# unixpickle/learn-nerf

Hardware: AMD Instinct MI355X
Metric: ray-samples/s (NeRF train step: fwd + bwd + Adam, 4096 rays x 192 samples per GPU) (higher is better)
Workload: dtype bf16; 1 GPU; vanilla NeRF coarse64+fine128 train step (BASELINE.json configs[1]); rays_per_gpu=4096, coarse_samples=64, fine_samples=128, global_batch_rays=4096, parallelism=dp1, precision=bf16 MFMA, fp32 accumulate/master weights

## Files before the change

include/lnrf.h:

```cpp
#ifndef LNRF_H
#define LNRF_H

#include <stddef.h>
#include <stdint.h>

#ifdef __cplusplus
extern "C" {
#endif

typedef void* lnrf_stream_t;

#define LNRF_VERSION 200

#define LNRF_OK 0
#define LNRF_ERR_ARG (-1)
#define LNRF_ERR_SHAPE (-2)
#define LNRF_ERR_UNSUPPORTED (-3)

#define LNRF_ACT_NONE 0
#define LNRF_ACT_RELU 1
#define LNRF_ACT_SOFTPLUS 2
#define LNRF_ACT_TANH 3
#define LNRF_ACT_EXP 4
#define LNRF_ACT_SIGMOID 5

int lnrf_version(void);
const char* lnrf_last_error(void);


int lnrf_ray_aabb_stratified(const float* rays, int64_t ray_stride, int64_t n_rays,
                             const float* bbox_min, const float* bbox_max, float min_t_range,
                             float epsilon, int32_t count, const float* u, uint64_t seed,
                             uint32_t stream_id, int64_t ray_offset, float* t_min, float* t_max,
                             uint8_t* mask, float* ts, lnrf_stream_t stream);

int lnrf_camera_rays(const float* origin, const float* x_axis, const float* y_axis, const float* z_axis,
                     float x_fov, float y_fov, int32_t width, int32_t height, float* rays,
                     lnrf_stream_t stream);

int lnrf_gather_rows(const float* src, int64_t n_src, int32_t row_floats, const int32_t* idx, int64_t n,
                     float* out, lnrf_stream_t stream);

int lnrf_stratified(const float* t_min, const float* t_max, int64_t n_rays, int32_t count,
                    const float* u, uint64_t seed, uint32_t stream_id, int64_t ray_offset,
                    float* ts, lnrf_stream_t stream);

int lnrf_ray_points(const float* rays, int64_t ray_stride, const float* ts, int64_t n_rays,
                    int32_t t, float* points, float* dirs, lnrf_stream_t stream);

int lnrf_fine_sample(const float* ts_c, const float* t_min, const float* t_max,
                     const float* density_c, int64_t n_rays, int32_t tc, int32_t tf, float eps,
                     int32_t combine, const float* u, uint64_t seed, uint32_t stream_id,
                     int64_t ray_offset, float* ts_out, lnrf_stream_t stream);

int lnrf_bin_edges(const float* ts, const float* t_min, const float* t_max, int64_t n_rays,
                   int32_t t, float* starts, float* ends, lnrf_stream_t stream);

int lnrf_termination_probs(const float* ts, const float* t_min, const float* t_max,
                           const float* density, int64_t n_rays, int32_t t, float* probs,
                           lnrf_stream_t stream);

int lnrf_composite_fwd(const float* rays, int64_t ray_stride, const float* ts, const float* t_min,
                       const float* t_max, const uint8_t* mask, const float* density,
                       const float* rgb, const float* aux, int32_t n_aux, const float* background,
                       int64_t n_rays, int32_t t, float* outputs, float* alphas, float* coords,
                       float* aux_sum, const float* targets, int64_t target_stride, float* sq_err,
                       lnrf_stream_t stream);

int64_t lnrf_composite_bwd_scratch_bytes(int64_t n_rays);
int lnrf_composite_bwd_det(const float* ts, const float* t_min, const float* t_max, const uint8_t* mask,
                           const float* density, const float* rgb, const float* aux, int32_t n_aux,
                           const float* background, int64_t n_rays, int32_t t, const float* g_out, const float* outputs,
                           const float* targets, int64_t target_stride, float out_scale, const float* g_aux_w,
                           float* g_density, float* g_rgb, float* g_aux, float* g_background, void* scratch,
                           int64_t scratch_bytes, lnrf_stream_t stream);

int lnrf_distortion(const float* ts, const float* t_min, const float* t_max, const uint8_t* mask,
                    const float* density, int64_t n_rays, int32_t t, float grad_scale, float* loss,
                    float* g_density, lnrf_stream_t stream);


int lnrf_sinusoidal_emb(const float* x, int64_t ldx, int64_t m, int32_t dims, int32_t freqs,
                        float* out, int64_t ldo, int64_t col_off, lnrf_stream_t stream);

#define LNRF_DENSE_FP32 0
#define LNRF_DENSE_BF16 1
int lnrf_set_dense_precision(int32_t precision);
int32_t lnrf_get_dense_precision(void);

int lnrf_dense_fwd(const float* x, int64_t ldx, const float* w, const float* b, int32_t act,
                   float* y, int64_t ldy, int64_t m, int32_t k, int32_t n, lnrf_stream_t stream);

int lnrf_act_bwd(float* g, int64_t ldg, const float* y, int64_t ldy, int32_t act, int64_t m,
                 int32_t n, lnrf_stream_t stream);

int lnrf_dense_bwd_input(const float* gy, int64_t ldgy, const float* w, float* gx, int64_t ldgx,
                         int32_t accumulate, int64_t m, int32_t k, int32_t n, lnrf_stream_t stream);

int lnrf_dense_bwd_input_gated(const float* gy, int64_t ldgy, const float* w, const float* y_below, int64_t ldy,
                               int32_t act_below, int32_t n_gated, float* gx, int64_t ldgx, int32_t accumulate,
                               int64_t m, int32_t k, int32_t n, lnrf_stream_t stream);
int lnrf_dense_fwd_gated(const float* x, int64_t ldx, const float* w, const float* b, int32_t act,
                         const float* y_gate, int64_t ldg, int32_t act_gate, float* y, int64_t ldy, int64_t m,
                         int32_t k, int32_t n, lnrf_stream_t stream);

int64_t lnrf_dense_bwd_weight_scratch_bytes(int64_t m, int32_t k, int32_t n);
int lnrf_dense_bwd_weight_det(const float* x, int64_t ldx, const float* gy, int64_t ldgy, float* gw, float* gb,
                              int64_t m, int32_t k, int32_t n, void* scratch, int64_t scratch_bytes,
                              lnrf_stream_t stream);

int lnrf_gemm_f32(const float* a, int64_t sa_i, int64_t sa_r, const float* b, int64_t sb_r, int64_t sb_j,
                  float* c, int64_t ldc, const float* bias, int32_t act, int32_t mode, int64_t i_rows,
                  int32_t j_cols, int64_t r_depth, int32_t splits, lnrf_stream_t stream);

int64_t lnrf_gemm_f32_det_scratch_bytes(int64_t i_rows, int32_t j_cols, int64_t r_depth);
int lnrf_gemm_f32_det(const float* a, int64_t sa_i, int64_t sa_r, const float* b, int64_t sb_r, int64_t sb_j, float* c,
                      int64_t i_rows, int32_t j_cols, int64_t r_depth, void* scratch, int64_t scratch_bytes,
                      lnrf_stream_t stream);


typedef struct {
  int32_t n_levels, feature_dim, smooth, pad_;
  float bbox_min[3], bbox_max[3];
  int32_t grid_size[32];
  int32_t table_size[32];
  int64_t table_offset[32];
  int32_t hashed[32];
} lnrf_hashgrid_desc;

int lnrf_hashgrid_fwd(const lnrf_hashgrid_desc* desc, const float* tables, const float* x, int64_t m,
                      float* enc_t, lnrf_stream_t stream);

int64_t lnrf_hashgrid_bwd_scratch_bytes(const lnrf_hashgrid_desc* desc, int64_t m);
int lnrf_hashgrid_bwd_bucketed(const lnrf_hashgrid_desc* desc, const float* x, const float* u, int64_t m,
                               const float* g_enc_t, const float* level_absmax, float* g_tables, void* scratch,
                               int64_t scratch_bytes, lnrf_stream_t stream);

int lnrf_hashgrid_jvp(const lnrf_hashgrid_desc* desc, const float* tables, const float* x, const float* u,
                      int64_t m, float* enc_t, lnrf_stream_t stream);
int lnrf_hashgrid_input_grad(const lnrf_hashgrid_desc* desc, const float* tables, const float* x, int64_t m,
                             const float* g_enc_t, float* g_x, lnrf_stream_t stream);
int lnrf_hashgrid_bwd_dir(const lnrf_hashgrid_desc* desc, const float* x, const float* u, int64_t m,
                          const float* g_enc_t, float* g_tables, lnrf_stream_t stream);


int lnrf_sinusoidal_emb_bwd(const float* x, int64_t ldx, int64_t m, int32_t dims, int32_t freqs,
                            const float* g_emb, int64_t ldg, int64_t col_off, float* g_x,
                            lnrf_stream_t stream);
int lnrf_sinusoidal_emb_jvp(const float* x, int64_t ldx, int64_t m, int32_t dims, int32_t freqs,
                            const float* u, float* v_emb, int64_t ldv, int64_t col_off,
                            lnrf_stream_t stream);

int lnrf_integrated_directional_encoding(int32_t sh_degree, const float* coords, const float* roughness,
                                         int64_t m, float* out, lnrf_stream_t stream);

int lnrf_refnerf_head_fwd(const float* spatial, int64_t lds, const float* nraw, const float* d, int64_t m,
                          int32_t sh_degree, float* density, float* diffuse, float* spectral, float* tail,
                          int64_t ld_tail, float* aux, lnrf_stream_t stream);
int lnrf_refnerf_head_bwd(const float* spatial, int64_t lds, const float* nraw, const float* d, int64_t m,
                          int32_t sh_degree, const float* g_density, const float* g_diffuse,
                          const float* g_spectral, const float* g_tail, int64_t ld_tail, const float* g_aux,
                          float* g_spatial, int64_t ldgs, float* g_nraw, lnrf_stream_t stream);

int lnrf_refnerf_color_fwd(const float* dir_out, const float* spectral, const float* diffuse, int64_t m,
                           float* rgb, lnrf_stream_t stream);
int lnrf_refnerf_color_bwd(const float* dir_out, const float* spectral, const float* diffuse, int64_t m,
                           const float* g_rgb, float* g_dir_out, float* g_spectral, float* g_diffuse,
                           lnrf_stream_t stream);


typedef struct {
  int32_t input_layers, mid_layers, hidden_dim, color_layer_dim, x_freqs, d_freqs;
} lnrf_nerf_shape;

int64_t lnrf_nerf_param_count(const lnrf_nerf_shape* shape);
int64_t lnrf_nerf_packed_bytes(const lnrf_nerf_shape* shape);
int64_t lnrf_nerf_save_bytes(const lnrf_nerf_shape* shape, int64_t m);
int64_t lnrf_nerf_bwd_scratch_bytes(const lnrf_nerf_shape* shape, int64_t m);

int lnrf_nerf_pack_weights(const lnrf_nerf_shape* shape, const float* params, void* packed,
                           lnrf_stream_t stream);

int lnrf_nerf_mlp_fwd(const lnrf_nerf_shape* shape, const void* packed, const float* x,
                      const float* d, const float* rays, int64_t ray_stride, const float* ts,
                      int32_t t, int64_t m, float* density, float* rgb, void* save,
                      lnrf_stream_t stream);

int lnrf_nerf_mlp_fwd_ls(const lnrf_nerf_shape* shape, const void* packed, const float* x,
                         const float* d, const float* rays, int64_t ray_stride, const float* ts,
                         int32_t t, int64_t m, float* density, float* rgb, void* save,
                         lnrf_stream_t stream);

int64_t lnrf_nerf_packed_split_bytes(const lnrf_nerf_shape* shape);
int lnrf_nerf_pack_weights_split(const lnrf_nerf_shape* shape, const float* params, void* packed_split,
                                 lnrf_stream_t stream);
int lnrf_nerf_mlp_fwd_split(const lnrf_nerf_shape* shape, const void* packed_split, const float* x,
                            const float* d, const float* rays, int64_t ray_stride, const float* ts,
                            int32_t t, int64_t m, float* density, float* rgb, lnrf_stream_t stream);

int lnrf_nerf_mlp_bwd_chain(const lnrf_nerf_shape* shape, const void* packed, const void* save,
                            const float* density, const float* rgb, const float* g_density,
                            const float* g_rgb, int64_t m, void* scratch, lnrf_stream_t stream);

int lnrf_nerf_mlp_bwd_weights(const lnrf_nerf_shape* shape, const void* save, void* scratch,
                              int64_t m, float* grads, lnrf_stream_t stream);

int64_t lnrf_nerf_bwd_ls_scratch_bytes(const lnrf_nerf_shape* shape, int64_t m);
int64_t lnrf_nerf_bwd_ls_status_offset(const lnrf_nerf_shape* shape, int64_t m);
int lnrf_nerf_mlp_bwd_ls(const lnrf_nerf_shape* shape, const void* packed, const void* save,
                         const float* density, const float* rgb, const float* g_density,
                         const float* g_rgb, int64_t m, void* scratch, float* grads, int32_t phases,
                         lnrf_stream_t stream);
int lnrf_nerf_mlp_bwd_ls2(const lnrf_nerf_shape* shape, const void* packed_a, const void* save_a,
                          const float* density_a, const float* rgb_a, const float* g_density_a,
                          const float* g_rgb_a, int64_t m_a, void* scratch_a, float* grads_a,
                          const void* packed_b, const void* save_b, const float* density_b,
                          const float* rgb_b, const float* g_density_b, const float* g_rgb_b, int64_t m_b,
                          void* scratch_b, float* grads_b, int32_t phases, lnrf_stream_t stream);

int64_t lnrf_refnerf_trunk_packed_bytes(void);
int lnrf_refnerf_trunk_pack(const float* params, void* packed, lnrf_stream_t stream);
int lnrf_refnerf_trunk_fwd(const void* packed, const float* x, int64_t m, void* save, float* spatial_out,
                           int64_t ld, lnrf_stream_t stream);
int lnrf_refnerf_normal_pass(const void* packed, const void* save, const float* x, int64_t m, void* cdump,
                             float* nraw, lnrf_stream_t stream);
int64_t lnrf_refnerf_trunk_bwd_scratch_bytes(int64_t m);
int lnrf_refnerf_trunk_bwd(const void* packed, const void* save, const float* g_spatial, int64_t ld, int64_t m,
                           void* scratch, float* grads, lnrf_stream_t stream);
// ... 154 lines not shown
```

learn-nerf_amd/csrc/layout_host.cpp:

```cpp
#include <stdint.h>
#include <string.h>

#include "dense_plan.h"
#include "fast_math.h"
#include "hashgrid_plan.h"
#include "nerf_wgrad.h"
#include "ngp_layout.h"

using namespace lnrf;

static WgradList wgrad_list_of(int which, int64_t n_tiles) {
  return which == 0 ? wgrad_list_split(n_tiles) : which == 1 ? wgrad_list_ls_finish(n_tiles)
       : which == 2 ? wgrad_list_ref_trunk(n_tiles) : which == 3 ? wgrad_list_ref_normal(n_tiles)
                                                                 : wgrad_list_ref_dir(n_tiles);
}
template <int NXF, int NYF, int WI, int WO>
static int64_t wgrad_count_owners(const WgradProblem& pb, int32_t* count, int64_t n) {
  int64_t outside = 0;
  int64_t i;
  auto hit = [&](bool owned) {
    if (!owned) return;
    if (i >= 0 && i < n) ++count[i];
    else ++outside;
  };
  for (int w = 0; w < kWaves; ++w)
    for (int j = 0; j < kWgradWaveTiles<NXF, NYF, WI, WO>; ++j) {
      const WgradTile tile = wgrad_tile<NXF, NYF, WI, WO>(w, j);
      if (!tile.real) continue;
      for (int lane = 0; lane < 64; ++lane) {
        const int colr = lane & 31, hh = lane >> 5;
        const WgradOwner<NerfWgradEpi, WgradProblem> own(pb, tile.ot, colr);
        if (tile.bias && pb.do_bias) hit(own.bias(hh, i));
        for (int qq = 0; qq < 16; ++qq) hit(own.weight(pb, tile.it, hh, qq, i));
      }
    }
  return outside;
}

template <int P>
static int64_t ngp_count_owners(const NgpWgradProblem& pb, int64_t dense_off, int32_t* count, int64_t n) {
  constexpr int NO = kNgpWgrad[P].nyf / 2, NT = ngp_wgrad_tiles(P);
  int64_t outside = 0;
  auto hit = [&](int part, int64_t i) {
    if (i >= 0 && i < n) ++count[part * n + i];
    else ++outside;
  };
  for (int w4 = 0; w4 < 4; ++w4)
    for (int lane = 0; lane < 64; ++lane) {
      const int colr = lane & 31, hh = lane >> 5;
      const int tile_id = w4 % NT, part = w4 / NT;
      const int it = tile_id / NO, ot = tile_id % NO;
      int out_idx = -1, out_dim = 1;
      int64_t w_off = 0, b_off = 0;
      NgpWgradEpi::cols(pb, ot, colr, out_idx, out_dim, w_off, b_off);
      w_off -= dense_off;
      b_off -= dense_off;
      if (it == 0 && hh == 0 && out_idx >= 0) hit(part, b_off + out_idx);
      for (int qq = 0; qq < 16; ++qq) {
        const int r = ngp_acc_row(qq, hh);
        const int f = 2 * it + (r >> 4);
        const int in_idx = NgpWgradEpi::row(pb, f, r & 15);
        if (out_idx >= 0 && in_idx >= 0) hit(part, w_off + (int64_t)in_idx * out_dim + out_idx);
      }
    }
  return outside;
}
static bool ngp_enc_dim_ok(int enc_dim) { return enc_dim >= 1 && enc_dim <= 32; }
static HashGridDesc hashgrid_desc_of(const void* desc) {
  HashGridDesc d;
  memcpy(&d, desc, sizeof(d));
  return d;
}

extern "C" {
int lnrf_host_fwd_frags(void) { return kFwdFrags; }
int lnrf_host_bwd_frags(void) { return kBwdFrags; }
int lnrf_host_bias_floats(void) { return kBiasFloats; }
int lnrf_host_fwd_used(void) { return kFwdUsed; }
int lnrf_host_fwd_seq(int c) { return fwd_seq(c); }
int lnrf_host_fwd3_frags(void) { return kFwd3Frags; }
int lnrf_host_fwd3_used(void) { return kFwd3Used; }
int lnrf_host_fwd3_seq(int c) { return fwd3_seq(c); }
int lnrf_host_fwd3_base(int s) { return fwd3_base(s); }
int lnrf_host_bwd_seq(int c) { return bwd_seq(c); }
int lnrf_host_fwd_layer_info(int s, int what) {
  return what == 0 ? fwd_nk(s) : what == 1 ? fwd_no(s) : what == 2 ? fwd_base(s) : what == 3 ? fwd_bias_base(s)
                                                                                             : fwd_cons_base(s);
}
int lnrf_host_bwd_layer_info(int t, int what) {
  return what == 0 ? bwd_nk(t) : what == 1 ? bwd_no(t) : what == 2 ? bwd_base(t) : bwd_dense(t);
}
int lnrf_host_fwd_weight_index(int g, int lane, int j) { return fwd_stream_index(g, lane, j, false); }
int lnrf_host_bwd_weight_index(int g, int lane, int j) { return bwd_stream_index(g, lane, j, false); }
int lnrf_host_fwd_bias_index(int i) { return bias_block_index(i, false); }
int lnrf_host_nrm_frags(void) { return kNrmFrags; }
int lnrf_host_nrm_weight_index(int g, int lane, int j) { return nrm_stream_index(g, lane, j); }
int64_t lnrf_host_stream_indices(int stream, int ref, int32_t* out) {
  const int frags[8] = {kFwdFrags, kBwdFrags, kFwd3Frags, 0, kNrmFrags, kDirFwdFrags, kDirBwdFrags, 0};
  if (stream < 0 || stream > 7) return -1;
  if (stream == 3 || stream == 7) {
    const int n = stream == 3 ? kBiasFloats : kDirBiasFloats;
    for (int i = 0; out && i < n; ++i) out[i] = stream == 3 ? bias_block_index(i, ref != 0) : dir_bias_index(i);
    return n;
  }
  const int64_t n = (int64_t)frags[stream] * 512;
  for (int64_t e = 0; out && e < n; ++e) {
    const int g = (int)(e >> 9), lane = (int)((e >> 3) & 63), j = (int)(e & 7);
    out[e] = stream == 0 ? fwd_stream_index(g, lane, j, ref != 0) : stream == 1 ? bwd_stream_index(g, lane, j, ref != 0)
           : stream == 2 ? fwd3_stream_index(g, lane, j, ref != 0) : stream == 4 ? nrm_stream_index(g, lane, j)
           : stream == 5 ? dir_fwd_weight_index(g, lane, j) : dir_bwd_weight_index(g, lane, j);
  }
  return n;
}
int64_t lnrf_host_pack_offset(int what) {
  const int64_t v[17] = {kPackFwdOff, kPackBwdOff, kPackBiasOff, kPackBytes, kPack3BiasOff, kPack3Bytes,
                         kRefPackNrmOff, kRefPackDirFwdOff, kRefPackDirBwdOff, kRefPackDirBiasOff, kRefPackBytes,
                         kRef3FwdOff, kRef3BiasOff, kRef3NrmOff, kRef3DirOff, kRef3DirBiasOff, kRef3Bytes};
  return what >= 0 && what < 17 ? v[what] : -1;
}
int lnrf_host_xemb_feat(int ks, int h, int j) { return xemb_feat(ks, h, j); }
int lnrf_host_save_slot(int what, int arg) {
  return what == 0 ? kSaveXin : what == 1 ? kSaveH + 16 * arg : what == 2 ? kSaveZ : what == 3 ? kSaveDin
       : what == 4 ? kSaveH10 : what == 5 ? kSaveMask : kSaveSlots;
}
int lnrf_host_grad_slot(int what, int arg) {
  return what == 0 ? kGradDy11 : what == 1 ? kGradDy10m : what == 2 ? grad_dy_slot(arg) : kGradSlots;
}
int lnrf_host_dir_slot(int what) {
  const int v[7] = {kDirSaveXin, kDirSaveH, kDirSaveMask, kDirSaveSlots, kDirGradDy10, kDirGradDy9, kDirGradSlots};
  return what >= 0 && what < 7 ? v[what] : -1;
}
int lnrf_host_demb_feat(int ks, int h, int j) { return demb_feat(ks, h, j); }
int lnrf_host_hidden_feat(int ks, int h, int j) { return hidden_feat(ks, h, j); }
int lnrf_host_dump_info(int what) { return what == 0 ? kFragBytes : what == 1 ? kTileCols : kWaves; }
int lnrf_host_mask_bit(int ks, int j) { return 16 * (ks >> 1) + 8 * (ks & 1) + j; }
int lnrf_host_dump_lane_off(int slot, int c, int hh) { return dump_lane_off(slot, c, hh); }
void lnrf_host_sincos_pe(float r, float* s, float* c) { lnrf::sincos_pe(r, s, c); }

int lnrf_host_wgrad_const(int what) {
  const int v[8] = {kWgradMaxBlocks, kSlabMaxTiles, kSlabMaxTO, kParamCount, kDirW9, kDirB9, kDirW10, kDirB10};
  return v[what];
}
int lnrf_host_wgrad_list(int which, int64_t n_tiles, int32_t* out) {
  const WgradList list = wgrad_list_of(which, n_tiles);
  for (int i = 0; i < list.args.n_problems; ++i) {
    const WgradProblem& pb = list.args.p[i];
    int32_t* o = out + 6 * i;
    o[0] = pb.first_block; o[1] = pb.n_blocks; o[4] = pb.do_bias; o[5] = 0;
    switch (pb.shape) {
#define X(name, id, NXF, NYF, WI, WO, SPI) case name: o[2] = WgShape<name>::TI * WgShape<name>::TO; o[3] = WgShape<name>::TO; break;
      LNRF_WGRAD_SHAPES(X, X)
#undef X
      default: return -1;
    }
    switch (pb.shape) {
#define X(name) case name:
      LNRF_WGRAD_LS_SHAPES(X, X) o[5] = 1; break;
#undef X
      default: break;
    }
  }
  return list.args.n_problems;
}
int64_t lnrf_host_ngp_stream_indices(int stream, int enc_dim, int32_t* out) {
  if (stream < 0 || stream > 2 || !ngp_enc_dim_ok(enc_dim)) return -1;
  const NgpOffsets off = ngp_offsets(enc_dim, 0);
  const int ne = ngp_ne(enc_dim);
  const int64_t n = stream == 2 ? kNgpBiasFloats : (int64_t)kNgpStreamFrags * 512;
  for (int64_t e = 0; out && e < n; ++e) {
    const int g = (int)(e >> 9), lane = (int)((e >> 3) & 63), j = (int)(e & 7);
    out[e] = (int32_t)(stream == 0 ? ngp_fwd_stream_index(g, lane, j, off, enc_dim, ne)
                     : stream == 1 ? ngp_bwd_stream_index(g, lane, j, off, enc_dim, ne) : ngp_bias_index((int)e, off));
  }
  return n;
}
int64_t lnrf_host_ngp_pack_offset(int what) {
  const int64_t v[7] = {kNgpPackBiasOff, kNgpPackBytes, kNgpSplitBiasOff, kNgpSplitBytes, kNgpStreamFrags,
                        kNgpSplitMaxFrags / 2, kNgpMaxParts};
  return what >= 0 && what < 7 ? v[what] : -1;
}
int64_t lnrf_host_ngp_wgrad_owners(int enc_dim, int32_t* count, int64_t n) {
  if (!ngp_enc_dim_ok(enc_dim)) return -1;
  const int64_t dense_off = 1001;
  const NgpWgradArgs a = ngp_wgrad_args(ngp_offsets(enc_dim, dense_off), enc_dim);
  return ngp_count_owners<0>(a.p[0], dense_off, count, n) + ngp_count_owners<1>(a.p[1], dense_off, count, n) +
         ngp_count_owners<2>(a.p[2], dense_off, count, n) + ngp_count_owners<3>(a.p[3], dense_off, count, n) +
         ngp_count_owners<4>(a.p[4], dense_off, count, n);
}
int lnrf_host_ngp_parts_plan(int enc_dim, int32_t* out) {
  if (!ngp_enc_dim_ok(enc_dim)) return -1;
  const NgpPartsPlan pl = ngp_parts_plan(ngp_offsets(enc_dim, 1001), 1001);
  for (int i = 0; i < kNgpLayers; ++i) {
    int32_t* o = out + 4 * i;
    o[0] = kNgpWgrad[i].layer; o[1] = pl.lo[i]; o[2] = pl.hi[i]; o[3] = pl.parts[i];
  }
  return ngp_dense_params(enc_dim);
}
void lnrf_host_gemm_plan(int64_t sa_i, int64_t sa_r, int64_t sb_r, int64_t sb_j, int64_t I, int32_t J, int64_t R,
                         uint32_t a_low, uint32_t b_low, int32_t bf16, int32_t mode, int32_t splits, int64_t* out) {
  const GemmPlan p = gemm_plan(sa_i, sa_r, sb_r, sb_j, I, J, R, a_low, b_low, bf16 != 0, mode, splits);
  const int64_t v[15] = {p.launch, p.big, p.bf16, p.a_fast_r, p.b_fast_r, p.b_aligned, p.kc, p.nsplit, p.lda, p.ldb,
                         p.r_per_split, p.gx, p.gy, p.gz, p.splits};
  for (int i = 0; i < 15; ++i) out[i] = v[i];
}
void lnrf_host_gemm_tile(int64_t I, int32_t J, uint32_t block0, int64_t count, int64_t* out) {
  for (int64_t e = 0; e < count; ++e) {
    const GemmTile t = gemm_big_tile(block0 + (uint32_t)e, (I + BI - 1) / BI, (J + BJ - 1) / BJ);
    out[2 * e] = t.it;
    out[2 * e + 1] = t.jt;
  }
}
int64_t lnrf_host_dense_bwd_weight_scratch_bytes(int64_t m, int32_t k, int32_t n) { return dense_wgrad_scratch_bytes(m, k, n); }
int64_t lnrf_host_gemm_det_scratch_bytes(int64_t I, int32_t J, int64_t R) { return gemm_det_scratch_bytes(I, J, R); }
void lnrf_host_hashgrid_corners(const void* desc, int32_t level, const float* x, uint32_t* idx, float* w, float* dw) {
  const HashGridDesc d = hashgrid_desc_of(desc);
  const int G = d.grid_size[level];
  const Corner k = locate(x, d, G);
  for (int c = 0; c < 8; ++c) {
    const int xo = c >> 2, yo = (c >> 1) & 1, zo = c & 1;
    idx[c] = entry_index(k.base[0] + xo, k.base[1] + yo, k.base[2] + zo, G, d.table_size[level], d.hashed[level]);
    w[c] = corner_weight(k, xo, yo, zo);
    corner_weight_grad(k, xo, yo, zo, dw + 3 * c);
  }
}
int64_t lnrf_host_hashgrid_xcd_plan(const void* desc, const int32_t* levels, int32_t n, int64_t m, int32_t* plan,
                                    int64_t* work) {
  const HashGridDesc d = hashgrid_desc_of(desc);
  LevelList ll;
  ll.n = n;
  for (int i = 0; i < n; ++i) ll.level[i] = levels[i];
  unsigned grid = 0;
  const XcdPlan p = make_xcd_plan(d, ll, m, &grid);
  for (int x = 0; plan && x <= kXcds; ++x) plan[x] = p.first_seg[x];
  for (int s = 0; plan && s < p.n_segs; ++s) {
    plan[9 + 3 * s] = p.seg_level[s]; plan[10 + 3 * s] = p.seg_chunk0[s]; plan[11 + 3 * s] = p.seg_chunks[s];
  }
  for (unsigned b = 0; work && b < grid; ++b) {
    const XcdWork w = xcd_work(p, b);
    work[2 * b] = w.seg < 0 ? -1 : xcd_level(p, w);
    work[2 * b + 1] = w.seg < 0 ? 0 : xcd_first_sample(p, w);
  }
  return grid;
}
int32_t lnrf_host_hashgrid_bucket_plan(const void* desc, int64_t m, int64_t* levels, int64_t* scratch) {
  const BucketPlan p = make_plan(hashgrid_desc_of(desc), m);
  for (int i = 0; i < p.n; ++i) {
    const int64_t v[7] = {p.level[i], p.slices[i], p.split[i], p.wg_off[i], p.tuple_off[i], p.cursor_off[i], p.cap[i]};
    for (int j = 0; j < 7; ++j) levels[7 * i + j] = v[j];
  }
  const BucketScratch s = bucket_scratch(p);
  scratch[0] = s.cursor_bytes; scratch[1] = s.level_max_off; scratch[2] = s.tuple_off; scratch[3] = s.total;
  scratch[4] = p.wg_off[p.n];
  return p.n;
}
void lnrf_host_hashgrid_reduce_work(const void* desc, int64_t m, int32_t block0, int64_t count, int64_t tuples,
                                    int64_t* out) {
  const BucketPlan p = make_plan(hashgrid_desc_of(desc), m);
  for (int64_t e = 0; e < count; ++e) {
    const ReduceWork w = reduce_work(p, block0 + (int)e);
    const TupleRange r = reduce_range(p, w, tuples);
    const int64_t v[6] = {w.li, w.level, w.bucket, w.part, r.lo, r.hi};
    for (int j = 0; j < 6; ++j) out[6 * e + j] = v[j];
  }
}
int64_t lnrf_host_wgrad_owners(int which, int64_t n_tiles, int32_t* count, int64_t n) {
  const WgradList list = wgrad_list_of(which, n_tiles);
// ... 13 lines not shown
```

learn-nerf_amd/csrc/nerf_bwd_ls.hip:

```cpp
#include "nerf_chain.h"

namespace lnrf {

constexpr int kLsWaves = 4;
constexpr int kLsThreads = kLsWaves * 64;
constexpr int kLsStages = 8;
constexpr int kLsLag = 2;
constexpr int kLsDist = kLsLag + 1;
constexpr int kLsBufs = kLsDist + 1;
constexpr int kLsTileBytes = 32 * kFragBytes;
constexpr int kLsPollOff = kLsBufs * kLsTileBytes;
constexpr int kLsLds = kLsPollOff + 5 * 256;
constexpr unsigned kLsMaxSpins = 1u << 18;
constexpr int kLsSlabWaveFloats = 16 * kSlabTileFloats + 2 * 64;
constexpr int64_t kLsSlabBlockBytes = (int64_t)kLsWaves * kLsSlabWaveFloats * (int64_t)sizeof(float);
constexpr int kLsCounterStride = 32;

struct LsJob {
  const char* packed;
  const char* save;
  char* gdump;
  unsigned* counters;
  float* slabs;
  unsigned* status;
// ... 391 lines not shown
    }
  } else if (bid - n_small < kLsStages * 64) {
    ls_fold_block<kSlabReduceWaves>(bid - n_small, a.ls_slabs[k], a.pipelines[k], a.grads[k], lds);
  }
}

struct BwdHeadSeq {
  static constexpr int count = bwd_cons_base(2);
  static constexpr int at(int c) { return bwd_seq(c); }
};
constexpr int kBwdHeadStages = bwd_base(2) / kStageFrags;

__global__ __launch_bounds__(kThreads) void nerf_bwd_head_kernel(
    const char* __restrict__ packed, const char* __restrict__ save, const float* __restrict__ density,
    const float* __restrict__ rgb, const float* __restrict__ g_density, const float* __restrict__ g_rgb,
    int64_t M, int64_t n_tiles, char* __restrict__ gdump, unsigned* __restrict__ zero_words, int n_zero_words) {
  const int tid = threadIdx.x;
  const int lane = tid & 63;
  const int wave = __builtin_amdgcn_readfirstlane(tid >> 6);
  const int64_t tile = (int64_t)blockIdx.x * kWaves + wave;
  for (int i = blockIdx.x * kThreads + tid; i < n_zero_words; i += gridDim.x * kThreads) zero_words[i] = 0u;
  Ring<kBwdHeadStages, BwdHeadSeq> ring;
  ring.stream = packed + kPackBwdOff;
  ring.wave = wave;
  ring.lane = lane;
  const DumpAddr gd{gdump, n_tiles, tile, lane & 31, lane >> 5, kGradTileSlots};
  bwd_chain_tile<true>(ring, gd, save, n_tiles, density, rgb, g_density, g_rgb, M, tile, lane);
}

}

using namespace lnrf;

#ifdef LNRF_TIMELINE
extern "C" int lnrf_debug_set_ls_timeline(void* buf) {
  hipError_t e = hipMemcpyToSymbol(HIP_SYMBOL(lnrf::g_ls_timeline_buf), &buf, sizeof(buf));
  return e == hipSuccess ? LNRF_OK : hip_fail(e, "hipMemcpyToSymbol(g_ls_timeline_buf)");
}
#endif

constexpr int kLsMaxPipelines = 64;
static int ls_pipelines_for_device(int need, int* out) {
  int cus = 0;
  if (int rc = cu_count(&cus)) return rc;
  *out = cus / kLsStages < kLsMaxPipelines ? cus / kLsStages : kLsMaxPipelines;
  if (*out < need) {
    set_error("layer-stationary backward: the device has too few CUs for a pipeline of 8 per model");
    return LNRF_ERR_UNSUPPORTED;
  }
  return LNRF_OK;
}

constexpr int64_t kLsCounterWords = (int64_t)kLsMaxPipelines * kLsStages * kLsCounterStride;
constexpr int64_t kLsCounterBytes = (kLsCounterWords + 64) * (int64_t)sizeof(unsigned);
struct LsScratch {
  int64_t small_slabs, counters, status, ls_slabs, bytes;
};
static LsScratch ls_scratch(int64_t m) {
  LsScratch s;
  s.small_slabs = (int64_t)kGradSlots * padded_tiles(m) * kFragBytes;
  s.counters = s.small_slabs + kWgradSlabBytes;
  s.status = s.counters + kLsCounterWords * (int64_t)sizeof(unsigned);
  s.ls_slabs = s.counters + kLsCounterBytes;
  s.bytes = s.ls_slabs + (int64_t)kLsMaxPipelines * kLsStages * kLsSlabBlockBytes;
  return s;
}
static LsJob ls_job(const void* packed, const void* save, void* scratch, int64_t m, int pipelines) {
  const LsScratch at = ls_scratch(m);
  char* sc = (char*)scratch;
  return LsJob{(const char*)packed, (const char*)save, sc, reinterpret_cast<unsigned*>(sc + at.counters),
               reinterpret_cast<float*>(sc + at.ls_slabs), reinterpret_cast<unsigned*>(sc + at.status), padded_tiles(m),
               pipelines};
}

extern "C" int64_t lnrf_nerf_bwd_ls_scratch_bytes(const lnrf_nerf_shape* s, int64_t m) {
  return nerf_shape_fused(s) ? ls_scratch(m).bytes : -1;
}
extern "C" int64_t lnrf_nerf_bwd_ls_status_offset(const lnrf_nerf_shape* s, int64_t m) {
  return nerf_shape_fused(s) ? ls_scratch(m).status : -1;
}
int64_t lnrf::ls_scratch_bytes(int64_t m) { return ls_scratch(m).bytes; }
float* lnrf::ls_small_slabs(void* scratch, int64_t m) {
  return reinterpret_cast<float*>((char*)scratch + ls_scratch(m).small_slabs);
}

int lnrf::launch_ls_pipeline(const void* packed, const void* save, void* scratch, int64_t m, float* grads, hipStream_t st) {
  int total = 0;
  int rc = ls_pipelines_for_device(1, &total);
  if (!rc) rc = set_max_dynamic_lds(nerf_bwd_ls_kernel, kLsLds);
  if (rc) return rc;
  LsArgs a;
  a.n_jobs = 1;
  a.total_pipelines = total;
  a.job[0] = a.job[1] = ls_job(packed, save, scratch, m, total);
  hipError_t e = hipMemsetAsync(a.job[0].counters, 0, kLsCounterBytes, st);
  if (e != hipSuccess) return hip_fail(e, "hipMemsetAsync(counters)");
  hipLaunchKernelGGL(nerf_bwd_ls_kernel, dim3((unsigned)(total * kLsStages)), dim3(kLsThreads), kLsLds, st, a);
  LNRF_LAUNCH_CHECK();
  hipLaunchKernelGGL(nerf_ls_reduce_kernel, dim3(kLsStages * 64), dim3(256), 0, st, (const float*)a.job[0].slabs, total, grads);
  LNRF_LAUNCH_CHECK();
  return LNRF_OK;
}

namespace {
struct LsModel {
  const void* packed;
  const void* save;
  const float *density, *rgb, *g_density, *g_rgb;
  int64_t m;
  void* scratch;
  float* grads;
};
}

static int ls_backward(const LsModel* mdl, int n_models, int phases, hipStream_t st) {
  constexpr int kHeadLds = kRingBytes + round_up(kBiasFloats * 4, 1024);
  int total = 0;
  int rc = ls_pipelines_for_device(n_models, &total);
  if (!rc) rc = set_max_dynamic_lds(nerf_bwd_head_kernel, kHeadLds);
  if (!rc) rc = set_max_dynamic_lds(nerf_bwd_ls_kernel, kLsLds);
  if (rc) return rc;
  int pipes[2] = {total, 0};
  if (n_models == 2) {
    const double share = (double)mdl[0].m / (double)(mdl[0].m + mdl[1].m);
    pipes[0] = (int)(total * share + 0.5);
    if (pipes[0] < 1) pipes[0] = 1;
    if (pipes[0] > total - 1) pipes[0] = total - 1;
    pipes[1] = total - pipes[0];
  }
  LsArgs a;
  a.n_jobs = n_models;
  a.total_pipelines = total;
  for (int k = 0; k < n_models; ++k) {
    const LsModel& md = mdl[k];
    const LsJob& j = a.job[k] = ls_job(md.packed, md.save, md.scratch, md.m, pipes[k]);
    if (phases & 1) {
      hipLaunchKernelGGL(nerf_bwd_head_kernel, dim3((unsigned)(j.n_tiles / kWaves)), dim3(kThreads), kHeadLds, st, j.packed,
                         j.save, md.density, md.rgb, md.g_density, md.g_rgb, md.m, j.n_tiles, j.gdump, j.counters,
                         (phases & 2) ? (int)(kLsCounterBytes / sizeof(unsigned)) : 0);
      LNRF_LAUNCH_CHECK();
    }
    if ((phases & 3) == 2) {
      hipError_t e = hipMemsetAsync(j.counters, 0, kLsCounterBytes, st);
      if (e != hipSuccess) return hip_fail(e, "hipMemsetAsync(counters)");
    }
  }
  if (n_models == 1) a.job[1] = a.job[0];
  if (phases & 2) {
    hipLaunchKernelGGL(nerf_bwd_ls_kernel, dim3((unsigned)(total * kLsStages)), dim3(kLsThreads), kLsLds, st, a);
    LNRF_LAUNCH_CHECK();
  }
  if (!(phases & 4)) return LNRF_OK;
  LsFoldArgs fold;
  for (int k = 0; k < n_models; ++k) {
    const LsModel& md = mdl[k];
    const LsJob& j = a.job[k];
    const WgradList w = wgrad_list_ls_finish(j.n_tiles);
    float* small_slabs = ls_small_slabs(md.scratch, md.m);
    rc = launch_nerf_wgrad(w, md.save, md.scratch, j.n_tiles, md.grads, st, WgLayout{kSaveTileSlots, kGradTileSlots, 1},
                           small_slabs, false, false);
    if (rc) return rc;
    fold.w[k] = w.args;
    fold.small_slabs[k] = small_slabs;
    fold.ls_slabs[k] = j.slabs;
    fold.grads[k] = md.grads;
    fold.pipelines[k] = pipes[k];
  }
  if (n_models == 1) {
    fold.w[1] = fold.w[0]; fold.small_slabs[1] = fold.small_slabs[0]; fold.ls_slabs[1] = fold.ls_slabs[0];
    fold.grads[1] = fold.grads[0]; fold.pipelines[1] = fold.pipelines[0];
  }
  const int gx = fold.w[0].n_problems * kWaves * kSlabMaxTiles + kLsStages * 64;
  hipLaunchKernelGGL(nerf_ls_fold_kernel, dim3((unsigned)gx, (unsigned)n_models), dim3(64 * kSlabReduceWaves), 0, st, fold);
  LNRF_LAUNCH_CHECK();
  return LNRF_OK;
}

extern "C" int lnrf_nerf_mlp_bwd_ls(const lnrf_nerf_shape* shape, const void* packed, const void* save,
                                    const float* density, const float* rgb, const float* g_density,
                                    const float* g_rgb, int64_t m, void* scratch, float* grads, int32_t phases,
                                    lnrf_stream_t stream) {
  LNRF_REQUIRE_NERF_SHAPE(shape);
  LNRF_CHECK_ARG(packed && save && density && rgb && g_density && g_rgb && scratch && grads, "null pointer");
  LNRF_CHECK_ARG(m >= 0, "bad m");
  if (m == 0) return LNRF_OK;
  LNRF_CHECK_ARG(phases >= 1 && phases <= 7, "phases: bit 0 head, bit 1 pipeline, bit 2 small problems + fold");
  const LsModel md{packed, save, density, rgb, g_density, g_rgb, m, scratch, grads};
  return ls_backward(&md, 1, phases, as_stream(stream));
}

extern "C" int lnrf_nerf_mlp_bwd_ls2(const lnrf_nerf_shape* shape, const void* packed_a, const void* save_a,
                                     const float* density_a, const float* rgb_a, const float* g_density_a,
                                     const float* g_rgb_a, int64_t m_a, void* scratch_a, float* grads_a,
                                     const void* packed_b, const void* save_b, const float* density_b,
                                     const float* rgb_b, const float* g_density_b, const float* g_rgb_b, int64_t m_b,
                                     void* scratch_b, float* grads_b, int32_t phases, lnrf_stream_t stream) {
  LNRF_REQUIRE_NERF_SHAPE(shape);
  LNRF_CHECK_ARG(packed_a && save_a && density_a && rgb_a && g_density_a && g_rgb_a && scratch_a && grads_a, "null pointer");
  LNRF_CHECK_ARG(packed_b && save_b && density_b && rgb_b && g_density_b && g_rgb_b && scratch_b && grads_b, "null pointer");
  LNRF_CHECK_ARG(m_a > 0 && m_b > 0, "both models need evaluations (use lnrf_nerf_mlp_bwd_ls for one)");
  const LsModel md[2] = {{packed_a, save_a, density_a, rgb_a, g_density_a, g_rgb_a, m_a, scratch_a, grads_a},
                         {packed_b, save_b, density_b, rgb_b, g_density_b, g_rgb_b, m_b, scratch_b, grads_b}};
  LNRF_CHECK_ARG(phases >= 1 && phases <= 7, "phases: bit 0 head, bit 1 pipeline, bit 2 small problems + fold");
  return ls_backward(md, 2, phases, as_stream(stream));
}
```

learn-nerf_amd/csrc/nerf_chain.h:

```cpp
#pragma once
#include "fused_chain.h"

namespace lnrf {

template <class Put>
__device__ __forceinline__ void x_encode(const float (&px)[3], int h, Put put) {
  static_for<4>([&](auto ks_) {
    constexpr int ks = decltype(ks_)::value;
#pragma unroll
    for (int pp = 0; pp < 4; ++pp) {
      const int p = 4 * ks + pp;
      float s = 0.0f, co = 0.0f;
      if (p < kXPairs) {
        const int pg = kXPairs * h + p;
        const int cd = pg / kXFreqs, f = pg - kXFreqs * cd;
        const float v = cd == 0 ? px[0] : (cd == 1 ? px[1] : px[2]);
        sincos_pe(v * (float)(1 << f), &s, &co);
      }
      put(ks_, 2 * pp, s);
      put(ks_, 2 * pp + 1, co);
    }
  });
}

template <int S, bool BIAS, class RING, class Epi>
__device__ __forceinline__ void trunk_layer(RING& ring, int h, const bf16x8 (&xe)[4], const bf16x8 (&in)[16], Epi epi) {
  chain_layer<fwd_cons_base(S), fwd_nk(S), fwd_no(S)>(
      ring,
      [&](auto o_) {
        if constexpr (BIAS) return bias_acc(fwd_bias_base(S) + 32 * decltype(o_)::value, h);
        else return zero_acc();
      },
      [&](auto k_) -> bf16x8 {
        constexpr int ks = decltype(k_)::value;
        if constexpr (S == 0) return xe[ks];
        else if constexpr (ks < 16) return in[ks];
        else return xe[ks - 16];
      },
      epi);
}
template <int S, class RING, class Epi>
__device__ __forceinline__ void trunk_layer_split(RING& ring, int h, const bf16x8 (&xe_hi)[4], const bf16x8 (&xe_lo)[4],
                                                  const bf16x8 (&inh)[16], const bf16x8 (&inl)[16], Epi epi) {
  chain_layer_split<fwd_cons_base(S), fwd_nk(S), fwd_no(S)>(
      ring, [&](auto o_) { return bias_acc(fwd_bias_base(S) + 32 * decltype(o_)::value, h); },
      [&](auto k_) -> bf16x8 {
        constexpr int ks = decltype(k_)::value;
        if constexpr (S == 0) return xe_hi[ks];
        else if constexpr (ks < 16) return inh[ks];
        else return xe_hi[ks - 16];
      },
      [&](auto k_) -> bf16x8 {
        constexpr int ks = decltype(k_)::value;
        if constexpr (S == 0) return xe_lo[ks];
        else if constexpr (ks < 16) return inl[ks];
        else return xe_lo[ks - 16];
      },
      epi);
}
template <int O>
__device__ __forceinline__ void masked_out_tile(const f32x16& acc, const uint4& mk, bf16x8 (&out)[16], const DumpAddr& gd,
                                                int slot0) {
  const unsigned mb = mask_word(mk, O);
  out[2 * O] = masked_frag<0>(acc, mb, 16 * (O & 1));
  out[2 * O + 1] = masked_frag<1>(acc, mb, 16 * (O & 1));
  gd.store(slot0 + 2 * O, frag_to_bits(out[2 * O]));
  gd.store(slot0 + 2 * O + 1, frag_to_bits(out[2 * O + 1]));
}
template <int C0, int L, class RING>
__device__ __forceinline__ void hidden_back(RING& ring, bf16x8 (&in)[16], bf16x8 (&out)[16], const uint4& mk,
                                            const DumpAddr& gd) {
  chain_layer<C0, 16, 8>(
      ring, [&](auto) { return zero_acc(); }, [&](auto k_) -> bf16x8 { return in[decltype(k_)::value]; },
      [&](auto o_, const f32x16& acc) { masked_out_tile<decltype(o_)::value>(acc, mk, out, gd, grad_dy_slot(L - 1)); });
}

struct BwdSeq {
  static constexpr int count = kBwdUsed;
  static constexpr int at(int c) { return bwd_seq(c); }
};
constexpr int kBwdStages = kBwdFrags / kStageFrags;

template <bool HEAD_ONLY = false, class RING>
__device__ __forceinline__ void bwd_chain_tile(RING& ring, const DumpAddr& gd, const char* __restrict__ save,
                                               int64_t save_tiles, const float* __restrict__ density,
                                               const float* __restrict__ rgb, const float* __restrict__ g_density,
                                               const float* __restrict__ g_rgb, int64_t M, int64_t tile, int lane) {
  const int c = lane & 31, h = lane >> 5;
  const int64_t m = tile * kTileCols + c;
  const bool valid = m < M;

  float gy11[3] = {0, 0, 0}, gy9 = 0.0f;
  if (valid && h == 0) {
#pragma unroll
    for (int k = 0; k < 3; ++k) {
      const float y = rgb[m * 3 + k];
      gy11[k] = g_rgb[m * 3 + k] * (1.0f - y * y);
    }
    gy9 = g_density[m] * -expm1f(-density[m]);
  }
  uint4 relu_mask[9];
#pragma unroll
  for (int i = HEAD_ONLY ? 8 : 0; i < 9; ++i)
    relu_mask[i] = *mask_at(save, kSaveMask + i, tile, save_tiles, kSaveTileSlots, lane);
  __syncthreads();
  ring.prologue();
  LNRF_TL_STAMP(ring);

  bf16x8 a0[16], a1[16];

  bf16x8 dy11 = zero_frag();
  dy11[0] = (__bf16)gy11[0];
  dy11[1] = (__bf16)gy11[1];
  dy11[2] = (__bf16)gy11[2];
  gd.store(kGradDy11, frag_to_bits(dy11));
  gd.store(kGradDy11 + 1, frag_to_bits(zero_frag()));

  chain_layer<bwd_cons_base(0), bwd_nk(0), bwd_no(0)>(
      ring, [&](auto) { return zero_acc(); }, [&](auto) -> bf16x8 { return dy11; },
      [&](auto o_, const f32x16& acc) {
        masked_out_tile<decltype(o_)::value>(acc, relu_mask[8], a0, gd, kGradDy10m);
      });
  bf16x8 dlogit = zero_frag();
  dlogit[0] = (__bf16)gy9;
  gd.store(kGradDy10m + 8, frag_to_bits(dlogit));
  gd.store(kGradDy10m + 9, frag_to_bits(zero_frag()));

  chain_layer<bwd_cons_base(1), bwd_nk(1), bwd_no(1)>(
      ring, [&](auto) { return zero_acc(); },
      [&](auto k_) -> bf16x8 {
        constexpr int ks = decltype(k_)::value;
        if constexpr (ks < 8) return a0[ks];
        else return dlogit;
      },
      [&](auto o_, const f32x16& acc) {
        constexpr int o = decltype(o_)::value;
        a1[2 * o] = acc_to_frag<0, false>(acc);
        a1[2 * o + 1] = acc_to_frag<1, false>(acc);
        gd.store(grad_dy_slot(8) + 2 * o, frag_to_bits(a1[2 * o]));
        gd.store(grad_dy_slot(8) + 2 * o + 1, frag_to_bits(a1[2 * o + 1]));
      });

  if constexpr (HEAD_ONLY) return;
  static_assert(bwd_nk(2) == 16 && bwd_no(2) == 8, "hidden_back");
  static_for<8>([&](auto i_) {
    constexpr int TT = 2 + decltype(i_)::value, l = bwd_dense(TT);
    if constexpr (TT % 2 == 0) hidden_back<bwd_cons_base(TT), l>(ring, a1, a0, relu_mask[l - 1], gd);
    else hidden_back<bwd_cons_base(TT), l>(ring, a0, a1, relu_mask[l - 1], gd);
  });
}

int launch_nerf_wgrad(const WgradList& list, const void* xbuf, const void* ybuf, int64_t n_tiles, float* grads,
                      hipStream_t stream, WgLayout lay, float* slabs, bool plain_loads = false,
                      bool fold = true);

int64_t ls_scratch_bytes(int64_t m);
float* ls_small_slabs(void* scratch, int64_t m);
int launch_ls_pipeline(const void* packed, const void* save, void* scratch, int64_t m, float* grads, hipStream_t stream);

}
```

learn-nerf_amd/csrc/nerf_layout.h:

```cpp
#pragma once
#include <stdint.h>

#if defined(__HIPCC__)
#define NL_HD __host__ __device__ __forceinline__
#else
#define NL_HD inline
#endif

namespace lnrf {
namespace nl {

constexpr int kFragBytes = 1024;
constexpr int kStageFrags = 16;
constexpr int kTileCols = 32;
constexpr int kWaves = 8;

constexpr int kNumDense = 12;
NL_HD constexpr int dense_in(int l) {
  return l == 0 ? 60 : (l == 5 ? 316 : (l == 10 ? 280 : (l == 11 ? 128 : 256)));
}
NL_HD constexpr int dense_out(int l) { return l == 9 ? 1 : (l == 10 ? 128 : (l == 11 ? 3 : 256)); }
NL_HD constexpr int dense_w_off(int l) {
  int off = 0;
  for (int i = 0; i < l; ++i) off += dense_in(i) * dense_out(i) + dense_out(i);
// ... 127 lines not shown
NL_HD constexpr int bwd_cons_base(int t) {
  int b = 0;
  for (int i = 0; i < t; ++i) b += bwd_nk(i) * bwd_no(i);
  return b;
}
constexpr int kBwdUsed = bwd_cons_base(kBwdLayers);
NL_HD constexpr int bwd_seq(int c) {
  int t = 0;
  for (int i = 1; i < kBwdLayers; ++i)
    if (c >= bwd_cons_base(i)) t = i;
  return bwd_base(t) + (c - bwd_cons_base(t));
}
NL_HD constexpr int bwd_dense(int t) { return t == 0 ? 11 : (t == 1 ? 10 : 10 - t); }

NL_HD constexpr int bwd_weight_index(int t, int o, int ks, int lane, int j) {
  const int r = lane & 31, h = lane >> 5;
  const int in = 32 * o + r;
  if (t == 0) {
    if (h != 0 || j >= 3) return -1;
    return dense_w_off(11) + in * 3 + j;
  }
  if (t == 1) {
    if (ks < 8) return dense_w_off(10) + in * 128 + hidden_feat(ks, h, j);
    if (h == 0 && j == 0) return dense_w_off(9) + in;
    return -1;
  }
  const int l = bwd_dense(t);
  return dense_w_off(l) + in * 256 + hidden_feat(ks, h, j);
}

constexpr int kNrmLayers = 10;
NL_HD constexpr bool nrm_is_x(int u) { return u == 3 || u == 9; }
NL_HD constexpr int nrm_nk(int) { return 16; }
NL_HD constexpr int nrm_no(int u) { return nrm_is_x(u) ? 2 : 8; }
NL_HD constexpr int nrm_base(int u) {
  int b = 0;
  for (int i = 0; i < u; ++i) b += nrm_nk(i) * nrm_no(i);
  return b;
}
constexpr int kNrmFrags = nrm_base(kNrmLayers);
static_assert(kNrmFrags == 1088 && kNrmFrags % kStageFrags == 0, "normal-pass stream length");
NL_HD constexpr int nrm_seq(int c) { return c; }
NL_HD constexpr int nrm_dense(int u) { return u < 3 ? 8 - u : (u == 4 ? 5 : 9 - u); }
NL_HD constexpr int nrm_x_row(int o, int r) {
  const int hh = (r >> 2) & 1, q = (r & 3) + 4 * (r >> 3);
  const int pg = 16 * o + 8 * hh + (q >> 1);
  if (pg >= 30) return -1;
  return 20 * (pg / 10) + (pg % 10) + 10 * (q & 1);
}
NL_HD constexpr int nrm_weight_index(int u, int o, int ks, int lane, int j) {
  const int r = lane & 31, h = lane >> 5;
  const int k = hidden_feat(ks, h, j);
  if (nrm_is_x(u)) {
    const int e = nrm_x_row(o, r);
    if (e < 0) return -1;
    return u == 3 ? dense_w_off(5) + (256 + e) * 256 + k : dense_w_off(0) + e * 256 + k;
  }
  return dense_w_off(nrm_dense(u)) + (32 * o + r) * 256 + k;
}

constexpr int64_t kPackFwdOff = 0;
constexpr int64_t kPackBwdOff = (int64_t)kFwdFrags * kFragBytes;
constexpr int64_t kPackBiasOff = kPackBwdOff + (int64_t)kBwdFrags * kFragBytes;
constexpr int64_t kPackBytes = kPackBiasOff + round_up(kBiasFloats * 4, 1024);
constexpr int kDirIn = 273, kDirHidden = 128;
constexpr int kDirW9 = dense_w_off(9);
constexpr int kDirB9 = kDirW9 + kDirIn * kDirHidden;
constexpr int kDirW10 = kDirB9 + kDirHidden;
constexpr int kDirB10 = kDirW10 + kDirHidden * 3;
constexpr int kDirFwdFrags = 96, kDirBwdFrags = 96, kDirBiasFloats = 160;
NL_HD constexpr int dir_fwd_seq(int c) { return c < 72 ? c : 80 + (c - 72); }
NL_HD constexpr int dir_bwd_seq(int c) { return c < 4 ? c : 16 + (c - 4); }
NL_HD constexpr int dir_fwd_weight_index(int g, int lane, int j) {
  const int r = lane & 31, h = lane >> 5;
  if (g < 72) {
    const int o = g / 18, ks = g % 18;
    const int in = hidden_feat(ks, h, j);
    return in < kDirIn ? kDirW9 + in * kDirHidden + 32 * o + r : -1;
  }
  if (g >= 80 && g < 88) {
    if (r >= 3) return -1;
    return kDirW10 + hidden_feat(g - 80, h, j) * 3 + r;
  }
  return -1;
}
NL_HD constexpr int dir_bwd_weight_index(int g, int lane, int j) {
  const int r = lane & 31, h = lane >> 5;
  if (g < 4) {
    if (h != 0 || j >= 3) return -1;
    return kDirW10 + (32 * g + r) * 3 + j;
  }
  if (g >= 16 && g < 88) {
    const int o = (g - 16) / 8, ks = (g - 16) % 8;
    const int in = 32 * o + r;
    return in < kDirIn ? kDirW9 + in * kDirHidden + hidden_feat(ks, h, j) : -1;
  }
  return -1;
}
NL_HD constexpr int dir_bias_index(int i) { return i < 128 ? kDirB9 + i : (i < 131 ? kDirB10 + (i - 128) : -1); }
constexpr int kDirSaveXin = 0, kDirSaveH = 18, kDirSaveMask = 26, kDirSaveSlots = 27;
constexpr int kDirGradDy10 = 0, kDirGradDy9 = 2, kDirGradSlots = 10;

constexpr int64_t kRefPackNrmOff = kPackBytes;
constexpr int64_t kRefPackDirFwdOff = kRefPackNrmOff + (int64_t)kNrmFrags * kFragBytes;
constexpr int64_t kRefPackDirBwdOff = kRefPackDirFwdOff + (int64_t)kDirFwdFrags * kFragBytes;
constexpr int64_t kRefPackDirBiasOff = kRefPackDirBwdOff + (int64_t)kDirBwdFrags * kFragBytes;
constexpr int64_t kRefPackBytes = kRefPackDirBiasOff + 1024;
constexpr int kRef3FwdFrags = fwd3_base(9);
constexpr int64_t kRef3FwdOff = 0;
constexpr int64_t kRef3BiasOff = (int64_t)kRef3FwdFrags * kFragBytes;
constexpr int64_t kRef3NrmOff = kRef3BiasOff + round_up(kBiasFloats * 4, 1024);
constexpr int64_t kRef3DirOff = kRef3NrmOff + 2 * (int64_t)kNrmFrags * kFragBytes;
constexpr int64_t kRef3DirBiasOff = kRef3DirOff + 2 * (int64_t)kDirFwdFrags * kFragBytes;
constexpr int64_t kRef3Bytes = kRef3DirBiasOff + 1024;
static_assert(kRef3FwdFrags % kStageFrags == 0 && (2 * kNrmFrags) % kStageFrags == 0 && (2 * kDirFwdFrags) % kStageFrags == 0,
              "split streams are whole stages");

NL_HD constexpr int fwd_stream_index(int g, int lane, int j, bool ref) {
  int s = 0;
  for (int i = 1; i < kFwdLayers; ++i)
    if (g >= fwd_base(i)) s = i;
  const int loc = g - fwd_base(s), nk = fwd_nk(s);
  if (loc >= nk * fwd_no(s) || (ref && s > 8)) return -1;
  return fwd_weight_index(s, loc / nk, loc % nk, lane, j);
}
NL_HD constexpr int bwd_stream_index(int g, int lane, int j, bool ref) {
  int t = 0;
  for (int i = 1; i < kBwdLayers; ++i)
    if (g >= bwd_base(i)) t = i;
  const int loc = g - bwd_base(t), nk = bwd_nk(t);
  if (loc >= nk * bwd_no(t) || (ref && t < 2)) return -1;
  return bwd_weight_index(t, loc / nk, loc % nk, lane, j);
}
NL_HD constexpr int nrm_stream_index(int g, int lane, int j) {
  int u = 0;
  for (int i = 1; i < kNrmLayers; ++i)
    if (g >= nrm_base(i)) u = i;
  const int loc = g - nrm_base(u);
  return nrm_weight_index(u, loc / nrm_nk(u), loc % nrm_nk(u), lane, j);
}
NL_HD constexpr int fwd3_stream_index(int g, int lane, int j, bool ref) {
  int s = 0;
  for (int i = 1; i < kFwdLayers; ++i)
    if (g >= fwd3_base(i)) s = i;
  const int pair = (g - fwd3_base(s)) >> 1, nk = fwd_nk(s);
  if (pair >= nk * fwd_no(s) || (ref && s > 8)) return -1;
  return fwd_weight_index(s, pair / nk, pair % nk, lane, j);
}
NL_HD constexpr int bias_block_index(int i, bool ref) {
  int s = 0;
  for (int k = 1; k < kFwdLayers; ++k)
    if (i >= fwd_bias_base(k)) s = k;
  return ref && s > 8 ? -1 : fwd_bias_index(s, i - fwd_bias_base(s));
}

NL_HD constexpr int dump_lane_off(int slot, int c, int hh) {
  return 256 * (c >> 3) + 128 * (((c >> 2) & 1) ^ (slot & 1)) + 64 * hh + 16 * (c & 3);
}
constexpr int kSaveXin = 0;
constexpr int kSaveH = 4;
constexpr int kSaveZ = 4 + 8 * 16;
constexpr int kSaveDin = kSaveZ + 16;
constexpr int kSaveH10 = kSaveDin + 2;
constexpr int kSaveMask = kSaveH10 + 8;
constexpr int kSaveSlots = kSaveMask + 9;
constexpr int kGradDy11 = 0;
constexpr int kGradDy10m = 2;
constexpr int kGradDy = 12;
constexpr int kGradSlots = kGradDy + 9 * 16;
constexpr int kSaveTileSlots = kSaveSlots, kGradTileSlots = kGradSlots;
constexpr int kDirSaveTileSlots = kDirSaveSlots, kDirGradTileSlots = kDirGradSlots;
NL_HD constexpr int grad_dy_pos(int l) { return l == 5 ? 8 : (l > 5 ? 8 - l : 7 - l); }
NL_HD constexpr int grad_dy_slot(int l) { return kGradDy + grad_dy_pos(l) * 16; }

}
}
```

learn-nerf_amd/csrc/nerf_mlp.hip:

```cpp
#include "nerf_chain.h"

namespace lnrf {

constexpr int kFusedLds = kRingBytes + round_up(kBiasFloats * 4, 1024);
#ifdef LNRF_TIMELINE
__device__ unsigned long long* g_timeline_buf = nullptr;
#endif

struct FwdSeq {
  static constexpr int count = kFwdUsed;
  static constexpr int at(int c) { return fwd_seq(c); }
};

constexpr int kFwdStages = kFwdFrags / kStageFrags;

template <bool SAVE, bool FROM_RAYS, bool HMASKS = true>
__global__ __launch_bounds__(kThreads) void nerf_fwd_kernel(
    const char* __restrict__ packed, const float* __restrict__ xin_g, const float* __restrict__ din_g,
    const float* __restrict__ rays, int64_t ray_stride, const float* __restrict__ ts, int T, int64_t M,
    int64_t n_tiles, float* __restrict__ density, float* __restrict__ rgb, char* __restrict__ save) {
  const auto [lane, wave, c, h, tile, m, valid] = tile_ctx<kWaves>(M);

  stage_bias<kThreads>(packed + kPackBiasOff, kBiasFloats);
  float px[3] = {0, 0, 0}, pd[3] = {0, 0, 0};
  if (valid) {
    if (FROM_RAYS) {
      const int64_t n = m / T;
      const float t = ts[m];
      const float* r = rays + n * ray_stride;
#pragma unroll
      for (int a = 0; a < 3; ++a) {
        pd[a] = r[3 + a];
        px[a] = r[a] + pd[a] * t;
      }
    } else {
#pragma unroll
      for (int a = 0; a < 3; ++a) {
        px[a] = xin_g[m * 3 + a];
        pd[a] = din_g[m * 3 + a];
      }
    }
  }
  __syncthreads();

  Ring<kFwdStages, FwdSeq> ring;
  ring.stream = packed + kPackFwdOff;
  ring.wave = wave;
  ring.lane = lane;
#ifdef LNRF_TIMELINE
  ring.tl.buf = g_timeline_buf + (SAVE ? 0 : 8 * 1024);
  ring.tl.n = 0;
  ring.tl.on = g_timeline_buf != nullptr && blockIdx.x == gridDim.x / 2;
  ring.tl.stamp();
#endif
  ring.prologue();
  LNRF_TL_STAMP(ring);

  bf16x8 xe[4], de[2];
  x_encode(px, h, [&](auto ks_, int j, float v) { xe[decltype(ks_)::value][j] = (__bf16)v; });
  static_for<2>([&](auto ks_) {
    constexpr int ks = decltype(ks_)::value;
#pragma unroll
    for (int pp = 0; pp < 4; ++pp) {
      const int p = 4 * ks + pp;
      float s = 0.0f, co = 0.0f;
      if (p < 6) {
        const int pg = 6 * h + p;
        const int cd = pg >> 2, f = pg & 3;
        const float v = cd == 0 ? pd[0] : (cd == 1 ? pd[1] : pd[2]);
        sincos_pe(v * (float)(1 << f), &s, &co);
      }
      de[ks][2 * pp] = (__bf16)s;
      de[ks][2 * pp + 1] = (__bf16)co;
    }
  });

  DumpAddr dump{save, n_tiles, tile, c, h, kSaveTileSlots};
  auto save_frag = [&](int slot, const bf16x8& f) {
    if (SAVE) dump.store(slot, frag_to_bits(f));
  };
  if (SAVE) {
    static_for<4>([&](auto i) { save_frag(kSaveXin + decltype(i)::value, xe[decltype(i)::value]); });
    static_for<2>([&](auto i) { save_frag(kSaveDin + decltype(i)::value, de[decltype(i)::value]); });
  }

  bf16x8 a0[16], a1[16];
  unsigned mask_bits[4] = {0u, 0u, 0u, 0u};

  auto hidden = [&](auto s_, bf16x8(&in)[16], bf16x8(&out)[16], auto relu_, int save_slot) {
    constexpr int S = decltype(s_)::value;
    constexpr bool RELU = decltype(relu_)::value;
    trunk_layer<S, true>(ring, h, xe, in, [&](auto o_, const f32x16& acc) {
      constexpr int o = decltype(o_)::value;
      out[2 * o] = acc_to_frag<0, RELU>(acc);
      out[2 * o + 1] = acc_to_frag<1, RELU>(acc);
      save_frag(save_slot + 2 * o, out[2 * o]);
      save_frag(save_slot + 2 * o + 1, out[2 * o + 1]);
      if constexpr (SAVE && RELU && HMASKS)
        mask_bits[o >> 1] |= relu_bits(out[2 * o], out[2 * o + 1]) << (16 * (o & 1));
    });
    if constexpr (SAVE && RELU && HMASKS) {
      *mask_at(save, kSaveMask + S, tile, n_tiles, kSaveTileSlots, lane) =
          make_uint4(mask_bits[0], mask_bits[1], mask_bits[2], mask_bits[3]);
      mask_bits[0] = mask_bits[1] = mask_bits[2] = mask_bits[3] = 0u;
    }
  };
  std::true_type relu;
  std::false_type lin;
  hidden(std::integral_constant<int, 0>{}, a1, a0, relu, kSaveH + 0 * 16);
  hidden(std::integral_constant<int, 1>{}, a0, a1, relu, kSaveH + 1 * 16);
  hidden(std::integral_constant<int, 2>{}, a1, a0, relu, kSaveH + 2 * 16);
  hidden(std::integral_constant<int, 3>{}, a0, a1, relu, kSaveH + 3 * 16);
  hidden(std::integral_constant<int, 4>{}, a1, a0, relu, kSaveH + 4 * 16);
  hidden(std::integral_constant<int, 5>{}, a0, a1, relu, kSaveH + 5 * 16);
  hidden(std::integral_constant<int, 6>{}, a1, a0, relu, kSaveH + 6 * 16);
  hidden(std::integral_constant<int, 7>{}, a0, a1, relu, kSaveH + 7 * 16);
  hidden(std::integral_constant<int, 8>{}, a1, a0, lin, kSaveZ);

  chain_layer<fwd_cons_base(9), fwd_nk(9), fwd_no(9)>(
      ring, [&](auto o_) { return bias_acc(fwd_bias_base(9) + 32 * decltype(o_)::value, h); },
      [&](auto k_) -> bf16x8 {
        constexpr int ks = decltype(k_)::value;
        if constexpr (ks < 16) return a0[ks];
        else return de[ks - 16];
      },
      [&](auto o_, const f32x16& acc) {
        constexpr int o = decltype(o_)::value;
        if constexpr (o < 4) {
          a1[2 * o] = acc_to_frag<0, true>(acc);
          a1[2 * o + 1] = acc_to_frag<1, true>(acc);
          save_frag(kSaveH10 + 2 * o, a1[2 * o]);
          save_frag(kSaveH10 + 2 * o + 1, a1[2 * o + 1]);
          if constexpr (SAVE) mask_bits[o >> 1] |= relu_bits(a1[2 * o], a1[2 * o + 1]) << (16 * (o & 1));
        } else {
          if constexpr (SAVE)
            *mask_at(save, kSaveMask + 8, tile, n_tiles, kSaveTileSlots, lane) = make_uint4(mask_bits[0], mask_bits[1], 0u, 0u);
          if (h == 0 && valid) {
            const float x = acc[0];
            density[m] = fmaxf(x, 0.0f) + log1pf(expf(-fabsf(x)));
          }
        }
      });
  chain_layer<fwd_cons_base(10), fwd_nk(10), fwd_no(10)>(
      ring, [&](auto) { return bias_acc(fwd_bias_base(10), h); },
      [&](auto k_) -> bf16x8 { return a1[decltype(k_)::value]; },
      [&](auto, const f32x16& acc) {
        if (h == 0 && valid) {
          rgb[m * 3 + 0] = tanhf(acc[0]);
          rgb[m * 3 + 1] = tanhf(acc[1]);
          rgb[m * 3 + 2] = tanhf(acc[2]);
        }
      });
// ... 4 lines not shown
  static constexpr int count = kFwd3Used;
  static constexpr int at(int c) { return fwd3_seq(c); }
};

template <bool FROM_RAYS>
__global__ __launch_bounds__(kSplitThreads) void nerf_fwd_split_kernel(
    const char* __restrict__ packed, const float* __restrict__ xin_g, const float* __restrict__ din_g,
    const float* __restrict__ rays, int64_t ray_stride, const float* __restrict__ ts, int T, int64_t M,
    float* __restrict__ density, float* __restrict__ rgb) {
  const auto [lane, wave, c, h, tile, m, valid] = tile_ctx<kSplitWaves>(M);

  stage_bias<kSplitThreads>(packed + kPack3BiasOff, kBiasFloats);
  float px[3] = {0, 0, 0}, pd[3] = {0, 0, 0};
  if (valid) {
    if (FROM_RAYS) {
      const int64_t n = m / T;
      const float t = ts[m];
      const float* r = rays + n * ray_stride;
#pragma unroll
      for (int a = 0; a < 3; ++a) {
        pd[a] = r[3 + a];
        px[a] = r[a] + pd[a] * t;
      }
    } else {
#pragma unroll
      for (int a = 0; a < 3; ++a) {
        px[a] = xin_g[m * 3 + a];
        pd[a] = din_g[m * 3 + a];
      }
    }
  }
  __syncthreads();

  Ring<kFwd3Stages, Fwd3Seq, kSplitWaves> ring;
  ring.stream = packed;
  ring.wave = wave;
  ring.lane = lane;
  ring.prologue();

  bf16x8 xe_hi[4], xe_lo[4], de_hi[2], de_lo[2];
  x_encode(px, h, [&](auto ks_, int j, float v) { split_store(v, xe_hi[decltype(ks_)::value], xe_lo[decltype(ks_)::value], j); });
  static_for<2>([&](auto ks_) {
    constexpr int ks = decltype(ks_)::value;
#pragma unroll
    for (int pp = 0; pp < 4; ++pp) {
      const int p = 4 * ks + pp;
      float s = 0.0f, co = 0.0f;
      if (p < 6) {
        const int pg = 6 * h + p;
        const int cd = pg >> 2, f = pg & 3;
        const float v = cd == 0 ? pd[0] : (cd == 1 ? pd[1] : pd[2]);
        sincos_pe(v * (float)(1 << f), &s, &co);
      }
      split_store(s, de_hi[ks], de_lo[ks], 2 * pp);
      split_store(co, de_hi[ks], de_lo[ks], 2 * pp + 1);
    }
  });

  bf16x8 a0h[16], a0l[16], a1h[16], a1l[16];

  auto hidden = [&](auto s_, bf16x8(&inh)[16], bf16x8(&inl)[16], bf16x8(&outh)[16], bf16x8(&outl)[16], auto relu_) {
    constexpr bool RELU = decltype(relu_)::value;
    trunk_layer_split<decltype(s_)::value>(ring, h, xe_hi, xe_lo, inh, inl, [&](auto o_, const f32x16& acc) {
      constexpr int o = decltype(o_)::value;
      acc_to_frag_split<0, RELU>(acc, outh[2 * o], outl[2 * o]);
      acc_to_frag_split<1, RELU>(acc, outh[2 * o + 1], outl[2 * o + 1]);
    });
  };
  std::true_type relu;
  std::false_type lin;
  hidden(std::integral_constant<int, 0>{}, a1h, a1l, a0h, a0l, relu);
  hidden(std::integral_constant<int, 1>{}, a0h, a0l, a1h, a1l, relu);
  hidden(std::integral_constant<int, 2>{}, a1h, a1l, a0h, a0l, relu);
  hidden(std::integral_constant<int, 3>{}, a0h, a0l, a1h, a1l, relu);
  hidden(std::integral_constant<int, 4>{}, a1h, a1l, a0h, a0l, relu);
  hidden(std::integral_constant<int, 5>{}, a0h, a0l, a1h, a1l, relu);
  hidden(std::integral_constant<int, 6>{}, a1h, a1l, a0h, a0l, relu);
  hidden(std::integral_constant<int, 7>{}, a0h, a0l, a1h, a1l, relu);
  hidden(std::integral_constant<int, 8>{}, a1h, a1l, a0h, a0l, lin);

  chain_layer_split<fwd_cons_base(9), fwd_nk(9), fwd_no(9)>(
      ring, [&](auto o_) { return bias_acc(fwd_bias_base(9) + 32 * decltype(o_)::value, h); },
      [&](auto k_) -> bf16x8 {
        constexpr int ks = decltype(k_)::value;
        if constexpr (ks < 16) return a0h[ks];
        else return de_hi[ks - 16];
      },
      [&](auto k_) -> bf16x8 {
        constexpr int ks = decltype(k_)::value;
        if constexpr (ks < 16) return a0l[ks];
        else return de_lo[ks - 16];
      },
      [&](auto o_, const f32x16& acc) {
        constexpr int o = decltype(o_)::value;
        if constexpr (o < 4) {
          acc_to_frag_split<0, true>(acc, a1h[2 * o], a1l[2 * o]);
          acc_to_frag_split<1, true>(acc, a1h[2 * o + 1], a1l[2 * o + 1]);
        } else {
          if (h == 0 && valid) {
            const float x = acc[0];
            density[m] = fmaxf(x, 0.0f) + log1pf(expf(-fabsf(x)));
          }
        }
      });
  chain_layer_split<fwd_cons_base(10), fwd_nk(10), fwd_no(10)>(
      ring, [&](auto) { return bias_acc(fwd_bias_base(10), h); },
      [&](auto k_) -> bf16x8 { return a1h[decltype(k_)::value]; },
      [&](auto k_) -> bf16x8 { return a1l[decltype(k_)::value]; },
      [&](auto, const f32x16& acc) {
        if (h == 0 && valid) {
          rgb[m * 3 + 0] = tanhf(acc[0]);
          rgb[m * 3 + 1] = tanhf(acc[1]);
          rgb[m * 3 + 2] = tanhf(acc[2]);
        }
      });
}

__global__ __launch_bounds__(kThreads) void nerf_bwd_chain_kernel(
    const char* __restrict__ packed, const char* __restrict__ save, const float* __restrict__ density,
    const float* __restrict__ rgb, const float* __restrict__ g_density, const float* __restrict__ g_rgb,
    int64_t M, int64_t n_tiles, char* __restrict__ gdump) {
  const auto [lane, wave, c, h, tile, m, valid] = tile_ctx<kWaves>(M);

  Ring<kBwdStages, BwdSeq> ring;
  ring.stream = packed + kPackBwdOff;
  ring.wave = wave;
  ring.lane = lane;
#ifdef LNRF_TIMELINE
  ring.tl.buf = g_timeline_buf + 16 * 1024;
  ring.tl.n = 0;
  ring.tl.on = g_timeline_buf != nullptr && blockIdx.x == gridDim.x / 2;
  ring.tl.stamp();
#endif
  const DumpAddr gd{gdump, n_tiles, tile, c, h, kGradTileSlots};
  bwd_chain_tile(ring, gd, save, n_tiles, density, rgb, g_density, g_rgb, M, tile, lane);
}

template <bool PLAIN>
__global__ __launch_bounds__(kThreads) void nerf_wgrad_kernel(WgradArgs args, const char* __restrict__ save,
                                                              const char* __restrict__ gdump, int64_t n_tiles,
                                                              WgLayout lay, float* __restrict__ slabs) {
  WgradProblem pb = args.p[0];
#pragma unroll
  for (int i = 1; i < kMaxProblems; ++i)
    if (i < args.n_problems && (int)blockIdx.x >= args.p[i].first_block) pb = args.p[i];
  switch (pb.shape) {
#define X(name, id, NXF, NYF, WI, WO, SPI) \
  case name: wgrad_body<NXF, NYF, WI, WO, SPI, PLAIN>(pb, save, gdump, n_tiles, lay, slabs); break;
    LNRF_WGRAD_SHAPES(X, default: X)
#undef X
  }
}

__global__ __launch_bounds__(64 * kSlabReduceWaves) void nerf_wgrad_reduce_kernel(WgradArgs args,
                                                                                 const float* __restrict__ slabs,
                                                                                 float* __restrict__ grads) {
  __shared__ float lds[(kSlabReduceWaves - 1) * 17 * 64];
  const int prob = blockIdx.x / (kWaves * kSlabMaxTiles), w = blockIdx.x / kSlabMaxTiles % kWaves, j = blockIdx.x % kSlabMaxTiles;
  const WgradProblem pb = args.p[prob];
  switch (pb.shape) {
#define X(name, id, NXF, NYF, WI, WO, SPI) \
  case name: wgrad_reduce_tile<NXF, NYF, WI, WO, NerfWgradEpi>(pb, w, j, slabs, grads, lds); break;
    LNRF_WGRAD_SHAPES(X, default: X)
#undef X
  }
}

__global__ void nerf_pack_kernel(const float* __restrict__ params, char* __restrict__ packed) {
  constexpr int64_t units_f = (int64_t)kFwdFrags * 64, units_b = (int64_t)kBwdFrags * 64;
  constexpr int64_t total = units_f + units_b + kBiasFloats;
  for (int64_t u = (int64_t)blockIdx.x * blockDim.x + threadIdx.x; u < total; u += (int64_t)gridDim.x * blockDim.x) {
    if (u < units_f + units_b) {
      const bool fwd = u < units_f;
      const int64_t uu = fwd ? u : u - units_f;
      const int g = (int)(uu >> 6), lane = (int)(uu & 63);
      bf16x8 out;
#pragma unroll
      for (int j = 0; j < 8; ++j)
        out[j] = (__bf16)param_or_zero(params, fwd ? fwd_stream_index(g, lane, j, false) : bwd_stream_index(g, lane, j, false));
      *reinterpret_cast<bf16x8*>(packed + (fwd ? kPackFwdOff : kPackBwdOff) + uu * 16) = out;
    } else {
      const int i = (int)(u - units_f - units_b);
      reinterpret_cast<float*>(packed + kPackBiasOff)[i] = param_or_zero(params, bias_block_index(i, false));
    }
  }
}

__global__ void nerf_pack_split_kernel(const float* __restrict__ params, char* __restrict__ packed) {
  const int64_t total_w = (int64_t)kFwd3Frags * 512;
  const int64_t total = total_w + kBiasFloats;
  for (int64_t e = (int64_t)blockIdx.x * blockDim.x + threadIdx.x; e < total;
       e += (int64_t)gridDim.x * blockDim.x) {
    if (e < total_w) {
      const int g = (int)(e >> 9), lane = (int)((e >> 3) & 63), j = (int)(e & 7);
      reinterpret_cast<__bf16*>(packed)[e] = split_half(param_or_zero(params, fwd3_stream_index(g, lane, j, false)), g & 1);
    } else {
      const int i = (int)(e - total_w);
      reinterpret_cast<float*>(packed + kPack3BiasOff)[i] = param_or_zero(params, bias_block_index(i, false));
    }
  }
}

}

using namespace lnrf;

extern "C" int64_t lnrf_nerf_param_count(const lnrf_nerf_shape* s) {
  if (!s) return -1;
  const int64_t xe = 6 * s->x_freqs, de = 6 * s->d_freqs, hd = s->hidden_dim, cd = s->color_layer_dim;
  int64_t n = 0, fan = xe;
  for (int i = 0; i < s->input_layers; ++i) { n += fan * hd + hd; fan = hd; }
  fan = hd + xe;
  for (int i = 0; i < s->mid_layers; ++i) { n += fan * hd + hd; fan = hd; }
  n += hd + 1;
  n += (hd + de) * cd + cd;
  n += cd * 3 + 3;
  return n;
}
extern "C" int64_t lnrf_nerf_packed_bytes(const lnrf_nerf_shape* s) {
  return nerf_shape_fused(s) ? kPackBytes : -1;
}
extern "C" int64_t lnrf_nerf_save_bytes(const lnrf_nerf_shape* s, int64_t m) {
  return nerf_shape_fused(s) ? (int64_t)kSaveSlots * padded_tiles(m) * kFragBytes : -1;
}
static int64_t grad_dump_bytes(int64_t m) { return (int64_t)kGradSlots * padded_tiles(m) * kFragBytes; }
extern "C" int64_t lnrf_nerf_bwd_scratch_bytes(const lnrf_nerf_shape* s, int64_t m) {
  return nerf_shape_fused(s) ? grad_dump_bytes(m) + kWgradSlabBytes : -1;
}

extern "C" int lnrf_nerf_pack_weights(const lnrf_nerf_shape* shape, const float* params, void* packed,
                                      lnrf_stream_t stream) {
  LNRF_REQUIRE_NERF_SHAPE(shape);
  LNRF_CHECK_ARG(params && packed, "null pointer");
  hipLaunchKernelGGL(nerf_pack_kernel, dim3(640), dim3(256), 0, as_stream(stream), params, (char*)packed);
  LNRF_LAUNCH_CHECK();
  return LNRF_OK;
}

static int nerf_fwd_launch(const void* packed, const float* x, const float* d, const float* rays, int64_t ray_stride,
                           const float* ts, int32_t t, int64_t m, float* density, float* rgb, void* save,
                           bool hidden_masks, lnrf_stream_t stream) {
  LNRF_CHECK_ARG(packed && density && rgb, "null pointer");
  LNRF_CHECK_ARG(m >= 0, "bad m");
  const bool from_rays = rays != nullptr;
  if (from_rays) LNRF_CHECK_ARG(ts && t >= 1 && ray_stride >= 6 && m % t == 0, "rays mode needs ts, t, m = n*t");
  else LNRF_CHECK_ARG(x && d, "need x and d (or rays and ts)");
  if (m == 0) return LNRF_OK;
  const int64_t n_tiles = padded_tiles(m);
  const dim3 grid((unsigned)((n_tiles + kWaves - 1) / kWaves)), block(kThreads);
  hipStream_t st = as_stream(stream);
  int rc;
#define LAUNCH_FWD(SAVE, RAYS, HM)                                                                        \
  do {                                                                                                    \
    rc = set_max_dynamic_lds(nerf_fwd_kernel<SAVE, RAYS, HM>, kFusedLds);                                 \
    if (rc) return rc;                                                                                    \
    hipLaunchKernelGGL((nerf_fwd_kernel<SAVE, RAYS, HM>), grid, block, kFusedLds, st, (const char*)packed, \
                       x, d, rays, ray_stride, ts, (int)t, m, n_tiles, density, rgb, (char*)save);        \
  } while (0)
  if (save != nullptr && hidden_masks) {
    if (from_rays) LAUNCH_FWD(true, true, true); else LAUNCH_FWD(true, false, true);
  } else if (save != nullptr) {
    if (from_rays) LAUNCH_FWD(true, true, false); else LAUNCH_FWD(true, false, false);
  } else {
    if (from_rays) LAUNCH_FWD(false, true, true); else LAUNCH_FWD(false, false, true);
  }
#undef LAUNCH_FWD
  LNRF_LAUNCH_CHECK();
  return LNRF_OK;
}

extern "C" int lnrf_nerf_mlp_fwd(const lnrf_nerf_shape* shape, const void* packed, const float* x,
                                 const float* d, const float* rays, int64_t ray_stride, const float* ts,
                                 int32_t t, int64_t m, float* density, float* rgb, void* save,
                                 lnrf_stream_t stream) {
  LNRF_REQUIRE_NERF_SHAPE(shape);
  return nerf_fwd_launch(packed, x, d, rays, ray_stride, ts, t, m, density, rgb, save, true, stream);
}

extern "C" int lnrf_nerf_mlp_fwd_ls(const lnrf_nerf_shape* shape, const void* packed, const float* x,
                                    const float* d, const float* rays, int64_t ray_stride, const float* ts,
                                    int32_t t, int64_t m, float* density, float* rgb, void* save,
                                    lnrf_stream_t stream) {
  LNRF_REQUIRE_NERF_SHAPE(shape);
  return nerf_fwd_launch(packed, x, d, rays, ray_stride, ts, t, m, density, rgb, save, false, stream);
}

extern "C" int64_t lnrf_nerf_packed_split_bytes(const lnrf_nerf_shape* s) {
  return nerf_shape_fused(s) ? kPack3Bytes : -1;
}

extern "C" int lnrf_nerf_pack_weights_split(const lnrf_nerf_shape* shape, const float* params, void* packed,
                                            lnrf_stream_t stream) {
  LNRF_REQUIRE_NERF_SHAPE(shape);
  LNRF_CHECK_ARG(params && packed, "null pointer");
  hipLaunchKernelGGL(nerf_pack_split_kernel, dim3(1024), dim3(256), 0, as_stream(stream), params, (char*)packed);
  LNRF_LAUNCH_CHECK();
  return LNRF_OK;
}

extern "C" int lnrf_nerf_mlp_fwd_split(const lnrf_nerf_shape* shape, const void* packed_split, const float* x,
                                       const float* d, const float* rays, int64_t ray_stride, const float* ts,
                                       int32_t t, int64_t m, float* density, float* rgb, lnrf_stream_t stream) {
  LNRF_REQUIRE_NERF_SHAPE(shape);
  LNRF_CHECK_ARG(packed_split && density && rgb, "null pointer");
  LNRF_CHECK_ARG(m >= 0, "bad m");
  const bool from_rays = rays != nullptr;
  if (from_rays) LNRF_CHECK_ARG(ts && t >= 1 && ray_stride >= 6 && m % t == 0, "rays mode needs ts, t, m = n*t");
  else LNRF_CHECK_ARG(x && d, "need x and d (or rays and ts)");
  if (m == 0) return LNRF_OK;
  const int64_t n_tiles = (m + kTileCols - 1) / kTileCols;
  const dim3 grid((unsigned)((n_tiles + kSplitWaves - 1) / kSplitWaves)), block(kSplitThreads);
  hipStream_t st = as_stream(stream);
  int rc;
  if (from_rays) {
    rc = set_max_dynamic_lds(nerf_fwd_split_kernel<true>, kFusedLds);
    if (rc) return rc;
    hipLaunchKernelGGL((nerf_fwd_split_kernel<true>), grid, block, kFusedLds, st, (const char*)packed_split, x, d,
                       rays, ray_stride, ts, (int)t, m, density, rgb);
  } else {
    rc = set_max_dynamic_lds(nerf_fwd_split_kernel<false>, kFusedLds);
    if (rc) return rc;
    hipLaunchKernelGGL((nerf_fwd_split_kernel<false>), grid, block, kFusedLds, st, (const char*)packed_split, x, d,
                       rays, ray_stride, ts, (int)t, m, density, rgb);
  }
  LNRF_LAUNCH_CHECK();
  return LNRF_OK;
}

extern "C" int lnrf_nerf_mlp_bwd_chain(const lnrf_nerf_shape* shape, const void* packed, const void* save,
                                       const float* density, const float* rgb, const float* g_density,
                                       const float* g_rgb, int64_t m, void* scratch, lnrf_stream_t stream) {
  LNRF_REQUIRE_NERF_SHAPE(shape);
  LNRF_CHECK_ARG(packed && save && density && rgb && g_density && g_rgb && scratch, "null pointer");
  LNRF_CHECK_ARG(m >= 0, "bad m");
  if (m == 0) return LNRF_OK;
  const int64_t n_tiles = padded_tiles(m);
  hipStream_t st = as_stream(stream);
  int rc = set_max_dynamic_lds(nerf_bwd_chain_kernel, kFusedLds);
  if (rc) return rc;
  hipLaunchKernelGGL(nerf_bwd_chain_kernel, dim3((unsigned)((n_tiles + kWaves - 1) / kWaves)), dim3(kThreads),
                     kFusedLds, st, (const char*)packed, (const char*)save, density, rgb, g_density, g_rgb, m,
                     n_tiles, (char*)scratch);
  LNRF_LAUNCH_CHECK();
  return LNRF_OK;
}

int lnrf::launch_nerf_wgrad(const WgradList& list, const void* xbuf, const void* ybuf, int64_t n_tiles, float* grads,
                            hipStream_t stream, WgLayout lay, float* slabs, bool plain, bool fold) {
  LNRF_CHECK_ARG(slabs != nullptr && list.blocks <= kWgradMaxBlocks, "needs slabs, and holds at most kWgradMaxBlocks of them");
  const int lds = 2 * 2 * 36 * kFragBytes;
  const dim3 grid((unsigned)list.blocks), block(kThreads);
  int rc = plain ? set_max_dynamic_lds(nerf_wgrad_kernel<true>, lds) : set_max_dynamic_lds(nerf_wgrad_kernel<false>, lds);
  if (rc) return rc;
  if (plain)
    hipLaunchKernelGGL(nerf_wgrad_kernel<true>, grid, block, lds, stream, list.args, (const char*)xbuf,
                       (const char*)ybuf, n_tiles, lay, slabs);
  else
    hipLaunchKernelGGL(nerf_wgrad_kernel<false>, grid, block, lds, stream, list.args, (const char*)xbuf,
                       (const char*)ybuf, n_tiles, lay, slabs);
  LNRF_LAUNCH_CHECK();
  if (fold) {
    hipLaunchKernelGGL(nerf_wgrad_reduce_kernel, dim3((unsigned)(list.args.n_problems * kWaves * kSlabMaxTiles)),
                       dim3(64 * kSlabReduceWaves), 0, stream, list.args, (const float*)slabs, grads);
    LNRF_LAUNCH_CHECK();
  }
  return LNRF_OK;
}

extern "C" int lnrf_nerf_mlp_bwd_weights(const lnrf_nerf_shape* shape, const void* save, void* scratch,
                                         int64_t m, float* grads, lnrf_stream_t stream) {
  LNRF_REQUIRE_NERF_SHAPE(shape);
  LNRF_CHECK_ARG(save && scratch && grads, "null pointer");
  LNRF_CHECK_ARG(m >= 0, "bad m");
  if (m == 0) return LNRF_OK;
  const int64_t n_tiles = padded_tiles(m);
  float* slabs = reinterpret_cast<float*>(reinterpret_cast<char*>(scratch) + grad_dump_bytes(m));
  constexpr int64_t kPlainFrom = 16384;
  return launch_nerf_wgrad(wgrad_list_split(n_tiles), save, scratch, n_tiles, grads, as_stream(stream),
                           WgLayout{kSaveTileSlots, kGradTileSlots}, slabs, n_tiles >= kPlainFrom);
}

#ifdef LNRF_TIMELINE
extern "C" int lnrf_debug_set_timeline(void* buf) {
  hipError_t e = hipMemcpyToSymbol(HIP_SYMBOL(lnrf::g_timeline_buf), &buf, sizeof(buf));
  return e == hipSuccess ? LNRF_OK : hip_fail(e, "hipMemcpyToSymbol(g_timeline_buf)");
}
#endif
```

learn-nerf_amd/csrc/rays.hip:

```cpp
#include "common.h"
#include "philox.h"
#include "ray_geom.h"

namespace lnrf {

__global__ void ray_aabb_stratified_kernel(const float* __restrict__ rays, int64_t ray_stride,
                                           int64_t n_rays, BBox bb, float min_t_range, float eps,
                                           int count, const float* __restrict__ u, uint64_t seed,
                                           uint32_t stream_id, int64_t ray_offset,
                                           float* __restrict__ t_min, float* __restrict__ t_max,
                                           uint8_t* __restrict__ mask, float* __restrict__ ts) {
  const int per = count > 0 ? count : 1;
  const int64_t total = n_rays * per;
  for (int64_t e = (int64_t)blockIdx.x * blockDim.x + threadIdx.x; e < total;
       e += (int64_t)gridDim.x * blockDim.x) {
    const int64_t n = e / per;
    const int i = (int)(e - n * per);
    const TRange r = ray_t_range(rays + n * ray_stride, bb.mn, bb.mx, min_t_range, eps);
    if (i == 0) {
      if (t_min) t_min[n] = r.t_min;
      if (t_max) t_max[n] = r.t_max;
      if (mask) mask[n] = r.mask ? 1 : 0;
    }
    if (count > 0) {
// ... 23 lines not shown

__global__ void ray_points_kernel(const float* __restrict__ rays, int64_t ray_stride,
                                  const float* __restrict__ ts, int64_t n_rays, int t,
                                  float* __restrict__ points, float* __restrict__ dirs) {
  const int64_t total = n_rays * t;
  for (int64_t e = (int64_t)blockIdx.x * blockDim.x + threadIdx.x; e < total;
       e += (int64_t)gridDim.x * blockDim.x) {
    const int64_t n = e / t;
    const float* r = rays + n * ray_stride;
    const float tt = ts[e];
#pragma unroll
    for (int a = 0; a < 3; ++a) {
      if (points) points[e * 3 + a] = r[a] + r[3 + a] * tt;
      if (dirs) dirs[e * 3 + a] = r[3 + a];
    }
  }
}

struct Quad {
  float a;
  float incl;
  float prev;
  float t;
  float end;
};

__device__ __forceinline__ Quad quad_chunk(const float* __restrict__ ts_row,
                                           const float* __restrict__ dens_row, int T, int i,
                                           int lane, float tmin, float tmax, float carry) {
  Quad q;
  const bool valid = i < T;
  const int ic = valid ? i : T - 1;
  const float t_i = ts_row[ic];
  const float t_p = ic > 0 ? ts_row[ic - 1] : 0.0f;
  const float t_n = ic < T - 1 ? ts_row[ic + 1] : 0.0f;
  const float start = ic == 0 ? tmin : (t_i + t_p) / 2.0f;
  const float end = ic == T - 1 ? tmax : (t_n + t_i) / 2.0f;
  const float delta = end - start;
  q.a = valid ? dens_row[ic] * delta : 0.0f;
  q.incl = wave_incl_scan(q.a, lane) + carry;
  const float up = __shfl_up(q.incl, 1, 64);
  q.prev = lane == 0 ? carry : up;
  q.t = t_i;
  q.end = end;
  return q;
}

__global__ void termination_probs_kernel(const float* __restrict__ ts, const float* __restrict__ t_min,
                                         const float* __restrict__ t_max,
                                         const float* __restrict__ density, int64_t n_rays, int T,
                                         float* __restrict__ probs) {
  const int lane = threadIdx.x & 63;
  const int64_t n = (int64_t)blockIdx.x * (blockDim.x >> 6) + (threadIdx.x >> 6);
  if (n >= n_rays) return;
  const float* ts_row = ts + n * T;
  const float* de_row = density + n * T;
  const float tmin = t_min[n], tmax = t_max[n];
  float carry = 0.0f;
  for (int base = 0; base < T; base += 64) {
    const int i = base + lane;
    const Quad q = quad_chunk(ts_row, de_row, T, i, lane, tmin, tmax, carry);
    if (i < T) probs[n * (T + 1) + i] = expf(-q.prev) * (1.0f - expf(-q.a));
    carry = __shfl(q.incl, 63, 64);
  }
  if (lane == 0) probs[n * (T + 1) + T] = expf(-carry);
}

constexpr int kMaxAux = 4;

__global__ void composite_fwd_kernel(const float* __restrict__ rays, int64_t ray_stride,
                                     const float* __restrict__ ts, const float* __restrict__ t_min,
                                     const float* __restrict__ t_max,
                                     const uint8_t* __restrict__ mask,
                                     const float* __restrict__ density,
                                     const float* __restrict__ rgb, const float* __restrict__ aux,
                                     int n_aux, const float* __restrict__ background,
                                     int64_t n_rays, int T, float* __restrict__ outputs,
                                     float* __restrict__ alphas, float* __restrict__ coords,
                                     float* __restrict__ aux_sum, const float* __restrict__ targets,
                                     int64_t target_stride, float* __restrict__ sq_err) {
  __shared__ float s_err[16];
  const int lane = threadIdx.x & 63;
  const int wave = threadIdx.x >> 6;
  const int64_t n = (int64_t)blockIdx.x * (blockDim.x >> 6) + wave;
  const bool live = n < n_rays;
  float err = 0.0f;
  if (live) {
    const float* ts_row = ts + n * T;
    const float* de_row = density + n * T;
    const float tmin = t_min[n], tmax = t_max[n];
    const bool m = mask[n] != 0;
    float o[3] = {0, 0, 0}, d[3] = {0, 0, 0};
    if (rays) {
#pragma unroll
      for (int a = 0; a < 3; ++a) {
        o[a] = rays[n * ray_stride + a];
        d[a] = rays[n * ray_stride + 3 + a];
      }
    }
    float acc_c[3] = {0, 0, 0}, acc_x[3] = {0, 0, 0}, acc_a[kMaxAux] = {0, 0, 0, 0};
    float carry = 0.0f;
    for (int base = 0; base < T; base += 64) {
      const int i = base + lane;
      const Quad q = quad_chunk(ts_row, de_row, T, i, lane, tmin, tmax, carry);
      if (i < T) {
        const float p = expf(-q.prev) * (1.0f - expf(-q.a));
        const int64_t e = n * T + i;
#pragma unroll
        for (int c = 0; c < 3; ++c) {
          acc_c[c] += p * rgb[e * 3 + c];
          acc_x[c] += p * (o[c] + d[c] * q.t);
        }
        for (int k = 0; k < n_aux; ++k) acc_a[k] += p * aux[e * n_aux + k];
      }
      carry = __shfl(q.incl, 63, 64);
    }
    const float p_bg = expf(-carry);
    float out[3];
#pragma unroll
    for (int c = 0; c < 3; ++c) {
      const float bg = background[c];
      const float s = wave_sum(acc_c[c]) + p_bg * bg;
      out[c] = m ? s : bg;
      const float x = wave_sum(acc_x[c]);
      if (lane == 0) {
        if (outputs) outputs[n * 3 + c] = out[c];
        if (coords) coords[n * 3 + c] = m ? x : 0.0f;
      }
    }
    for (int k = 0; k < n_aux; ++k) {
      const float s = wave_sum(acc_a[k]);
      if (lane == 0 && aux_sum) aux_sum[n * n_aux + k] = m ? s : 0.0f;
    }
    if (lane == 0 && alphas) alphas[n] = m ? 1.0f - p_bg : 0.0f;
    if (targets && lane == 0) {
#pragma unroll
      for (int c = 0; c < 3; ++c) {
        const float df = out[c] - targets[n * target_stride + c];
        err += df * df;
      }
    }
  }
  if (sq_err && targets) {
    if (lane == 0) s_err[wave] = err;
    __syncthreads();
    if (threadIdx.x == 0) {
      float s = 0.0f;
      for (int w = 0; w < (int)(blockDim.x >> 6); ++w) s += s_err[w];
      atomicAdd(sq_err, s);
    }
  }
}

__global__ void composite_bwd_kernel(const float* __restrict__ ts, const float* __restrict__ t_min,
                                     const float* __restrict__ t_max,
                                     const uint8_t* __restrict__ mask,
                                     const float* __restrict__ density,
                                     const float* __restrict__ rgb, const float* __restrict__ aux,
                                     int n_aux, const float* __restrict__ background,
                                     int64_t n_rays, int T, const float* __restrict__ g_out,
                                     const float* __restrict__ outputs,
                                     const float* __restrict__ targets, int64_t target_stride,
                                     float out_scale, float gw0, float gw1, float gw2, float gw3,
                                     float* __restrict__ g_density, float* __restrict__ g_rgb,
                                     float* __restrict__ g_aux, float* __restrict__ g_background,
                                     float* __restrict__ bg_parts) {
  __shared__ float s_bg[16][3];
  const int lane = threadIdx.x & 63;
  const int wave = threadIdx.x >> 6;
  const int64_t n = (int64_t)blockIdx.x * (blockDim.x >> 6) + wave;
  const bool live = n < n_rays;
  const float gw[kMaxAux] = {gw0, gw1, gw2, gw3};
  float gbg[3] = {0, 0, 0};
  if (live) {
    const float* ts_row = ts + n * T;
    const float* de_row = density + n * T;
    const float tmin = t_min[n], tmax = t_max[n];
    const bool m = mask[n] != 0;
    float g[3];
#pragma unroll
    for (int c = 0; c < 3; ++c)
      g[c] = g_out ? g_out[n * 3 + c]
                   : out_scale * (outputs[n * 3 + c] - targets[n * target_stride + c]);
    if (!m) {
      for (int i = lane; i < T; i += 64) {
        const int64_t e = n * T + i;
        g_density[e] = 0.0f;
#pragma unroll
        for (int c = 0; c < 3; ++c) g_rgb[e * 3 + c] = 0.0f;
        for (int k = 0; k < n_aux; ++k) g_aux[e * n_aux + k] = 0.0f;
      }
#pragma unroll
      for (int c = 0; c < 3; ++c) gbg[c] = g[c];
    } else {
      float carry = 0.0f, f_part = 0.0f;
      for (int base = 0; base < T; base += 64) {
        const int i = base + lane;
        const Quad q = quad_chunk(ts_row, de_row, T, i, lane, tmin, tmax, carry);
        if (i < T) {
          const float p = expf(-q.prev) * (1.0f - expf(-q.a));
          const int64_t e = n * T + i;
          float w = 0.0f;
#pragma unroll
          for (int c = 0; c < 3; ++c) w += g[c] * rgb[e * 3 + c];
          for (int k = 0; k < n_aux; ++k) w += gw[k] * aux[e * n_aux + k];
          f_part += p * w;
        }
        carry = __shfl(q.incl, 63, 64);
      }
      const float p_bg = expf(-carry);
      float w_bg = 0.0f;
#pragma unroll
      for (int c = 0; c < 3; ++c) w_bg += g[c] * background[c];
      const float F = wave_sum(f_part) + p_bg * w_bg;
      carry = 0.0f;
      float pw_carry = 0.0f;
      for (int base = 0; base < T; base += 64) {
        const int i = base + lane;
        const Quad q = quad_chunk(ts_row, de_row, T, i, lane, tmin, tmax, carry);
        const bool valid = i < T;
        const int64_t e = n * T + (valid ? i : T - 1);
        float p = 0.0f, w = 0.0f;
        if (valid) {
          p = expf(-q.prev) * (1.0f - expf(-q.a));
#pragma unroll
          for (int c = 0; c < 3; ++c) w += g[c] * rgb[e * 3 + c];
          for (int k = 0; k < n_aux; ++k) w += gw[k] * aux[e * n_aux + k];
        }
        const float pw_incl = wave_incl_scan(p * w, lane) + pw_carry;
        if (valid) {
          const float s_next = expf(-q.incl);
          const float rest = F - pw_incl;
          const float t_p = i > 0 ? ts_row[i - 1] : 0.0f;
          const float start = i == 0 ? tmin : (q.t + t_p) / 2.0f;
          const float dl = q.end - start;
          g_density[e] = dl * (s_next * w - rest);
#pragma unroll
          for (int c = 0; c < 3; ++c) g_rgb[e * 3 + c] = p * g[c];
          for (int k = 0; k < n_aux; ++k) g_aux[e * n_aux + k] = p * gw[k];
        }
        carry = __shfl(q.incl, 63, 64);
        pw_carry = __shfl(pw_incl, 63, 64);
      }
#pragma unroll
      for (int c = 0; c < 3; ++c) gbg[c] = p_bg * g[c];
    }
  }
  if (g_background) {
    if (lane == 0) {
#pragma unroll
      for (int c = 0; c < 3; ++c) s_bg[wave][c] = gbg[c];
    }
    __syncthreads();
    if (threadIdx.x < 3) {
      float s = 0.0f;
      for (int w = 0; w < (int)(blockDim.x >> 6); ++w) s += s_bg[w][threadIdx.x];
      bg_parts[(int64_t)blockIdx.x * 4 + threadIdx.x] = s;
    }
  }
}

__global__ __launch_bounds__(256) void composite_bg_fold_kernel(const float* __restrict__ parts, int n_blocks,
                                                                float* __restrict__ g_background) {
  __shared__ float red[256][3];
  float s[3] = {0.0f, 0.0f, 0.0f};
  for (int b = threadIdx.x; b < n_blocks; b += 256) {
    const float4 v = *reinterpret_cast<const float4*>(parts + (int64_t)b * 4);
    s[0] += v.x; s[1] += v.y; s[2] += v.z;
  }
#pragma unroll
  for (int c = 0; c < 3; ++c) red[threadIdx.x][c] = s[c];
  __syncthreads();
  for (int half = 128; half > 0; half >>= 1) {
    if ((int)threadIdx.x < half) {
#pragma unroll
      for (int c = 0; c < 3; ++c) red[threadIdx.x][c] += red[threadIdx.x + half][c];
    }
    __syncthreads();
  }
  if (threadIdx.x < 3) atomicAdd(g_background + threadIdx.x, red[0][threadIdx.x]);
}

struct Dist {
  float w, m, d, delta;
  float incl;
  float w_ex, m_ex;
  float w_in, m_in;
};

struct DistCarry {
  float a, w, m;
};

__device__ __forceinline__ Dist dist_chunk(const float* __restrict__ ts_row, const float* __restrict__ dens_row,
                                           int T, int i, int lane, float tmin, float tmax, float r, DistCarry& c) {
  const Quad q = quad_chunk(ts_row, dens_row, T, i, lane, tmin, tmax, c.a);
  const bool valid = i < T;
  const int ic = valid ? i : T - 1;
  const float t_p = ic > 0 ? ts_row[ic - 1] : 0.0f;
  const float start = ic == 0 ? tmin : (q.t + t_p) / 2.0f;
  Dist s;
  s.delta = q.end - start;
  s.w = valid ? expf(-q.prev) * (1.0f - expf(-q.a)) : 0.0f;
  s.m = ((start + q.end) / 2.0f - tmin) / r;
  s.d = s.delta / r;
  s.incl = q.incl;
  s.w_in = wave_incl_scan(s.w, lane) + c.w;
  s.m_in = wave_incl_scan(s.w * s.m, lane) + c.m;
  const float w_up = __shfl_up(s.w_in, 1, 64), m_up = __shfl_up(s.m_in, 1, 64);
  s.w_ex = lane == 0 ? c.w : w_up;
  s.m_ex = lane == 0 ? c.m : m_up;
  c.a = __shfl(q.incl, 63, 64);
  c.w = __shfl(s.w_in, 63, 64);
  c.m = __shfl(s.m_in, 63, 64);
  return s;
}

__device__ __forceinline__ float dist_g(const Dist& s, float w_tot, float m_tot) {
  return 2.0f * (s.m * s.w_ex - s.m_ex + (m_tot - s.m_in) - s.m * (w_tot - s.w_in)) + (2.0f / 3.0f) * s.w * s.d;
}

__device__ __forceinline__ float dist_accumulate(float g, float grad_scale, float v) {
#pragma clang fp contract(off)
  const float x = grad_scale * v;
  return g + x;
}

__global__ __launch_bounds__(256) void distortion_kernel(const float* __restrict__ ts, const float* __restrict__ t_min,
                                                         const float* __restrict__ t_max,
                                                         const uint8_t* __restrict__ mask,
                                                         const float* __restrict__ density, int64_t n_rays, int T,
                                                         float grad_scale, float* __restrict__ loss,
                                                         float* __restrict__ g_density) {
  const int lane = threadIdx.x & 63;
  const int64_t n = (int64_t)blockIdx.x * (blockDim.x >> 6) + (threadIdx.x >> 6);
  if (n >= n_rays) return;
  const float tmin = t_min[n], tmax = t_max[n];
  const float r = tmax - tmin;
  if (mask[n] == 0 || !(r > 0.0f) || !(r <= 3.402823466e38f)) {
    if (loss && lane == 0) loss[n] = 0.0f;
    return;
  }
  const float* ts_row = ts + n * T;
  const float* de_row = density + n * T;
  DistCarry c = {0.0f, 0.0f, 0.0f};
  float l_part = 0.0f;
  for (int base = 0; base < T; base += 64) {
    const Dist s = dist_chunk(ts_row, de_row, T, base + lane, lane, tmin, tmax, r, c);
    l_part += 2.0f * s.w * (s.m * s.w_ex - s.m_ex) + (1.0f / 3.0f) * s.w * s.w * s.d;
  }
  const float w_tot = c.w, m_tot = c.m;
  const float l = wave_sum(l_part);
  if (loss && lane == 0) loss[n] = l;
  if (!g_density) return;
  c = {0.0f, 0.0f, 0.0f};
  float gw_part = 0.0f;
  for (int base = 0; base < T; base += 64) {
    const Dist s = dist_chunk(ts_row, de_row, T, base + lane, lane, tmin, tmax, r, c);
    gw_part += dist_g(s, w_tot, m_tot) * s.w;
  }
  const float gamma = wave_sum(gw_part);
  c = {0.0f, 0.0f, 0.0f};
  float gw_carry = 0.0f;
  for (int base = 0; base < T; base += 64) {
    const int i = base + lane;
    const Dist s = dist_chunk(ts_row, de_row, T, i, lane, tmin, tmax, r, c);
    const float gk = dist_g(s, w_tot, m_tot);
    const float gw_incl = wave_incl_scan(gk * s.w, lane) + gw_carry;
    if (i < T) {
      const float v = s.delta * (gk * expf(-s.incl) - (gamma - gw_incl));
      const int64_t e = n * T + i;
      g_density[e] = dist_accumulate(g_density[e], grad_scale, v);
    }
    gw_carry = __shfl(gw_incl, 63, 64);
  }
}

__global__ void fine_sample_kernel(const float* __restrict__ ts_c, const float* __restrict__ t_min,
                                   const float* __restrict__ t_max,
                                   const float* __restrict__ density_c, int64_t n_rays, int tc,
                                   int tf, float eps, int combine, const float* __restrict__ u,
                                   uint64_t seed, uint32_t stream_id, int64_t ray_offset,
                                   float* __restrict__ ts_out) {
  extern __shared__ __attribute__((aligned(16))) float smem[];
  const int lane = threadIdx.x & 63;
  const int wave = threadIdx.x >> 6;
  const int per_wave = 2 * (tc + 1) + tc + tf;
  float* xs = smem + (size_t)wave * per_wave;
  float* ys = xs + (tc + 1);
  float* comb = ys + (tc + 1);
  int64_t n = (int64_t)blockIdx.x * (blockDim.x >> 6) + wave;
  const bool live = n < n_rays;
  if (!live) n = n_rays - 1;
  const float* ts_row = ts_c + n * tc;
  const float* de_row = density_c + n * tc;
  const float tmin = t_min[n], tmax = t_max[n];

  float carry = 0.0f, wcarry = 0.0f;
  for (int base = 0; base < tc; base += 64) {
    const int i = base + lane;
    const Quad q = quad_chunk(ts_row, de_row, tc, i, lane, tmin, tmax, carry);
    const float p = expf(-q.prev) * (1.0f - expf(-q.a));
    const float w = i < tc ? p + eps : 0.0f;
    const float wincl = wave_incl_scan(w, lane) + wcarry;
    if (i < tc) {
      xs[i + 1] = wincl;
      ys[i + 1] = q.end;
      comb[i] = q.t;
    }
    carry = __shfl(q.incl, 63, 64);
    wcarry = __shfl(wincl, 63, 64);
  }
  if (lane == 0) {
    xs[0] = 0.0f;
    ys[0] = tmin;
  }
  __syncthreads();
  const float total = xs[tc];
  __syncthreads();
  for (int i = lane; i <= tc; i += 64) xs[i] = xs[i] / total;
  __syncthreads();

  const float bin = (1.0f - 0.0f) / (float)tf;
  for (int j = lane; j < tf; j += 64) {
    const float uu = u ? u[n * tf + j] : philox_uniform(seed, stream_id, (uint64_t)(ray_offset + n) * tf + j);
    const float x = ((float)j * bin + 0.0f) + uu * bin;
    int lo = 0, hi = tc + 1;
    while (lo < hi) {
      const int mid = (lo + hi) >> 1;
      if (xs[mid] <= x) lo = mid + 1; else hi = mid;
    }
    int idx = lo < 1 ? 1 : (lo > tc ? tc : lo);
    const float x0 = xs[idx - 1], x1 = xs[idx], y0 = ys[idx - 1], y1 = ys[idx];
// ... 61 lines not shown
#pragma unroll
    for (int a = 0; a < 6; ++a) rays[e * 6 + a] = ray[a];
  }
}

__global__ void gather_rows_kernel(const float* __restrict__ src, int64_t n_src, int row_floats,
                                   const int32_t* __restrict__ idx, int64_t n, float* __restrict__ out) {
  const int64_t total = n * row_floats;
  for (int64_t e = (int64_t)blockIdx.x * blockDim.x + threadIdx.x; e < total;
       e += (int64_t)gridDim.x * blockDim.x) {
    const int64_t i = e / row_floats;
    const int f = (int)(e - i * row_floats);
    const int64_t r = idx[i];
    out[e] = (r >= 0 && r < n_src) ? src[r * row_floats + f] : 0.0f;
  }
}

}

using namespace lnrf;

static inline int grid_for(int64_t total, int block, int cap = 2048 * 8) {
  int64_t g = (total + block - 1) / block;
  if (g < 1) g = 1;
  if (g > cap) g = cap;
  return (int)g;
}

extern "C" int lnrf_ray_aabb_stratified(const float* rays, int64_t ray_stride, int64_t n_rays,
                                        const float* bbox_min, const float* bbox_max,
                                        float min_t_range, float epsilon, int32_t count,
                                        const float* u, uint64_t seed, uint32_t stream_id,
                                        int64_t ray_offset, float* t_min, float* t_max,
                                        uint8_t* mask, float* ts, lnrf_stream_t stream) {
  if (n_rays == 0) return LNRF_OK;
  LNRF_CHECK_ARG(rays && bbox_min && bbox_max, "null rays/bbox");
  LNRF_CHECK_ARG(n_rays >= 0 && count >= 0 && ray_stride >= 6, "bad sizes");
  LNRF_CHECK_ARG(count == 0 || ts, "ts is NULL with count > 0");
  if (n_rays == 0) return LNRF_OK;
  BBox bb;
  for (int a = 0; a < 3; ++a) {
    bb.mn[a] = bbox_min[a];
    bb.mx[a] = bbox_max[a];
  }
  const int64_t total = n_rays * (count > 0 ? count : 1);
  hipLaunchKernelGGL(ray_aabb_stratified_kernel, dim3(grid_for(total, 256)), dim3(256), 0,
                     as_stream(stream), rays, ray_stride, n_rays, bb, min_t_range, epsilon, count, u,
                     seed, stream_id, ray_offset, t_min, t_max, mask, ts);
  LNRF_LAUNCH_CHECK();
  return LNRF_OK;
}

extern "C" int lnrf_stratified(const float* t_min, const float* t_max, int64_t n_rays,
                               int32_t count, const float* u, uint64_t seed, uint32_t stream_id,
                               int64_t ray_offset, float* ts, lnrf_stream_t stream) {
  if (n_rays == 0 || count == 0) return LNRF_OK;
  LNRF_CHECK_ARG(t_min && t_max, "null t range");
  LNRF_CHECK_ARG(n_rays >= 0 && count >= 0, "bad sizes");
  if (n_rays == 0 || count == 0) return LNRF_OK;
  LNRF_CHECK_ARG(ts, "null ts");
  hipLaunchKernelGGL(stratified_kernel, dim3(grid_for(n_rays * count, 256)), dim3(256), 0,
                     as_stream(stream), t_min, t_max, n_rays, count, u, seed, stream_id, ray_offset, ts);
  LNRF_LAUNCH_CHECK();
  return LNRF_OK;
}

extern "C" int lnrf_ray_points(const float* rays, int64_t ray_stride, const float* ts,
                               int64_t n_rays, int32_t t, float* points, float* dirs,
                               lnrf_stream_t stream) {
  if (n_rays == 0 || t == 0) return LNRF_OK;
  LNRF_CHECK_ARG(rays && ts, "null rays/ts");
  LNRF_CHECK_ARG(n_rays >= 0 && t >= 0 && ray_stride >= 6, "bad sizes");
  if (n_rays == 0 || t == 0) return LNRF_OK;
  hipLaunchKernelGGL(ray_points_kernel, dim3(grid_for(n_rays * t, 256)), dim3(256), 0,
                     as_stream(stream), rays, ray_stride, ts, n_rays, t, points, dirs);
  LNRF_LAUNCH_CHECK();
  return LNRF_OK;
}

extern "C" int lnrf_termination_probs(const float* ts, const float* t_min, const float* t_max,
                                      const float* density, int64_t n_rays, int32_t t,
                                      float* probs, lnrf_stream_t stream) {
  if (n_rays == 0) return LNRF_OK;
  LNRF_CHECK_ARG(ts && t_min && t_max && density && probs, "null pointer");
  LNRF_CHECK_ARG(n_rays >= 0 && t >= 1, "bad sizes");
  if (n_rays == 0) return LNRF_OK;
  const int wpb = 4;
  hipLaunchKernelGGL(termination_probs_kernel, dim3((unsigned)((n_rays + wpb - 1) / wpb)),
                     dim3(wpb * 64), 0, as_stream(stream), ts, t_min, t_max, density, n_rays, t, probs);
  LNRF_LAUNCH_CHECK();
  return LNRF_OK;
}

extern "C" int lnrf_composite_fwd(const float* rays, int64_t ray_stride, const float* ts,
                                  const float* t_min, const float* t_max, const uint8_t* mask,
                                  const float* density, const float* rgb, const float* aux,
                                  int32_t n_aux, const float* background, int64_t n_rays, int32_t t,
                                  float* outputs, float* alphas, float* coords, float* aux_sum,
                                  const float* targets, int64_t target_stride, float* sq_err,
                                  lnrf_stream_t stream) {
  if (n_rays == 0) return LNRF_OK;
  LNRF_CHECK_ARG(ts && t_min && t_max && mask && density && rgb && background, "null pointer");
  LNRF_CHECK_ARG(n_rays >= 0 && t >= 1, "bad sizes");
  LNRF_CHECK_ARG(n_aux >= 0 && n_aux <= kMaxAux && (n_aux == 0 || aux), "bad aux");
  LNRF_CHECK_ARG(!coords || rays, "coords needs rays");
  if (n_rays == 0) return LNRF_OK;
  const int wpb = (sq_err && targets) ? 16 : 4;
  hipLaunchKernelGGL(composite_fwd_kernel, dim3((unsigned)((n_rays + wpb - 1) / wpb)),
                     dim3(wpb * 64), 0, as_stream(stream), rays, ray_stride, ts, t_min, t_max, mask,
                     density, rgb, aux, n_aux, background, n_rays, t, outputs, alphas, coords,
                     aux_sum, targets, target_stride, sq_err);
  LNRF_LAUNCH_CHECK();
  return LNRF_OK;
}

extern "C" int64_t lnrf_composite_bwd_scratch_bytes(int64_t n_rays) {
  return n_rays < 0 ? -1 : ((n_rays + 3) / 4) * 4 * (int64_t)sizeof(float) + 16;
}

extern "C" int lnrf_composite_bwd_det(const float* ts, const float* t_min, const float* t_max,
                                      const uint8_t* mask, const float* density, const float* rgb,
                                      const float* aux, int32_t n_aux, const float* background,
                                      int64_t n_rays, int32_t t, const float* g_out,
                                      const float* outputs, const float* targets,
                                      int64_t target_stride, float out_scale, const float* g_aux_w,
                                      float* g_density, float* g_rgb, float* g_aux,
                                      float* g_background, void* scratch, int64_t scratch_bytes, lnrf_stream_t stream) {
  if (n_rays == 0) return LNRF_OK;
  if (n_rays > 0 && g_background)
    LNRF_CHECK_ARG(scratch && scratch_bytes >= lnrf_composite_bwd_scratch_bytes(n_rays) &&
                       (reinterpret_cast<uintptr_t>(scratch) & 15u) == 0, "scratch too small or unaligned");
  LNRF_CHECK_ARG(ts && t_min && t_max && mask && density && rgb && background, "null pointer");
  LNRF_CHECK_ARG(g_density && g_rgb, "null gradient outputs");
  LNRF_CHECK_ARG(g_out || (outputs && targets), "need g_out or outputs+targets");
  LNRF_CHECK_ARG(n_rays >= 0 && t >= 1, "bad sizes");
  LNRF_CHECK_ARG(n_aux >= 0 && n_aux <= kMaxAux && (n_aux == 0 || (aux && g_aux && g_aux_w)), "bad aux");
  float gw[kMaxAux] = {0, 0, 0, 0};
  for (int k = 0; k < n_aux; ++k) gw[k] = g_aux_w[k];
  float* bg_parts = g_background ? reinterpret_cast<float*>(scratch) : nullptr;
  const int wpb = 4;
  hipLaunchKernelGGL(composite_bwd_kernel, dim3((unsigned)((n_rays + wpb - 1) / wpb)),
                     dim3(wpb * 64), 0, as_stream(stream), ts, t_min, t_max, mask, density, rgb, aux,
                     n_aux, background, n_rays, t, g_out, outputs, targets, target_stride, out_scale,
                     gw[0], gw[1], gw[2], gw[3], g_density, g_rgb, g_aux, g_background, bg_parts);
  LNRF_LAUNCH_CHECK();
  if (g_background) {
    hipLaunchKernelGGL(composite_bg_fold_kernel, dim3(1), dim3(256), 0, as_stream(stream), bg_parts,
                       (int)((n_rays + wpb - 1) / wpb), g_background);
    LNRF_LAUNCH_CHECK();
  }
  return LNRF_OK;
}

extern "C" int lnrf_distortion(const float* ts, const float* t_min, const float* t_max, const uint8_t* mask,
                               const float* density, int64_t n_rays, int32_t t, float grad_scale, float* loss,
                               float* g_density, lnrf_stream_t stream) {
  LNRF_CHECK_ARG(n_rays >= 0 && t >= 1, "bad sizes");
  LNRF_CHECK_ARG(loss || g_density, "both outputs are NULL");
  if (n_rays == 0) return LNRF_OK;
  LNRF_CHECK_ARG(ts && t_min && t_max && mask && density, "null pointer");
  const int wpb = 4;
  hipLaunchKernelGGL(distortion_kernel, dim3((unsigned)((n_rays + wpb - 1) / wpb)), dim3(wpb * 64), 0,
                     as_stream(stream), ts, t_min, t_max, mask, density, n_rays, (int)t, grad_scale, loss, g_density);
  LNRF_LAUNCH_CHECK();
  return LNRF_OK;
}

extern "C" int lnrf_fine_sample(const float* ts_c, const float* t_min, const float* t_max,
                                const float* density_c, int64_t n_rays, int32_t tc, int32_t tf,
                                float eps, int32_t combine, const float* u, uint64_t seed,
                                uint32_t stream_id, int64_t ray_offset, float* ts_out,
                                lnrf_stream_t stream) {
  if (n_rays == 0) return LNRF_OK;
  LNRF_CHECK_ARG(ts_c && t_min && t_max && density_c && ts_out, "null pointer");
  LNRF_CHECK_ARG(n_rays >= 0 && tc >= 1 && tf >= 0, "bad sizes");
  if (n_rays == 0) return LNRF_OK;
  if (tf == 0 && !combine) return LNRF_OK;
  const int wpb = 4;
  const size_t lds = (size_t)wpb * (2 * (tc + 1) + tc + tf) * sizeof(float);
  LNRF_CHECK_ARG(lds <= 160 * 1024, "tc+tf too large for LDS");
  hipLaunchKernelGGL(fine_sample_kernel, dim3((unsigned)((n_rays + wpb - 1) / wpb)), dim3(wpb * 64),
                     lds, as_stream(stream), ts_c, t_min, t_max, density_c, n_rays, tc, tf, eps,
                     combine, u, seed, stream_id, ray_offset, ts_out);
  LNRF_LAUNCH_CHECK();
  return LNRF_OK;
}

extern "C" int lnrf_bin_edges(const float* ts, const float* t_min, const float* t_max, int64_t n_rays,
                              int32_t t, float* starts, float* ends, lnrf_stream_t stream) {
  if (n_rays == 0 || t == 0) return LNRF_OK;
  LNRF_CHECK_ARG(ts && t_min && t_max, "null pointer");
  LNRF_CHECK_ARG(n_rays >= 0 && t >= 0, "bad sizes");
  if (n_rays == 0 || t == 0) return LNRF_OK;
  hipLaunchKernelGGL(bin_edges_kernel, dim3(grid_for(n_rays * t, 256)), dim3(256), 0, as_stream(stream), ts,
                     t_min, t_max, n_rays, t, starts, ends);
  LNRF_LAUNCH_CHECK();
  return LNRF_OK;
}

extern "C" int lnrf_gather_rows(const float* src, int64_t n_src, int32_t row_floats, const int32_t* idx, int64_t n,
                                float* out, lnrf_stream_t stream) {
  LNRF_CHECK_ARG(n >= 0 && n_src >= 0 && row_floats >= 1, "bad sizes");
  if (n == 0) return LNRF_OK;
  LNRF_CHECK_ARG(src && idx && out, "null pointer");
  hipLaunchKernelGGL(gather_rows_kernel, dim3(grid_for(n * row_floats, 256)), dim3(256), 0, as_stream(stream), src,
                     n_src, (int)row_floats, idx, n, out);
  LNRF_LAUNCH_CHECK();
  return LNRF_OK;
}

extern "C" int lnrf_camera_rays(const float* origin, const float* x_axis, const float* y_axis, const float* z_axis,
                                float x_fov, float y_fov, int32_t width, int32_t height, float* rays,
                                lnrf_stream_t stream) {
  LNRF_CHECK_ARG(origin && x_axis && y_axis && z_axis && rays, "null pointer");
  LNRF_CHECK_ARG(width >= 1 && height >= 1, "bad image size");
  const Camera cam = make_camera(origin, x_axis, y_axis, z_axis, x_fov, y_fov);
  hipLaunchKernelGGL(camera_rays_kernel, dim3(grid_for((int64_t)width * height, 256)), dim3(256), 0,
                     as_stream(stream), cam, (int)width, (int)height, rays);
  LNRF_LAUNCH_CHECK();
  return LNRF_OK;
}
```

learn-nerf_amd/learn_nerf/_lib.py:

```python
import ctypes
import os
from ctypes import POINTER, c_char_p, c_float, c_int32, c_int64, c_uint8, c_uint32, c_uint64, c_void_p

import torch

_HERE = os.path.dirname(os.path.abspath(__file__))
_DEFAULT = os.path.normpath(os.path.join(_HERE, "..", "lib", "liblnrf.so"))

ERR_UNSUPPORTED = -3
ACT_NONE, ACT_RELU, ACT_SOFTPLUS, ACT_TANH, ACT_EXP, ACT_SIGMOID = range(6)


class HashGridDesc(ctypes.Structure):
    _fields_ = [("n_levels", c_int32), ("feature_dim", c_int32), ("smooth", c_int32), ("pad_", c_int32),
                ("bbox_min", c_float * 3), ("bbox_max", c_float * 3), ("grid_size", c_int32 * 32),
                ("table_size", c_int32 * 32), ("table_offset", c_int64 * 32), ("hashed", c_int32 * 32)]


class NerfShape(ctypes.Structure):
    _fields_ = [(n, c_int32) for n in
                ("input_layers", "mid_layers", "hidden_dim", "color_layer_dim", "x_freqs", "d_freqs")]


FUSED_NERF_SHAPE = NerfShape(5, 4, 256, 128, 10, 4)


class NgpMlpDesc(ctypes.Structure):
    _fields_ = [("enc_dim", c_int32), ("hidden_dim", c_int32), ("density_dim", c_int32),
                ("density_layers", c_int32), ("color_layers", c_int32), ("d_freqs", c_int32),
                ("dense_offset", c_int64)]


class PcGrid(ctypes.Structure):
    _fields_ = [("lo", c_float * 3), ("h", c_float), ("dims", c_int32 * 3), ("pad_", c_int32)]


class RtBvh(ctypes.Structure):
    _fields_ = [("center", c_float * 3), ("radius", c_float), ("half", c_float * 3), ("n_tris", c_int32),
                ("leaf_size", c_int32), ("pad_", c_int32)]


_P = c_void_p
_F3 = POINTER(c_float)

PROTOTYPES = {
    "lnrf_version": (c_int32, []),
    "lnrf_last_error": (c_char_p, []),
    "lnrf_ray_aabb_stratified": (c_int32, [_P, c_int64, c_int64, _F3, _F3, c_float, c_float, c_int32, _P,
                                           c_uint64, c_uint32, c_int64, _P, _P, _P, _P, _P]),
    "lnrf_camera_rays": (c_int32, [_F3, _F3, _F3, _F3, c_float, c_float, c_int32, c_int32, _P, _P]),
    "lnrf_gather_rows": (c_int32, [_P, c_int64, c_int32, _P, c_int64, _P, _P]),
    "lnrf_stratified": (c_int32, [_P, _P, c_int64, c_int32, _P, c_uint64, c_uint32, c_int64, _P, _P]),
    "lnrf_ray_points": (c_int32, [_P, c_int64, _P, c_int64, c_int32, _P, _P, _P]),
    "lnrf_fine_sample": (c_int32, [_P, _P, _P, _P, c_int64, c_int32, c_int32, c_float, c_int32, _P,
                                   c_uint64, c_uint32, c_int64, _P, _P]),
    "lnrf_bin_edges": (c_int32, [_P, _P, _P, c_int64, c_int32, _P, _P, _P]),
    "lnrf_termination_probs": (c_int32, [_P, _P, _P, _P, c_int64, c_int32, _P, _P]),
    "lnrf_composite_fwd": (c_int32, [_P, c_int64, _P, _P, _P, _P, _P, _P, _P, c_int32, _P, c_int64, c_int32,
                                     _P, _P, _P, _P, _P, c_int64, _P, _P]),
    "lnrf_composite_bwd_scratch_bytes": (c_int64, [c_int64]),
    "lnrf_composite_bwd_det": (c_int32, [_P, _P, _P, _P, _P, _P, _P, c_int32, _P, c_int64, c_int32, _P, _P, _P,
                                         c_int64, c_float, _F3, _P, _P, _P, _P, _P, c_int64, _P]),
    "lnrf_distortion": (c_int32, [_P, _P, _P, _P, _P, c_int64, c_int32, c_float, _P, _P, _P]),
    "lnrf_sinusoidal_emb": (c_int32, [_P, c_int64, c_int64, c_int32, c_int32, _P, c_int64, c_int64, _P]),
    "lnrf_dense_fwd": (c_int32, [_P, c_int64, _P, _P, c_int32, _P, c_int64, c_int64, c_int32, c_int32, _P]),
    "lnrf_act_bwd": (c_int32, [_P, c_int64, _P, c_int64, c_int32, c_int64, c_int32, _P]),
    "lnrf_dense_bwd_input": (c_int32, [_P, c_int64, _P, _P, c_int64, c_int32, c_int64, c_int32, c_int32, _P]),
    "lnrf_gemm_f32_det_scratch_bytes": (c_int64, [c_int64, c_int32, c_int64]),
    "lnrf_gemm_f32_det": (c_int32, [_P, c_int64, c_int64, _P, c_int64, c_int64, _P, c_int64, c_int32, c_int64, _P, c_int64, _P]),
    "lnrf_dense_bwd_weight_scratch_bytes": (c_int64, [c_int64, c_int32, c_int32]),
    "lnrf_dense_bwd_weight_det": (c_int32, [_P, c_int64, _P, c_int64, _P, _P, c_int64, c_int32, c_int32, _P, c_int64, _P]),
    "lnrf_gemm_f32": (c_int32, [_P, c_int64, c_int64, _P, c_int64, c_int64, _P, c_int64, _P, c_int32, c_int32,
                                c_int64, c_int32, c_int64, c_int32, _P]),
    "lnrf_hashgrid_fwd": (c_int32, [POINTER(HashGridDesc), _P, _P, c_int64, _P, _P]),
    "lnrf_hashgrid_bwd_scratch_bytes": (c_int64, [POINTER(HashGridDesc), c_int64]),
    "lnrf_hashgrid_bwd_bucketed": (c_int32, [POINTER(HashGridDesc), _P, _P, c_int64, _P, _P, _P, _P, c_int64, _P]),
    "lnrf_hashgrid_jvp": (c_int32, [POINTER(HashGridDesc), _P, _P, _P, c_int64, _P, _P]),
    "lnrf_hashgrid_input_grad": (c_int32, [POINTER(HashGridDesc), _P, _P, c_int64, _P, _P, _P]),
    "lnrf_hashgrid_bwd_dir": (c_int32, [POINTER(HashGridDesc), _P, _P, c_int64, _P, _P, _P]),
    "lnrf_sinusoidal_emb_bwd": (c_int32, [_P, c_int64, c_int64, c_int32, c_int32, _P, c_int64, c_int64, _P, _P]),
    "lnrf_sinusoidal_emb_jvp": (c_int32, [_P, c_int64, c_int64, c_int32, c_int32, _P, _P, c_int64, c_int64, _P]),
    "lnrf_integrated_directional_encoding": (c_int32, [c_int32, _P, _P, c_int64, _P, _P]),
    "lnrf_refnerf_head_fwd": (c_int32, [_P, c_int64, _P, _P, c_int64, c_int32, _P, _P, _P, _P, c_int64, _P, _P]),
    "lnrf_refnerf_head_bwd": (c_int32, [_P, c_int64, _P, _P, c_int64, c_int32, _P, _P, _P, _P, c_int64, _P, _P,
                                        c_int64, _P, _P]),
    "lnrf_refnerf_color_fwd": (c_int32, [_P, _P, _P, c_int64, _P, _P]),
    "lnrf_refnerf_color_bwd": (c_int32, [_P, _P, _P, c_int64, _P, _P, _P, _P, _P]),
    "lnrf_refnerf_trunk_packed_bytes": (c_int64, []),
    "lnrf_refnerf_trunk_pack": (c_int32, [_P, _P, _P]),
    "lnrf_refnerf_trunk_fwd": (c_int32, [_P, _P, c_int64, _P, _P, c_int64, _P]),
    "lnrf_refnerf_normal_pass": (c_int32, [_P, _P, _P, c_int64, _P, _P, _P]),
    "lnrf_refnerf_trunk_bwd_scratch_bytes": (c_int64, [c_int64]),
    "lnrf_refnerf_trunk_bwd": (c_int32, [_P, _P, _P, c_int64, c_int64, _P, _P, _P]),
    "lnrf_refnerf_normal_bwd": (c_int32, [_P, _P, _P, _P, _P, c_int64, _P, _P, _P]),
    "lnrf_refnerf_dir_save_bytes": (c_int64, [c_int64]),
    "lnrf_refnerf_dir_scratch_bytes": (c_int64, [c_int64]),
    "lnrf_refnerf_dir_fwd": (c_int32, [_P, _P, c_int64, c_int64, _P, _P, _P]),
    "lnrf_refnerf_dir_bwd": (c_int32, [_P, _P, _P, c_int64, _P, _P, c_int64, _P, _P]),
    "lnrf_refnerf_render_packed_bytes": (c_int64, []),
    "lnrf_refnerf_render_pack": (c_int32, [_P, _P, _P]),
    "lnrf_refnerf_trunk_normal_split_scratch_bytes": (c_int64, [c_int64]),
    "lnrf_refnerf_trunk_normal_split": (c_int32, [_P, _P, c_int64, _P, c_int64, _P, _P, _P]),
    "lnrf_refnerf_dir_fwd_split": (c_int32, [_P, _P, c_int64, c_int64, _P, _P]),
    "lnrf_nerf_param_count": (c_int64, [POINTER(NerfShape)]),
    "lnrf_nerf_packed_bytes": (c_int64, [POINTER(NerfShape)]),
    "lnrf_nerf_save_bytes": (c_int64, [POINTER(NerfShape), c_int64]),
    "lnrf_nerf_bwd_scratch_bytes": (c_int64, [POINTER(NerfShape), c_int64]),
    "lnrf_nerf_pack_weights": (c_int32, [POINTER(NerfShape), _P, _P, _P]),
    "lnrf_nerf_mlp_fwd": (c_int32, [POINTER(NerfShape), _P, _P, _P, _P, c_int64, _P, c_int32, c_int64, _P, _P,
                                    _P, _P]),
    "lnrf_nerf_mlp_fwd_ls": (c_int32, [POINTER(NerfShape), _P, _P, _P, _P, c_int64, _P, c_int32, c_int64, _P, _P,
                                       _P, _P]),
    "lnrf_nerf_packed_split_bytes": (c_int64, [POINTER(NerfShape)]),
    "lnrf_nerf_pack_weights_split": (c_int32, [POINTER(NerfShape), _P, _P, _P]),
    "lnrf_nerf_mlp_fwd_split": (c_int32, [POINTER(NerfShape), _P, _P, _P, _P, c_int64, _P, c_int32, c_int64, _P, _P,
                                          _P]),
    "lnrf_nerf_mlp_bwd_chain": (c_int32, [POINTER(NerfShape), _P, _P, _P, _P, _P, _P, c_int64, _P, _P]),
    "lnrf_nerf_mlp_bwd_weights": (c_int32, [POINTER(NerfShape), _P, _P, c_int64, _P, _P]),
    "lnrf_nerf_bwd_ls_scratch_bytes": (c_int64, [POINTER(NerfShape), c_int64]),
    "lnrf_nerf_bwd_ls_status_offset": (c_int64, [POINTER(NerfShape), c_int64]),
    "lnrf_nerf_mlp_bwd_ls": (c_int32, [POINTER(NerfShape), _P, _P, _P, _P, _P, _P, c_int64, _P, _P, c_int32, _P]),
    "lnrf_nerf_mlp_bwd_ls2": (c_int32, [POINTER(NerfShape), _P, _P, _P, _P, _P, _P, c_int64, _P, _P,
                                        _P, _P, _P, _P, _P, _P, c_int64, _P, _P, c_int32, _P]),
    "lnrf_ngp_mlp_packed_bytes": (c_int64, [POINTER(NgpMlpDesc)]),
    "lnrf_ngp_mlp_scratch_bytes": (c_int64, [POINTER(NgpMlpDesc), c_int64]),
    "lnrf_ngp_mlp_pack": (c_int32, [POINTER(NgpMlpDesc), _P, _P, _P]),
    "lnrf_ngp_mlp_fwd": (c_int32, [POINTER(NgpMlpDesc), _P, _P, _P, c_int64, _P, _P, _P]),
    "lnrf_ngp_mlp_packed_split_bytes": (c_int64, [POINTER(NgpMlpDesc)]),
    "lnrf_ngp_mlp_pack_split": (c_int32, [POINTER(NgpMlpDesc), _P, _P, _P]),
    "lnrf_ngp_mlp_fwd_split": (c_int32, [POINTER(NgpMlpDesc), _P, _P, _P, c_int64, _P, _P, _P]),
    "lnrf_ngp_mlp_bwd": (c_int32, [POINTER(NgpMlpDesc), _P, _P, _P, _P, _P, c_int64, _P, _P, _P, _P, _P]),
    "lnrf_dense_bwd_input_gated": (c_int32, [_P, c_int64, _P, _P, c_int64, c_int32, c_int32, _P, c_int64, c_int32,
                                             c_int64, c_int32, c_int32, _P]),
    "lnrf_dense_fwd_gated": (c_int32, [_P, c_int64, _P, _P, c_int32, _P, c_int64, c_int32, _P, c_int64, c_int64,
                                       c_int32, c_int32, _P]),
    "lnrf_set_dense_precision": (c_int32, [c_int32]),
    "lnrf_get_dense_precision": (c_int32, []),
    "lnrf_comm_get_unique_id": (c_int32, [_P]),
    "lnrf_comm_init": (c_int32, [_P, c_int32, c_int32, POINTER(c_void_p)]),
    "lnrf_comm_allreduce": (c_int32, [_P, _P, c_int64, _P]),
    "lnrf_comm_info": (c_int32, [_P, POINTER(c_int32), POINTER(c_int32)]),
    "lnrf_comm_destroy": (c_int32, [_P]),
    "lnrf_adam_step": (c_int32, [_P, _P, _P, _P, c_int64, c_float, c_float, c_float, c_float, c_int32,
                                 c_float, _P]),
    "lnrf_adam_step_norms": (c_int32, [_P, _P, _P, _P, c_int64, c_float, c_float, c_float, c_float, c_int32,
                                       c_float, _P, _P]),
    "lnrf_step_log": (c_int32, [_P, c_float, c_float, c_int32, _P, _P]),
    "lnrf_sq_norm": (c_int32, [_P, c_int64, _P, _P]),
    "lnrf_mc_scratch_bytes": (c_int64, [c_int64, c_int64, c_int64]),
    "lnrf_mc_count": (c_int32, [_P, c_int64, c_int64, c_int64, c_float, _P, _P, _P]),
    "lnrf_mc_emit": (c_int32, [_P, c_int64, c_int64, c_int64, c_float, _P, c_int64, c_int64, _P, _P, _P]),
    "lnrf_mc_case_table": (c_int32, [_P]),
    "lnrf_pc_cell_ids": (c_int32, [POINTER(PcGrid), _P, c_int64, _P, _P]),
    "lnrf_pc_knn_dist2": (c_int32, [POINTER(PcGrid), _P, _P, c_int64, _P, c_int64, c_int32, _P, _P]),
    "lnrf_pc_nearest": (c_int32, [POINTER(PcGrid), _P, _P, _P, c_int64, _P, c_int64, c_float, _P, _P, _P]),
    "lnrf_rt_node_count": (c_int64, [c_int64, c_int32]),
    "lnrf_rt_morton": (c_int32, [POINTER(RtBvh), _P, _P, _P]),
    "lnrf_rt_fit": (c_int32, [POINTER(RtBvh), _P, _P, _P]),
    "lnrf_rt_closest": (c_int32, [POINTER(RtBvh), _P, _P, _P, _P, _P, c_int64, _P, _P, _P]),
    "lnrf_rt_occluded": (c_int32, [POINTER(RtBvh), _P, _P, _P, _P, c_int64, _P, _P]),
    "lnrf_sq_err_scratch_bytes": (c_int64, [c_int64]),
    "lnrf_sq_err_f64": (c_int32, [_P, _P, c_int64, c_int64, _P, _P, _P, c_int64, _P]),
    "lnrf_view_miss_scratch_bytes": (c_int64, [c_int32, c_int32]),
    "lnrf_view_miss_stats": (c_int32, [_F3, _F3, _F3, _F3, c_float, c_float, c_int32, c_int32, _P, _F3, _F3, c_float,
                                       c_float, _P, _P, _P, c_int64, _P]),
    "lnrf_ssim_scratch_bytes": (c_int64, [c_int32, c_int32]),
    "lnrf_ssim_f64": (c_int32, [_P, _P, c_int32, c_int32, _P, _P, _P, c_int64, _P]),
    "lnrf_occ_scratch_bytes": (c_int64, [c_int32]),
    "lnrf_occ_build": (c_int32, [_P, c_int32, c_float, c_int32, _P, _P, _P, c_int64, _P]),
    "lnrf_occ_clip_rays": (c_int32, [_P, c_int64, c_int64, _F3, _F3, _P, c_int32, c_float, c_float, _P, _P, _P, _P,
                                     _P, _P, _P]),
    "lnrf_compact_mask": (c_int32, [_P, c_int64, _P, _P, _P]),
    "lnrf_scatter_rows": (c_int32, [_P, c_int32, _P, c_int64, _P, c_int64, _P]),
    "lnrf_cc_max_rounds": (c_int32, []),
    "lnrf_cc_scratch_bytes": (c_int64, [c_int64, c_int64, c_int64]),
    "lnrf_cc_local": (c_int32, [_P, c_int64, c_int64, c_int64, c_int32, _P, _P, c_int64, _P]),
    "lnrf_cc_merge_round": (c_int32, [c_int64, c_int64, c_int64, c_int32, c_int32, _P, _P, _P, c_int64, _P]),
    "lnrf_cc_sizes": (c_int32, [_P, c_int64, _P, _P]),
    "lnrf_cc_keep": (c_int32, [_P, _P, c_int64, c_int32, c_int32, c_int32, _P, _P]),
}

_lib = None


def library_path() -> str:
    return os.environ.get("LNRF_LIB", _DEFAULT)


def lib() -> ctypes.CDLL:
    global _lib
    if _lib is None:
        path = library_path()
        if not os.path.exists(path):
            raise RuntimeError(
                f"liblnrf.so not found at {path}: build it with `python -c 'import __graft_entry__ as g; "
                f"g.build()'` (or `make -C learn-nerf_amd/csrc`). The HIP library is required."
            )
        handle = ctypes.CDLL(path)
        for name, (res, args) in PROTOTYPES.items():
            fn = getattr(handle, name)
            fn.restype = res
            fn.argtypes = args
        _lib = handle
    return _lib


def check(rc: int, what: str = "") -> None:
    if rc != 0:
        msg = lib().lnrf_last_error()
        raise RuntimeError(f"lnrf error {rc} {what}: {msg.decode() if msg else ''}")


def ptr(t, dtype=torch.float32):
    if t is None:
        return None
# ... 20 lines not shown
```

learn-nerf_amd/learn_nerf/ops.py:

```python
import contextlib
import ctypes
import functools
from typing import Optional, Sequence, Tuple

import torch

from . import _lib as L
from . import _ws

F32 = torch.float32


def _dev(t: torch.Tensor):
    return t.device


def _ray_stride(rays: torch.Tensor) -> int:
    assert rays.dim() == 3 and rays.shape[2] == 3 and rays.shape[1] in (2, 3), rays.shape
    return rays.shape[1] * 3


def _seed(seed) -> int:
    return int(seed) & 0xFFFFFFFFFFFFFFFF

# ... 74 lines not shown
        raise ValueError("occ_clip_rays: bitfield size does not match the resolution")
    lo = torch.empty(n, dtype=F32, device=dev)
    hi = torch.empty(n, dtype=F32, device=dev)
    out_mask = torch.empty(n, dtype=torch.uint8, device=dev)
    L.check(L.lib().lnrf_occ_clip_rays(
        L.ptr(rays), _ray_stride(rays), n, L.f3(bbox_min), L.f3(bbox_max), L.ptr(bits, torch.int32), int(resolution),
        min_t_range, epsilon, L.ptr(t_min), L.ptr(t_max), L.ptr(mask, torch.uint8), L.ptr(lo), L.ptr(hi),
        L.ptr(out_mask, torch.uint8), L.stream()), "occ_clip_rays")
    return lo, hi, out_mask


def _cc_scratch(shape) -> int:
    nx, ny, nz = (int(s) for s in shape)
    if min(nx, ny, nz) < 1:
        raise ValueError(f"connected components: every dimension must be at least 1, got {(nx, ny, nz)}")
    nbytes = L.lib().lnrf_cc_scratch_bytes(nx, ny, nz)
    if nbytes < 0:
        raise ValueError(f"connected components: {(nx, ny, nz)} has more than 2^31 - 1 cells")
    return nbytes


def cc_local(mask: torch.Tensor, connectivity: int) -> Tuple[torch.Tensor, torch.Tensor]:
    if mask.dim() != 3:
        raise ValueError(f"expected a 3-d mask, got shape {tuple(mask.shape)}")
    nx, ny, nz = mask.shape
    nbytes = _cc_scratch(mask.shape)
    labels = torch.empty(mask.shape, dtype=torch.int32, device=_dev(mask))
    scratch = torch.empty(nbytes, dtype=torch.uint8, device=_dev(mask))
    L.check(L.lib().lnrf_cc_local(L.ptr(mask, torch.uint8), nx, ny, nz, int(connectivity), L.ptr(labels, torch.int32),
                                  L.ptr(scratch, torch.uint8), nbytes, L.stream()), "cc_local")
    return labels, scratch


def cc_merge_round(labels: torch.Tensor, scratch: torch.Tensor, changed: torch.Tensor, connectivity: int,
                   round_index: int) -> None:
    nx, ny, nz = labels.shape
    L.check(L.lib().lnrf_cc_merge_round(nx, ny, nz, int(connectivity), int(round_index), L.ptr(labels, torch.int32),
                                        L.ptr(changed, torch.int32), L.ptr(scratch, torch.uint8), scratch.numel(),
                                        L.stream()), "cc_merge_round")


def cc_sizes(labels: torch.Tensor) -> torch.Tensor:
    sizes = torch.empty_like(labels)
    L.check(L.lib().lnrf_cc_sizes(L.ptr(labels, torch.int32), labels.numel(), L.ptr(sizes, torch.int32), L.stream()),
            "cc_sizes")
    return sizes


def cc_keep(labels: torch.Tensor, sizes: torch.Tensor, min_cells: int, cut_size: int, cut_label: int) -> torch.Tensor:
    keep = torch.empty(labels.shape, dtype=torch.uint8, device=_dev(labels))
    L.check(L.lib().lnrf_cc_keep(L.ptr(labels, torch.int32), L.ptr(sizes, torch.int32), labels.numel(),
                                 int(min_cells), int(cut_size), int(cut_label), L.ptr(keep, torch.uint8), L.stream()),
            "cc_keep")
    return keep


def stratified(t_min, t_max, count: int, u=None, seed: int = 0, stream_id: int = 0, ray_offset: int = 0):
    n = t_min.shape[0]
    ts = torch.empty((n, count), dtype=F32, device=_dev(t_min))
    L.check(L.lib().lnrf_stratified(L.ptr(t_min), L.ptr(t_max), n, count, L.ptr(u), _seed(seed), stream_id,
                                    ray_offset, L.ptr(ts) if count > 0 else None, L.stream()), "stratified")
    return ts


def ray_points(rays, ts, want_dirs: bool = True):
    n, t = ts.shape
    pts = torch.empty((n, t, 3), dtype=F32, device=_dev(ts))
    dirs = torch.empty((n, t, 3), dtype=F32, device=_dev(ts)) if want_dirs else None
    L.check(L.lib().lnrf_ray_points(L.ptr(rays), _ray_stride(rays), L.ptr(ts), n, t, L.ptr(pts), L.ptr(dirs),
                                    L.stream()), "ray_points")
    return pts, dirs


def fine_sample(ts_c, t_min, t_max, density_c, count: int, u=None, seed: int = 0, stream_id: int = 1,
                ray_offset: int = 0, combine: bool = True, eps: float = 1e-8):
    n, tc = ts_c.shape
    width = tc + count if combine else count
    out = torch.empty((n, width), dtype=F32, device=_dev(ts_c))
    if width == 0:
        return out
    if u is not None:
        assert u.shape == (n, count)
    L.check(L.lib().lnrf_fine_sample(L.ptr(ts_c), L.ptr(t_min), L.ptr(t_max), L.ptr(density_c), n, tc, count,
                                     eps, 1 if combine else 0, L.ptr(u), _seed(seed), stream_id, ray_offset,
                                     L.ptr(out), L.stream()), "fine_sample")
    return out


def bin_edges(ts, t_min, t_max):
    n, t = ts.shape
    starts = torch.empty((n, t), dtype=F32, device=_dev(ts))
    ends = torch.empty((n, t), dtype=F32, device=_dev(ts))
    L.check(L.lib().lnrf_bin_edges(L.ptr(ts), L.ptr(t_min), L.ptr(t_max), n, t, L.ptr(starts), L.ptr(ends),
                                   L.stream()), "bin_edges")
    return starts, ends


def termination_probs(ts, t_min, t_max, density):
    n, t = ts.shape
    probs = torch.empty((n, t + 1), dtype=F32, device=_dev(ts))
    L.check(L.lib().lnrf_termination_probs(L.ptr(ts), L.ptr(t_min), L.ptr(t_max), L.ptr(density), n, t,
                                           L.ptr(probs), L.stream()), "termination_probs")
    return probs


def composite_fwd(rays, ts, t_min, t_max, mask, density, rgb, background, aux=None, targets=None,
                  sq_err=None, want_coords: bool = True):
    n, t = ts.shape
    dev = _dev(ts)
    n_aux = 0 if aux is None else aux.shape[-1]
    outputs = torch.empty((n, 3), dtype=F32, device=dev)
    alphas = torch.empty(n, dtype=F32, device=dev)
    coords = torch.empty((n, 3), dtype=F32, device=dev) if (want_coords and rays is not None) else None
    aux_sum = torch.empty((n, n_aux), dtype=F32, device=dev) if n_aux else None
    tstride = 0
    tptr = None
    if targets is not None:
        assert targets.shape == (n, 3) and targets.stride(1) == 1
        tstride = targets.stride(0)
        tptr = L.c_void_p(targets.data_ptr())
    L.check(L.lib().lnrf_composite_fwd(
        L.ptr(rays) if rays is not None else None, _ray_stride(rays) if rays is not None else 6, L.ptr(ts),
        L.ptr(t_min), L.ptr(t_max), L.ptr(mask, torch.uint8), L.ptr(density), L.ptr(rgb), L.ptr(aux), n_aux,
        L.ptr(background), n, t, L.ptr(outputs), L.ptr(alphas), L.ptr(coords), L.ptr(aux_sum), tptr, tstride,
        L.ptr(sq_err), L.stream()), "composite_fwd")
    return outputs, alphas, coords, aux_sum


def composite_bwd(ts, t_min, t_max, mask, density, rgb, background, g_background, g_out=None, outputs=None,
                  targets=None, out_scale: float = 0.0, aux=None, g_aux_w: Sequence[float] = ()):
    n, t = ts.shape
    dev = _dev(ts)
    n_aux = 0 if aux is None else aux.shape[-1]
    g_density = torch.empty((n, t), dtype=F32, device=dev)
    g_rgb = torch.empty((n, t, 3), dtype=F32, device=dev)
    g_aux = torch.empty((n, t, n_aux), dtype=F32, device=dev) if n_aux else None
    tstride, tptr = 0, None
    if targets is not None:
        assert targets.shape == (n, 3) and targets.stride(1) == 1
        tstride = targets.stride(0)
        tptr = L.c_void_p(targets.data_ptr())
    gw = (L.c_float * 4)(*([float(x) for x in g_aux_w] + [0.0] * (4 - len(g_aux_w))))
    nbytes = L.lib().lnrf_composite_bwd_scratch_bytes(n)
    lease = _ws.lease("composite_bwd", nbytes, dev)
    L.check(L.lib().lnrf_composite_bwd_det(
        L.ptr(ts), L.ptr(t_min), L.ptr(t_max), L.ptr(mask, torch.uint8), L.ptr(density), L.ptr(rgb),
        L.ptr(aux), n_aux, L.ptr(background), n, t, L.ptr(g_out), L.ptr(outputs), tptr, tstride,
        float(out_scale), gw, L.ptr(g_density), L.ptr(g_rgb), L.ptr(g_aux), L.ptr(g_background),
        L.ptr(lease.buf, torch.uint8), nbytes, L.stream()), "composite_bwd_det")
    lease.release()
    return g_density, g_rgb, g_aux


def distortion(ts, t_min, t_max, mask, density, g_density=None, grad_scale: float = 0.0, want_loss: bool = True):
    n, t = ts.shape
    assert want_loss or g_density is not None
    assert density.shape == (n, t) and (g_density is None or g_density.shape == (n, t))
    loss = torch.empty(n, dtype=F32, device=_dev(ts)) if want_loss else None
    L.check(L.lib().lnrf_distortion(L.ptr(ts), L.ptr(t_min), L.ptr(t_max), L.ptr(mask, torch.uint8), L.ptr(density),
                                    n, t, float(grad_scale), L.ptr(loss), L.ptr(g_density), L.stream()), "distortion")
    return loss



_DENSE_PRECISIONS = {"fp32": 0, "bf16": 1}


@contextlib.contextmanager
def dense_precision(precision: str):
    if precision not in _DENSE_PRECISIONS:
        raise ValueError(f"unknown precision {precision!r}")
    lib = L.lib()
    previous = lib.lnrf_get_dense_precision()
    L.check(lib.lnrf_set_dense_precision(_DENSE_PRECISIONS[precision]), "set_dense_precision")
    try:
        yield
    finally:
        lib.lnrf_set_dense_precision(previous)


def uses_model_precision(method):
    @functools.wraps(method)
    def wrapped(self, *args, **kwargs):
        with dense_precision(getattr(self, "precision", "fp32")):
            return method(self, *args, **kwargs)
    return wrapped


def _ld(t: torch.Tensor) -> int:
    assert t.dim() == 2 and t.stride(1) == 1, "need a row-major 2-D view"
    return t.stride(0)


def _vptr(t: torch.Tensor):
    assert t.is_cuda and t.dtype == F32
    return L.c_void_p(t.data_ptr())


def sinusoidal_emb_into(x: torch.Tensor, freqs: int, out: torch.Tensor, col_off: int = 0):
    m, dims = x.shape
    L.check(L.lib().lnrf_sinusoidal_emb(_vptr(x), _ld(x), m, dims, freqs, _vptr(out), _ld(out), col_off,
                                        L.stream()), "sinusoidal_emb")
    return out


def dense_fwd(x: torch.Tensor, w: torch.Tensor, b: Optional[torch.Tensor], act: int,
              out: Optional[torch.Tensor] = None, gate: Optional[torch.Tensor] = None,
              gate_act: int = L.ACT_RELU) -> torch.Tensor:
    m, k = x.shape
    k2, n = w.shape
    assert k == k2 and w.is_contiguous()
    if out is None:
        out = torch.empty((m, n), dtype=F32, device=_dev(x))
    if gate is None:
        L.check(L.lib().lnrf_dense_fwd(_vptr(x), _ld(x), L.ptr(w), L.ptr(b), act, _vptr(out), _ld(out), m, k, n,
                                       L.stream()), "dense_fwd")
    else:
        assert gate.shape == (m, n)
        L.check(L.lib().lnrf_dense_fwd_gated(_vptr(x), _ld(x), L.ptr(w), L.ptr(b), act, _vptr(gate), _ld(gate),
                                             gate_act, _vptr(out), _ld(out), m, k, n, L.stream()), "dense_fwd_gated")
    return out


def act_bwd_(g: torch.Tensor, y: torch.Tensor, act: int) -> torch.Tensor:
    m, n = g.shape
    L.check(L.lib().lnrf_act_bwd(_vptr(g), _ld(g), _vptr(y), _ld(y), act, m, n, L.stream()), "act_bwd")
    return g


def dense_bwd_input(gy: torch.Tensor, w: torch.Tensor, out: Optional[torch.Tensor] = None,
                    accumulate: bool = False, gate: Optional[torch.Tensor] = None,
                    gate_act: int = L.ACT_RELU) -> torch.Tensor:
    m, n = gy.shape
    k, n2 = w.shape
    assert n == n2
    if out is None:
        out = torch.empty((m, k), dtype=F32, device=_dev(gy))
        accumulate = False
    if gate is None:
        L.check(L.lib().lnrf_dense_bwd_input(_vptr(gy), _ld(gy), L.ptr(w), _vptr(out), _ld(out),
                                             1 if accumulate else 0, m, k, n, L.stream()), "dense_bwd_input")
    else:
        assert gate.shape[0] == m and gate.shape[1] <= k
        L.check(L.lib().lnrf_dense_bwd_input_gated(_vptr(gy), _ld(gy), L.ptr(w), _vptr(gate), _ld(gate), gate_act,
                                                   gate.shape[1], _vptr(out), _ld(out), 1 if accumulate else 0, m,
                                                   k, n, L.stream()), "dense_bwd_input_gated")
    return out


def dense_bwd_weight(x: torch.Tensor, gy: torch.Tensor, gw: torch.Tensor, gb: Optional[torch.Tensor]):
    m, k = x.shape
    m2, n = gy.shape
    assert m == m2 and gw.shape == (k, n) and gw.is_contiguous()
    nbytes = L.lib().lnrf_dense_bwd_weight_scratch_bytes(m, k, n)
    lease = _ws.lease("dense_wgrad", nbytes, _dev(x))
    L.check(L.lib().lnrf_dense_bwd_weight_det(_vptr(x), _ld(x), _vptr(gy), _ld(gy), L.ptr(gw), L.ptr(gb), m, k, n,
                                              L.ptr(lease.buf, torch.uint8), nbytes, L.stream()), "dense_bwd_weight_det")
    lease.release()


def bias_grad(gy: torch.Tensor, gb: torch.Tensor):
    m, n = gy.shape
    nbytes = L.lib().lnrf_dense_bwd_weight_scratch_bytes(m, 0, n)
    lease = _ws.lease("dense_wgrad", nbytes, _dev(gy))
    L.check(L.lib().lnrf_dense_bwd_weight_det(None, 0, _vptr(gy), _ld(gy), None, L.ptr(gb), m, 0, n,
                                              L.ptr(lease.buf, torch.uint8), nbytes, L.stream()), "bias_grad")
    lease.release()


def gemm(a: torch.Tensor, sa_i: int, sa_r: int, b: torch.Tensor, sb_r: int, sb_j: int, c: torch.Tensor, ldc: int,
         i_rows: int, j_cols: int, r_depth: int, bias=None, act: int = 0, mode: int = 0, splits: int = 0):
    if mode == 2 and ldc == j_cols and bias is None and splits == 0:
        nbytes = L.lib().lnrf_gemm_f32_det_scratch_bytes(i_rows, j_cols, r_depth)
        lease = _ws.lease("gemm_det", nbytes, _dev(a))
        L.check(L.lib().lnrf_gemm_f32_det(_vptr(a), sa_i, sa_r, _vptr(b), sb_r, sb_j, _vptr(c), i_rows, j_cols, r_depth,
                                          L.ptr(lease.buf, torch.uint8), nbytes, L.stream()), "gemm_f32_det")
        lease.release()
        return c
    L.check(L.lib().lnrf_gemm_f32(_vptr(a), sa_i, sa_r, _vptr(b), sb_r, sb_j, _vptr(c), ldc, L.ptr(bias), act, mode,
                                  i_rows, j_cols, r_depth, splits, L.stream()), "gemm_f32")
    return c


def hashgrid_fwd(desc, tables: torch.Tensor, x: torch.Tensor) -> torch.Tensor:
    m = x.shape[0]
    enc_t = torch.empty((desc.n_levels * desc.feature_dim, m), dtype=F32, device=_dev(x))
    L.check(L.lib().lnrf_hashgrid_fwd(ctypes.byref(desc), L.ptr(tables), L.ptr(x), m, L.ptr(enc_t), L.stream()),
            "hashgrid_fwd")
    return enc_t


def hashgrid_jvp(desc, tables: torch.Tensor, x: torch.Tensor, u: torch.Tensor) -> torch.Tensor:
    m = x.shape[0]
    out = torch.empty((desc.n_levels * desc.feature_dim, m), dtype=F32, device=_dev(x))
    L.check(L.lib().lnrf_hashgrid_jvp(ctypes.byref(desc), L.ptr(tables), L.ptr(x), L.ptr(u), m, L.ptr(out),
                                      L.stream()), "hashgrid_jvp")
    return out


def hashgrid_input_grad(desc, tables: torch.Tensor, x: torch.Tensor, g_enc_t: torch.Tensor) -> torch.Tensor:
    m = x.shape[0]
    g_x = torch.empty((m, 3), dtype=F32, device=_dev(x))
    L.check(L.lib().lnrf_hashgrid_input_grad(ctypes.byref(desc), L.ptr(tables), L.ptr(x), m, L.ptr(g_enc_t),
                                             L.ptr(g_x), L.stream()), "hashgrid_input_grad")
    return g_x

# ... 175 lines not shown
```

learn-nerf_amd/learn_nerf/train.py:

```python
import os
from dataclasses import dataclass
from typing import Any, Callable, Dict, Optional, Sequence

import numpy as np
import torch

from . import _prof
from . import ops
from . import parallel
from .model import ModelBase
from .params import ParamTree, as_generator, build_tree, default_device, split_seed
from .render import STREAM_COARSE, STREAM_FINE, NeRFRenderer, _vec3
from .rng import Key, KeyLike, Uniforms, as_key, sampler_args, split

F32 = torch.float32


def _dist():
    import torch.distributed as dist

    return dist if (dist.is_available() and dist.is_initialized()) else None


@dataclass
# ... 25 lines not shown
        distortion_weight: Optional[float] = None,
    ):
        self.coarse = coarse
        self.fine = fine
        if hasattr(coarse, "tag") and hasattr(fine, "tag") and coarse is not fine:
            coarse.tag, fine.tag = "coarse", "fine"
        self.coarse_ts = coarse_ts
        self.fine_ts = fine_ts
        self.lr, self.adam_b1, self.adam_b2, self.adam_eps = lr, adam_b1, adam_b2, adam_eps
        self.loss_weights = loss_weights if loss_weights is not None else default_loss_weights()
        self.density_penalty = density_penalty
        self.density_penalty_batch_size = density_penalty_batch_size
        self.distortion_weight = distortion_weight
        self.device = device if device is not None else default_device()

        seed = as_generator(init_rng).initial_seed()
        coarse_seed, fine_seed = split_seed(seed, 2)
        self.n_coarse, self.n_fine = coarse.num_params(), fine.num_params()
        total = self.n_coarse + self.n_fine + 3
        host = torch.zeros(total, dtype=F32)
        coarse.init_flat_(host[: self.n_coarse], as_generator(coarse_seed))
        fine.init_flat_(host[self.n_coarse: self.n_coarse + self.n_fine], as_generator(fine_seed))
        host[-3:] = -1.0
        self.flat = host.to(self.device)
        self.grad = torch.zeros_like(self.flat)
        self.state = TrainState(params=self._views(self.flat), step=0, opt_m=torch.zeros_like(self.flat),
                                opt_v=torch.zeros_like(self.flat))
        self._scalars = torch.zeros(8, dtype=F32, device=self.device)
        self._scalars_dirty = False
        env = os.environ.get("LNRF_OVERLAP_BACKWARD")
        want = (env != "0") if env is not None else bool(getattr(coarse, "overlap_backward_hint", True))
        self.overlap_backward = torch.device(self.device).type == "cuda" and coarse is not fine and want
        self._side_stream = None
        self._early_reduce = (0, None)

    def _params_changed(self):
        for mdl in (self.coarse, self.fine):
            if hasattr(mdl, "invalidate_packed"):
                mdl.invalidate_packed()

    def _slices(self, flat):
        a, b = self.n_coarse, self.n_coarse + self.n_fine
        return flat[:a], flat[a:b], flat[b:b + 3]

    def _views(self, flat) -> Dict[str, Any]:
        c, f, bg = self._slices(flat)
        return dict(coarse=self.coarse.tree(c), fine=self.fine.tree(f), background=bg)

    def save(self, path: str):
        tmp_path = path + ".tmp"
        c, f, bg = self._slices(self.flat)
        arrays = {"format": np.array("lnrf-params-v3"), "background": bg.detach().cpu().numpy(),
                  "opt/step": np.array(self.state.step, dtype=np.int64),
                  "opt/m": self.state.opt_m.detach().cpu().numpy(), "opt/v": self.state.opt_v.detach().cpu().numpy()}
        for name in ("coarse", "fine"):
            for key, leaf in _flatten_tree(self.state.params[name]):
                arrays[f"{name}/{key}"] = leaf.detach().cpu().numpy()
        with open(tmp_path, "wb") as fh:
            np.savez(fh, **arrays)
        os.rename(tmp_path, path)

    def load(self, path: str, load_optimizer: bool = True):
        with np.load(path, allow_pickle=False) as blob:
            c, f, bg = self._slices(self.flat)
            for name, model, dst in (("coarse", self.coarse, c), ("fine", self.fine, f)):
                dst.copy_(_checkpoint_flat(blob, path, name, model).to(self.device))
            bg.copy_(torch.from_numpy(blob["background"]).to(F32).to(self.device))
            if load_optimizer and "opt/m" in blob and blob["opt/m"].shape[0] == self.flat.numel():
                self.state.opt_m.copy_(torch.from_numpy(blob["opt/m"]).to(self.device))
                self.state.opt_v.copy_(torch.from_numpy(blob["opt/v"]).to(self.device))
                self.state.step = int(blob["opt/step"])
        self._params_changed()

    def step_fn(self, bbox_min, bbox_max) -> Callable[[KeyLike, torch.Tensor], Dict[str, torch.Tensor]]:
        bmin, bmax = _vec3(bbox_min), _vec3(bbox_max)

        def in_place_step(key: KeyLike, batch: torch.Tensor) -> Dict[str, torch.Tensor]:
            return self._step(key, bmin, bmax, batch)

        return in_place_step

    def _forward_backward(self, key, bmin, bmax, batch, params_flat, grad_flat, want_grad: bool):
        n = batch.shape[0]
        dist = _dist()
        world = dist.get_world_size() if dist else 1
        c_flat, f_flat, bg = self._slices(params_flat)
        sc = self._scalars
        if self._scalars_dirty:
            sc.zero_()
        self._scalars_dirty = True
        render_key, density_key = split(key, 2)
        coarse_key, fine_key = split(render_key, 2)
        targets = batch[:, 2]

        t_min, t_max, mask, ts_c = ops.ray_aabb_stratified(batch, bmin, bmax, self.coarse_ts,
                                                           **sampler_args(coarse_key, STREAM_COARSE))
        dens_c, rgb_c, aux_c, ctx_c = self.coarse.forward_rays(c_flat, batch, ts_c, save=want_grad)
        names_c = list(aux_c.keys())
        auxs_c = torch.stack([aux_c[k] for k in names_c], -1).contiguous() if names_c else None
        out_c, _, _, asum_c = ops.composite_fwd(None, ts_c, t_min, t_max, mask, dens_c, rgb_c, bg, aux=auxs_c,
                                                targets=targets, sq_err=sc[0:1], want_coords=False)
        ts_f = ops.fine_sample(ts_c, t_min, t_max, dens_c, self.fine_ts, **sampler_args(fine_key, STREAM_FINE))

        inv = 1.0 / (3.0 * n)
        out_scale = 2.0 * inv
        gc, gf, gbg = self._slices(grad_flat) if want_grad else (None, None, None)

        dist_w = self.distortion_weight
        dist_rays = {}

        def output_grads(prefix, ts, dens, rgb, out, names, auxs):
            gw = [self.loss_weights[k] / n for k in names]
            gd, grgb, gaux = ops.composite_bwd(ts, t_min, t_max, mask, dens, rgb, bg, gbg, outputs=out,
                                               targets=targets, out_scale=out_scale, aux=auxs, g_aux_w=gw)
            if dist_w is not None:
                dist_rays[prefix] = ops.distortion(ts, t_min, t_max, mask, dens, g_density=gd if dist_w != 0.0 else None,
                                                   grad_scale=dist_w / n)
            g_aux = {k: gaux[..., i] for i, k in enumerate(names)} if names else None
            return gd, grgb, g_aux

        def backward_of(prefix, ts, dens, rgb, out, model, ctx, gslice, names, auxs):
            gd, grgb, g_aux = output_grads(prefix, ts, dens, rgb, out, names, auxs)
            model.backward(ctx, gd, grgb, g_aux, gslice)

        coarse_args = ("coarse", ts_c, dens_c, rgb_c, out_c, self.coarse, ctx_c, gc, names_c, auxs_c)
        coarse_done = None
        if want_grad and self.overlap_backward:
            if self._side_stream is None:
                self._side_stream = torch.cuda.Stream(device=self.device)
            main = torch.cuda.current_stream(self.device)
            ready = torch.cuda.Event()
            ready.record(main)
            with torch.cuda.stream(self._side_stream):
                self._side_stream.wait_event(ready)
                backward_of(*coarse_args)
                coarse_done = torch.cuda.Event()
                coarse_done.record(self._side_stream)
        dens_f, rgb_f, aux_f, ctx_f = self.fine.forward_rays(f_flat, batch, ts_f, save=want_grad)
        names_f = list(aux_f.keys())
        auxs_f = torch.stack([aux_f[k] for k in names_f], -1).contiguous() if names_f else None
        out_f, _, _, asum_f = ops.composite_fwd(None, ts_f, t_min, t_max, mask, dens_f, rgb_f, bg, aux=auxs_f,
                                                targets=targets, sq_err=sc[1:2], want_coords=False)

        loss_dict = {} if want_grad else dict(coarse=sc[0] * inv, fine=sc[1] * inv)
        for prefix, names, asum in (("coarse", names_c, asum_c), ("fine", names_f, asum_f)):
            if names:
                means = asum.mean(dim=0)
                for i, k in enumerate(names):
                    loss_dict[f"{prefix}_{k}"] = means[i]

        if want_grad and coarse_done is None and _ls_pair(self.coarse, ctx_c, self.fine, ctx_f):
            from .model import backward_ls_pair

            gd_c, grgb_c, _ = output_grads("coarse", ts_c, dens_c, rgb_c, out_c, names_c, auxs_c)
            gd_f, grgb_f, _ = output_grads("fine", ts_f, dens_f, rgb_f, out_f, names_f, auxs_f)
            backward_ls_pair(ctx_c, gd_c, grgb_c, gc, ctx_f, gd_f, grgb_f, gf)
        elif want_grad:
            if coarse_done is None:
                backward_of(*coarse_args)
                if self.density_penalty is None:
                    self._early_reduce = (self.n_coarse, parallel.begin_reduce_(gc))
            backward_of("fine", ts_f, dens_f, rgb_f, out_f, self.fine, ctx_f, gf, names_f, auxs_f)
            if coarse_done is not None:
                torch.cuda.current_stream(self.device).wait_event(coarse_done)

        if dist_w is not None:
            if not want_grad:
                dist_rays["coarse"] = ops.distortion(ts_c, t_min, t_max, mask, dens_c)
                dist_rays["fine"] = ops.distortion(ts_f, t_min, t_max, mask, dens_f)
            elif coarse_done is not None:
                dist_rays["coarse"].record_stream(torch.cuda.current_stream(self.device))
            for prefix in ("coarse", "fine"):
                loss_dict[f"{prefix}_distortion"] = dist_rays[prefix].mean()

        if self.density_penalty is not None:
            gsl = self._slices(grad_flat) if want_grad else (None, None, None)
            for prefix, model, pflat, gslice in (("fine", self.fine, f_flat, gsl[1]),
                                                 ("coarse", self.coarse, c_flat, gsl[0])):
                loss_dict[f"{prefix}_density"] = self._average_density(density_key, model, pflat, bmin, bmax,
                                                                       gslice if want_grad else None)
        return loss_dict, world

    def density_points(self, key, bmin, bmax):
        b = self.density_penalty_batch_size
        k = as_key(key)
        gen = torch.Generator(device=self.device)
        gen.manual_seed((k.seed if isinstance(k, Key) else 0) & 0x7FFFFFFFFFFFFFFF)
        lo = torch.tensor(bmin, dtype=F32, device=self.device)
        hi = torch.tensor(bmax, dtype=F32, device=self.device)
        coords = torch.rand((b, 3), generator=gen, device=self.device) * (hi - lo) + lo
        dirs = torch.randn((b, 3), generator=gen, device=self.device)
        dirs = dirs / dirs.norm(dim=-1, keepdim=True)
        return coords.contiguous(), dirs.contiguous()

    def _average_density(self, key, model, pflat, bmin, bmax, gslice):
        b = self.density_penalty_batch_size
        coords, dirs = self.density_points(key, bmin, bmax)
        dens, rgb, aux, ctx = model.forward_points(pflat, coords, dirs, save=gslice is not None)
        if gslice is not None:
            g_d = torch.full_like(dens, self.density_penalty / b)
            g_aux = {kk: torch.zeros_like(v) for kk, v in aux.items()} if aux else None
            model.backward(ctx, g_d, torch.zeros_like(rgb), g_aux, gslice)
        return dens.mean()

    def _step(self, key, bmin, bmax, batch):
        self.grad.zero_()
        self._early_reduce = (0, None)
        aux_losses, _ = self._forward_backward(key, bmin, bmax, batch.contiguous(), self.flat, self.grad, True)
        self.state.step += 1
        sc = self._scalars
        prefix, pending = self._early_reduce
        scale = apply_gradients(self.flat, self.grad, self.state.opt_m, self.state.opt_v, self.state.step, self.lr,
                                self.adam_b1, self.adam_b2, self.adam_eps, sq_norms=sc[2:4],
                                reduced_prefix=prefix, pending=pending)
        log = ops.step_log(sc, 1.0 / (3.0 * batch.shape[0]), scale, clear=True)
        self._scalars_dirty = False
        self._params_changed()
        loss_dict = dict(coarse=log[0], fine=log[1])
        loss_dict.update(aux_losses)
        loss_dict.update(grad_norm=log[2], param_norm=log[3])
        return loss_dict

    def losses(self, key: KeyLike, bbox_min, bbox_max, batch: torch.Tensor, params=None):
        flat = self.flat if params is None else self._flat_from_params(params)
        loss_dict, _ = self._forward_backward(key, _vec3(bbox_min), _vec3(bbox_max), batch.contiguous(), flat,
                                              None, False)
        total = loss_dict["coarse"] + loss_dict["fine"]
        for k, v in loss_dict.items():
            for prefix in ("coarse_", "fine_"):
                if k.startswith(prefix):
                    name = k[len(prefix):]
                    if name in self.loss_weights:
                        total = total + self.loss_weights[name] * v
                    elif name == "density" and self.density_penalty is not None:
                        total = total + self.density_penalty * v
                    elif name == "distortion" and self.distortion_weight is not None:
                        total = total + self.distortion_weight * v
        return total, loss_dict

    def _flat_from_params(self, params) -> torch.Tensor:
        if params is self.state.params:
            return self.flat
        return torch.cat([self.coarse.flat(params["coarse"]).reshape(-1), self.fine.flat(params["fine"]).reshape(-1),
                          torch.as_tensor(params["background"], dtype=F32, device=self.device).reshape(-1)])

    def average_density(self, key, model, params, bbox_min, bbox_max) -> torch.Tensor:
        return self._average_density(key, model, model.flat(params), _vec3(bbox_min), _vec3(bbox_max), None)


def _ls_pair(coarse, ctx_c, fine, ctx_f) -> bool:
    from .model import NeRFModel

    return all(type(mdl) is NeRFModel and mdl.backward_kernel == "ls" and isinstance(ctx, dict)
               and ctx.get("kind") == "fused" and ctx["m"] > 0 for mdl, ctx in ((coarse, ctx_c), (fine, ctx_f)))


def apply_gradients(flat, grad, opt_m, opt_v, step: int, lr: float, b1: float, b2: float, eps: float,
                    sq_norms: torch.Tensor, kernels=ops, reduced_prefix: int = 0, pending=None) -> float:
    with _prof.section("allreduce"):
        scale = parallel.reduce_gradient_(grad, reduced_prefix, pending)
    with _prof.section("norms_adam"):
        kernels.adam_step_(flat, grad, opt_m, opt_v, lr, b1, b2, eps, step, grad_scale=scale, sq_norms=sq_norms)
    return scale


def load_params(path: str, coarse: ModelBase, fine: ModelBase, device) -> Dict[str, Any]:
    out = {}
    with np.load(path, allow_pickle=False) as blob:
        for name, model in (("coarse", coarse), ("fine", fine)):
            out[name] = model.tree(_checkpoint_flat(blob, path, name, model).to(device))
        out["background"] = torch.from_numpy(blob["background"]).to(F32).to(device)
    return out


def _checkpoint_flat(blob, path: str, name: str, model: ModelBase) -> torch.Tensor:
    if str(blob["format"]) != "lnrf-params-v3":
        raise ValueError(f"{path}: not an lnrf-params-v3 checkpoint")
    return torch.cat([torch.from_numpy(blob[f"{name}/{module}/{leaf}"]).to(F32).reshape(-1)
                      for module, leaf, _ in model.param_spec()])


def _flatten_tree(tree, prefix=""):
    for k, v in tree.items():
        path = f"{prefix}/{k}" if prefix else k
        if isinstance(v, torch.Tensor):
            yield path, v
        else:
            yield from _flatten_tree(v, path)


def default_loss_weights() -> Dict[str, float]:
    return dict(normal_mse=3e-4, neg_normal=0.1)
```

Baseline: 186.9 million ray-samples/s.

## Fuse coarse/fine composite bwd and wgrad launches; table-driven weight packing

Coarse and fine composite backward passes now run in one paired kernel with a single background-gradient fold, instead of separate launches. The two models' weight-gradient kernels also run as one 2D-grid launch. Weight packing reads precomputed index tables cached on the device rather than computing the stream indices per element. The aim is fewer kernel launches and less index arithmetic, at the cost of more code paths, a per-device cached table, and possible idle blocks when the two models differ in tile count.

```diff
diff --git a/include/lnrf.h b/include/lnrf.h
--- a/include/lnrf.h
+++ b/include/lnrf.h
@@ -74,6 +74,15 @@
                            const float* targets, int64_t target_stride, float out_scale, const float* g_aux_w,
                            float* g_density, float* g_rgb, float* g_aux, float* g_background, void* scratch,
                            int64_t scratch_bytes, lnrf_stream_t stream);
+int lnrf_composite_bwd_det2(const float* t_min, const float* t_max, const uint8_t* mask, const float* background,
+                            int64_t n_rays, const float* targets, int64_t target_stride, float out_scale,
+                            const float* ts_a, const float* density_a, const float* rgb_a, const float* aux_a,
+                            int32_t n_aux_a, int32_t t_a, const float* g_out_a, const float* outputs_a,
+                            const float* g_aux_w_a, float* g_density_a, float* g_rgb_a, float* g_aux_a,
+                            const float* ts_b, const float* density_b, const float* rgb_b, const float* aux_b,
+                            int32_t n_aux_b, int32_t t_b, const float* g_out_b, const float* outputs_b,
+                            const float* g_aux_w_b, float* g_density_b, float* g_rgb_b, float* g_aux_b,
+                            float* g_background, void* scratch, int64_t scratch_bytes, lnrf_stream_t stream);
 
 int lnrf_distortion(const float* ts, const float* t_min, const float* t_max, const uint8_t* mask,
                     const float* density, int64_t n_rays, int32_t t, float grad_scale, float* loss,
diff --git a/learn-nerf_amd/csrc/layout_host.cpp b/learn-nerf_amd/csrc/layout_host.cpp
--- a/learn-nerf_amd/csrc/layout_host.cpp
+++ b/learn-nerf_amd/csrc/layout_host.cpp
@@ -112,6 +112,10 @@
   }
   return n;
 }
+int64_t lnrf_host_pack_table(int32_t* out) {
+  for (int64_t e = 0; out && e < kPackTableInts; ++e) out[e] = pack_table_entry(e);
+  return kPackTableInts;
+}
 int64_t lnrf_host_pack_offset(int what) {
   const int64_t v[17] = {kPackFwdOff, kPackBwdOff, kPackBiasOff, kPackBytes, kPack3BiasOff, kPack3Bytes,
                          kRefPackNrmOff, kRefPackDirFwdOff, kRefPackDirBwdOff, kRefPackDirBiasOff, kRefPackBytes,
diff --git a/learn-nerf_amd/csrc/nerf_bwd_ls.hip b/learn-nerf_amd/csrc/nerf_bwd_ls.hip
--- a/learn-nerf_amd/csrc/nerf_bwd_ls.hip
+++ b/learn-nerf_amd/csrc/nerf_bwd_ls.hip
@@ -567,14 +567,25 @@
   }
   if (!(phases & 4)) return LNRF_OK;
   LsFoldArgs fold;
+  const WgLayout lay{kSaveTileSlots, kGradTileSlots, 1};
+  const WgradList lists[2] = {wgrad_list_ls_finish(a.job[0].n_tiles), wgrad_list_ls_finish(a.job[1].n_tiles)};
+  if (n_models == 2) {
+    const void* xbuf[2] = {mdl[0].save, mdl[1].save};
+    const void* ybuf[2] = {mdl[0].scratch, mdl[1].scratch};
+    const int64_t nt[2] = {a.job[0].n_tiles, a.job[1].n_tiles};
+    float* slabs[2] = {ls_small_slabs(mdl[0].scratch, mdl[0].m), ls_small_slabs(mdl[1].scratch, mdl[1].m)};
+    rc = launch_nerf_wgrad_pair(lists, xbuf, ybuf, nt, slabs, st, lay);
+    if (rc) return rc;
+  }
   for (int k = 0; k < n_models; ++k) {
     const LsModel& md = mdl[k];
     const LsJob& j = a.job[k];
-    const WgradList w = wgrad_list_ls_finish(j.n_tiles);
+    const WgradList& w = lists[k];
     float* small_slabs = ls_small_slabs(md.scratch, md.m);
-    rc = launch_nerf_wgrad(w, md.save, md.scratch, j.n_tiles, md.grads, st, WgLayout{kSaveTileSlots, kGradTileSlots, 1},
-                           small_slabs, false, false);
-    if (rc) return rc;
+    if (n_models == 1) {
+      rc = launch_nerf_wgrad(w, md.save, md.scratch, j.n_tiles, md.grads, st, lay, small_slabs, false, false);
+      if (rc) return rc;
+    }
     fold.w[k] = w.args;
     fold.small_slabs[k] = small_slabs;
     fold.ls_slabs[k] = j.slabs;
diff --git a/learn-nerf_amd/csrc/nerf_chain.h b/learn-nerf_amd/csrc/nerf_chain.h
--- a/learn-nerf_amd/csrc/nerf_chain.h
+++ b/learn-nerf_amd/csrc/nerf_chain.h
@@ -153,6 +153,8 @@
 int launch_nerf_wgrad(const WgradList& list, const void* xbuf, const void* ybuf, int64_t n_tiles, float* grads,
                       hipStream_t stream, WgLayout lay, float* slabs, bool plain_loads = false,
                       bool fold = true);
+int launch_nerf_wgrad_pair(const WgradList* list, const void* const* xbuf, const void* const* ybuf, const int64_t* n_tiles,
+                           float* const* slabs, hipStream_t stream, WgLayout lay);
 
 int64_t ls_scratch_bytes(int64_t m);
 float* ls_small_slabs(void* scratch, int64_t m);
diff --git a/learn-nerf_amd/csrc/nerf_layout.h b/learn-nerf_amd/csrc/nerf_layout.h
--- a/learn-nerf_amd/csrc/nerf_layout.h
+++ b/learn-nerf_amd/csrc/nerf_layout.h
@@ -303,6 +303,20 @@
   for (int k = 1; k < kFwdLayers; ++k)
     if (i >= fwd_bias_base(k)) s = k;
   return ref && s > 8 ? -1 : fwd_bias_index(s, i - fwd_bias_base(s));
+}
+
+constexpr int64_t kPackUnits = (int64_t)(kFwdFrags + kBwdFrags) * 64;
+constexpr int64_t kPackTableInts = kPackUnits * 8 + kBiasFloats;
+static_assert(kPackFwdOff == 0 && kPackBwdOff == (int64_t)kFwdFrags * 64 * 16 && kPackBiasOff == kPackUnits * 16,
+              "the streams and the bias block are contiguous");
+NL_HD constexpr int pack_table_entry(int64_t e) {
+  if (e >= kPackUnits * 8) return bias_block_index((int)(e - kPackUnits * 8), false);
+  const int64_t u = e >> 3, units_f = (int64_t)kFwdFrags * 64;
+  const int j = (int)(e & 7);
+  const bool fwd = u < units_f;
+  const int64_t uu = fwd ? u : u - units_f;
+  const int g = (int)(uu >> 6), lane = (int)(uu & 63);
+  return fwd ? fwd_stream_index(g, lane, j, false) : bwd_stream_index(g, lane, j, false);
 }
 
 NL_HD constexpr int dump_lane_off(int slot, int c, int hh) {
diff --git a/learn-nerf_amd/csrc/nerf_mlp.hip b/learn-nerf_amd/csrc/nerf_mlp.hip
--- a/learn-nerf_amd/csrc/nerf_mlp.hip
+++ b/learn-nerf_amd/csrc/nerf_mlp.hip
@@ -1,3 +1,6 @@
+#include <mutex>
+#include <vector>
+
 #include "nerf_chain.h"
 
 namespace lnrf {
@@ -308,6 +311,34 @@
   }
 }
 
+struct Wgrad2Args {
+  WgradArgs args[2];
+  const char* save[2];
+  const char* gdump[2];
+  int64_t n_tiles[2];
+  float* slabs[2];
+  int blocks[2];
+};
+__global__ __launch_bounds__(kThreads) void nerf_wgrad2_kernel(Wgrad2Args a, WgLayout lay) {
+  const bool second = blockIdx.y != 0;
+  if ((int)blockIdx.x >= (second ? a.blocks[1] : a.blocks[0])) return;
+  const WgradArgs& args = second ? a.args[1] : a.args[0];
+  const char* save = second ? a.save[1] : a.save[0];
+  const char* gdump = second ? a.gdump[1] : a.gdump[0];
+  const int64_t n_tiles = second ? a.n_tiles[1] : a.n_tiles[0];
+  float* slabs = second ? a.slabs[1] : a.slabs[0];
+  WgradProblem pb = args.p[0];
+#pragma unroll
+  for (int i = 1; i < kMaxProblems; ++i)
+    if (i < args.n_problems && (int)blockIdx.x >= args.p[i].first_block) pb = args.p[i];
+  switch (pb.shape) {
+#define X(name, id, NXF, NYF, WI, WO, SPI) \
+  case name: wgrad_body<NXF, NYF, WI, WO, SPI, false>(pb, save, gdump, n_tiles, lay, slabs); break;
+    LNRF_WGRAD_SHAPES(X, default: X)
+#undef X
+  }
+}
+
 __global__ __launch_bounds__(64 * kSlabReduceWaves) void nerf_wgrad_reduce_kernel(WgradArgs args,
                                                                                  const float* __restrict__ slabs,
                                                                                  float* __restrict__ grads) {
@@ -322,22 +353,20 @@
   }
 }
 
-__global__ void nerf_pack_kernel(const float* __restrict__ params, char* __restrict__ packed) {
-  constexpr int64_t units_f = (int64_t)kFwdFrags * 64, units_b = (int64_t)kBwdFrags * 64;
-  constexpr int64_t total = units_f + units_b + kBiasFloats;
+__global__ void nerf_pack_kernel(const float* __restrict__ params, char* __restrict__ packed,
+                                 const int32_t* __restrict__ table) {
+  constexpr int64_t total = kPackUnits + kBiasFloats;
   for (int64_t u = (int64_t)blockIdx.x * blockDim.x + threadIdx.x; u < total; u += (int64_t)gridDim.x * blockDim.x) {
-    if (u < units_f + units_b) {
-      const bool fwd = u < units_f;
-      const int64_t uu = fwd ? u : u - units_f;
-      const int g = (int)(uu >> 6), lane = (int)(uu & 63);
+    if (u < kPackUnits) {
+      const int4 lo = *reinterpret_cast<const int4*>(table + u * 8), hi = *reinterpret_cast<const int4*>(table + u * 8 + 4);
+      const int idx[8] = {lo.x, lo.y, lo.z, lo.w, hi.x, hi.y, hi.z, hi.w};
       bf16x8 out;
 #pragma unroll
-      for (int j = 0; j < 8; ++j)
-        out[j] = (__bf16)param_or_zero(params, fwd ? fwd_stream_index(g, lane, j, false) : bwd_stream_index(g, lane, j, false));
-      *reinterpret_cast<bf16x8*>(packed + (fwd ? kPackFwdOff : kPackBwdOff) + uu * 16) = out;
+      for (int j = 0; j < 8; ++j) out[j] = (__bf16)param_or_zero(params, idx[j]);
+      *reinterpret_cast<bf16x8*>(packed + u * 16) = out;
     } else {
-      const int i = (int)(u - units_f - units_b);
-      reinterpret_cast<float*>(packed + kPackBiasOff)[i] = param_or_zero(params, bias_block_index(i, false));
+      const int i = (int)(u - kPackUnits);
+      reinterpret_cast<float*>(packed + kPackBiasOff)[i] = param_or_zero(params, table[kPackUnits * 8 + i]);
     }
   }
 }
@@ -384,11 +413,39 @@
   return nerf_shape_fused(s) ? grad_dump_bytes(m) + kWgradSlabBytes : -1;
 }
 
+static int nerf_pack_table(const int32_t** out) {
+  constexpr int kMaxDevices = 64;
+  static std::mutex lock;
+  static const int32_t* tables[kMaxDevices] = {};
+  int dev = 0;
+  hipError_t e = hipGetDevice(&dev);
+  if (e != hipSuccess) return hip_fail(e, "hipGetDevice");
+  LNRF_CHECK_ARG(dev >= 0 && dev < kMaxDevices, "device index out of range");
+  std::lock_guard<std::mutex> guard(lock);
+  if (!tables[dev]) {
+    std::vector<int32_t> host((size_t)kPackTableInts);
+    for (int64_t i = 0; i < kPackTableInts; ++i) host[(size_t)i] = pack_table_entry(i);
+    void* buf = nullptr;
+    e = hipMalloc(&buf, host.size() * sizeof(int32_t));
+    if (e != hipSuccess) return hip_fail(e, "hipMalloc(pack table)");
+    e = hipMemcpy(buf, host.data(), host.size() * sizeof(int32_t), hipMemcpyHostToDevice);
+    if (e != hipSuccess) {
+      (void)hipFree(buf);
+      return hip_fail(e, "hipMemcpy(pack table)");
+    }
+    tables[dev] = static_cast<const int32_t*>(buf);
+  }
+  *out = tables[dev];
+  return LNRF_OK;
+}
+
 extern "C" int lnrf_nerf_pack_weights(const lnrf_nerf_shape* shape, const float* params, void* packed,
                                       lnrf_stream_t stream) {
   LNRF_REQUIRE_NERF_SHAPE(shape);
   LNRF_CHECK_ARG(params && packed, "null pointer");
-  hipLaunchKernelGGL(nerf_pack_kernel, dim3(640), dim3(256), 0, as_stream(stream), params, (char*)packed);
+  const int32_t* table = nullptr;
+  if (int rc = nerf_pack_table(&table)) return rc;
+  hipLaunchKernelGGL(nerf_pack_kernel, dim3(640), dim3(256), 0, as_stream(stream), params, (char*)packed, table);
   LNRF_LAUNCH_CHECK();
   return LNRF_OK;
 }
@@ -523,6 +580,30 @@
   return LNRF_OK;
 }
 
+int lnrf::launch_nerf_wgrad_pair(const WgradList* list, const void* const* xbuf, const void* const* ybuf,
+                                 const int64_t* n_tiles, float* const* slabs, hipStream_t stream, WgLayout lay) {
+  const int lds = 2 * 2 * 36 * kFragBytes;
+  const int first = n_tiles[1] > n_tiles[0] ? 1 : 0;
+  Wgrad2Args a;
+  for (int y = 0; y < 2; ++y) {
+    const int k = y == 0 ? first : 1 - first;
+    LNRF_CHECK_ARG(slabs[k] != nullptr && list[k].blocks <= kWgradMaxBlocks,
+                   "needs slabs, and holds at most kWgradMaxBlocks of them");
+    a.args[y] = list[k].args;
+    a.save[y] = (const char*)xbuf[k];
+    a.gdump[y] = (const char*)ybuf[k];
+    a.n_tiles[y] = n_tiles[k];
+    a.slabs[y] = slabs[k];
+    a.blocks[y] = list[k].blocks;
+  }
+  int rc = set_max_dynamic_lds(nerf_wgrad2_kernel, lds);
+  if (rc) return rc;
+  const int gx = a.blocks[0] > a.blocks[1] ? a.blocks[0] : a.blocks[1];
+  hipLaunchKernelGGL(nerf_wgrad2_kernel, dim3((unsigned)gx, 2), dim3(kThreads), lds, stream, a, lay);
+  LNRF_LAUNCH_CHECK();
+  return LNRF_OK;
+}
+
 extern "C" int lnrf_nerf_mlp_bwd_weights(const lnrf_nerf_shape* shape, const void* save, void* scratch,
                                          int64_t m, float* grads, lnrf_stream_t stream) {
   LNRF_REQUIRE_NERF_SHAPE(shape);
diff --git a/learn-nerf_amd/csrc/rays.hip b/learn-nerf_amd/csrc/rays.hip
--- a/learn-nerf_amd/csrc/rays.hip
+++ b/learn-nerf_amd/csrc/rays.hip
@@ -199,6 +199,108 @@
   }
 }
 
+__device__ __forceinline__ void composite_bwd_block(
+    int64_t block, float (*s_bg)[3], const float* __restrict__ ts, const float* __restrict__ t_min,
+    const float* __restrict__ t_max, const uint8_t* __restrict__ mask, const float* __restrict__ density,
+    const float* __restrict__ rgb, const float* __restrict__ aux, int n_aux, const float* __restrict__ background,
+    int64_t n_rays, int T, const float* __restrict__ g_out, const float* __restrict__ outputs,
+    const float* __restrict__ targets, int64_t target_stride, float out_scale, float gw0, float gw1, float gw2, float gw3,
+    float* __restrict__ g_density, float* __restrict__ g_rgb, float* __restrict__ g_aux,
+    float* __restrict__ g_background, float* __restrict__ bg_parts) {
+  const int lane = threadIdx.x & 63;
+  const int wave = threadIdx.x >> 6;
+  const int64_t n = block * (blockDim.x >> 6) + wave;
+  const bool live = n < n_rays;
+  const float gw[kMaxAux] = {gw0, gw1, gw2, gw3};
+  float gbg[3] = {0, 0, 0};
+  if (live) {
+    const float* ts_row = ts + n * T;
+    const float* de_row = density + n * T;
+    const float tmin = t_min[n], tmax = t_max[n];
+    const bool m = mask[n] != 0;
+    float g[3];
+#pragma unroll
+    for (int c = 0; c < 3; ++c)
+      g[c] = g_out ? g_out[n * 3 + c]
+                   : out_scale * (outputs[n * 3 + c] - targets[n * target_stride + c]);
+    if (!m) {
+      for (int i = lane; i < T; i += 64) {
+        const int64_t e = n * T + i;
+        g_density[e] = 0.0f;
+#pragma unroll
+        for (int c = 0; c < 3; ++c) g_rgb[e * 3 + c] = 0.0f;
+        for (int k = 0; k < n_aux; ++k) g_aux[e * n_aux + k] = 0.0f;
+      }
+#pragma unroll
+      for (int c = 0; c < 3; ++c) gbg[c] = g[c];
+    } else {
+      float carry = 0.0f, f_part = 0.0f;
+      for (int base = 0; base < T; base += 64) {
+        const int i = base + lane;
+        const Quad q = quad_chunk(ts_row, de_row, T, i, lane, tmin, tmax, carry);
+        if (i < T) {
+          const float p = expf(-q.prev) * (1.0f - expf(-q.a));
+          const int64_t e = n * T + i;
+          float w = 0.0f;
+#pragma unroll
+          for (int c = 0; c < 3; ++c) w += g[c] * rgb[e * 3 + c];
+          for (int k = 0; k < n_aux; ++k) w += gw[k] * aux[e * n_aux + k];
+          f_part += p * w;
+        }
+        carry = __shfl(q.incl, 63, 64);
+      }
+      const float p_bg = expf(-carry);
+      float w_bg = 0.0f;
+#pragma unroll
+      for (int c = 0; c < 3; ++c) w_bg += g[c] * background[c];
+      const float F = wave_sum(f_part) + p_bg * w_bg;
+      carry = 0.0f;
+      float pw_carry = 0.0f;
+      for (int base = 0; base < T; base += 64) {
+        const int i = base + lane;
+        const Quad q = quad_chunk(ts_row, de_row, T, i, lane, tmin, tmax, carry);
+        const bool valid = i < T;
+        const int64_t e = n * T + (valid ? i : T - 1);
+        float p = 0.0f, w = 0.0f;
+        if (valid) {
+          p = expf(-q.prev) * (1.0f - expf(-q.a));
+#pragma unroll
+          for (int c = 0; c < 3; ++c) w += g[c] * rgb[e * 3 + c];
+          for (int k = 0; k < n_aux; ++k) w += gw[k] * aux[e * n_aux + k];
+        }
+        const float pw_incl = wave_incl_scan(p * w, lane) + pw_carry;
+        if (valid) {
+          const float s_next = expf(-q.incl);
+          const float rest = F - pw_incl;
+          const float t_p = i > 0 ? ts_row[i - 1] : 0.0f;
+          const float start = i == 0 ? tmin : (q.t + t_p) / 2.0f;
+          const float dl = q.end - start;
+          g_density[e] = dl * (s_next * w - rest);
+#pragma unroll
+          for (int c = 0; c < 3; ++c) g_rgb[e * 3 + c] = p * g[c];
+          for (int k = 0; k < n_aux; ++k) g_aux[e * n_aux + k] = p * gw[k];
+        }
+        carry = __shfl(q.incl, 63, 64);
+        pw_carry = __shfl(pw_incl, 63, 64);
+      }
+#pragma unroll
+      for (int c = 0; c < 3; ++c) gbg[c] = p_bg * g[c];
+    }
+  }
+  if (g_background) {
+    if (lane == 0) {
+#pragma unroll
+      for (int c = 0; c < 3; ++c) s_bg[wave][c] = gbg[c];
+    }
+    __syncthreads();
+    if (threadIdx.x < 3) {
+      float s = 0.0f;
+      for (int w = 0; w < (int)(blockDim.x >> 6); ++w) s += s_bg[w][threadIdx.x];
+      bg_parts[block * 4 + threadIdx.x] = s;
+    }
+  }
+}
+
 __global__ void composite_bwd_kernel(const float* __restrict__ ts, const float* __restrict__ t_min,
                                      const float* __restrict__ t_max,
                                      const uint8_t* __restrict__ mask,
@@ -213,98 +315,28 @@
                                      float* __restrict__ g_aux, float* __restrict__ g_background,
                                      float* __restrict__ bg_parts) {
   __shared__ float s_bg[16][3];
-  const int lane = threadIdx.x & 63;
-  const int wave = threadIdx.x >> 6;
-  const int64_t n = (int64_t)blockIdx.x * (blockDim.x >> 6) + wave;
-  const bool live = n < n_rays;
-  const float gw[kMaxAux] = {gw0, gw1, gw2, gw3};
-  float gbg[3] = {0, 0, 0};
-  if (live) {
-    const float* ts_row = ts + n * T;
-    const float* de_row = density + n * T;
-    const float tmin = t_min[n], tmax = t_max[n];
-    const bool m = mask[n] != 0;
-    float g[3];
-#pragma unroll
-    for (int c = 0; c < 3; ++c)
-      g[c] = g_out ? g_out[n * 3 + c]
-                   : out_scale * (outputs[n * 3 + c] - targets[n * target_stride + c]);
-    if (!m) {
-      for (int i = lane; i < T; i += 64) {
-        const int64_t e = n * T + i;
-        g_density[e] = 0.0f;
-#pragma unroll
-        for (int c = 0; c < 3; ++c) g_rgb[e * 3 + c] = 0.0f;
-        for (int k = 0; k < n_aux; ++k) g_aux[e * n_aux + k] = 0.0f;
-      }
-#pragma unroll
-      for (int c = 0; c < 3; ++c) gbg[c] = g[c];
-    } else {
-      float carry = 0.0f, f_part = 0.0f;
-      for (int base = 0; base < T; base += 64) {
-        const int i = base + lane;
-        const Quad q = quad_chunk(ts_row, de_row, T, i, lane, tmin, tmax, carry);
-        if (i < T) {
-          const float p = expf(-q.prev) * (1.0f - expf(-q.a));
-          const int64_t e = n * T + i;
-          float w = 0.0f;
-#pragma unroll
-          for (int c = 0; c < 3; ++c) w += g[c] * rgb[e * 3 + c];
-          for (int k = 0; k < n_aux; ++k) w += gw[k] * aux[e * n_aux + k];
-          f_part += p * w;
-        }
-        carry = __shfl(q.incl, 63, 64);
-      }
-      const float p_bg = expf(-carry);
-      float w_bg = 0.0f;
-#pragma unroll
-      for (int c = 0; c < 3; ++c) w_bg += g[c] * background[c];
-      const float F = wave_sum(f_part) + p_bg * w_bg;
-      carry = 0.0f;
-      float pw_carry = 0.0f;
-      for (int base = 0; base < T; base += 64) {
-        const int i = base + lane;
-        const Quad q = quad_chunk(ts_row, de_row, T, i, lane, tmin, tmax, carry);
-        const bool valid = i < T;
-        const int64_t e = n * T + (valid ? i : T - 1);
-        float p = 0.0f, w = 0.0f;
-        if (valid) {
-          p = expf(-q.prev) * (1.0f - expf(-q.a));
-#pragma unroll
-          for (int c = 0; c < 3; ++c) w += g[c] * rgb[e * 3 + c];
-          for (int k = 0; k < n_aux; ++k) w += gw[k] * aux[e * n_aux + k];
-        }
-        const float pw_incl = wave_incl_scan(p * w, lane) + pw_carry;
-        if (valid) {
-          const float s_next = expf(-q.incl);
-          const float rest = F - pw_incl;
-          const float t_p = i > 0 ? ts_row[i - 1] : 0.0f;
-          const float start = i == 0 ? tmin : (q.t + t_p) / 2.0f;
-          const float dl = q.end - start;
-          g_density[e] = dl * (s_next * w - rest);
-#pragma unroll
-          for (int c = 0; c < 3; ++c) g_rgb[e * 3 + c] = p * g[c];
-          for (int k = 0; k < n_aux; ++k) g_aux[e * n_aux + k] = p * gw[k];
-        }
-        carry = __shfl(q.incl, 63, 64);
-        pw_carry = __shfl(pw_incl, 63, 64);
-      }
-#pragma unroll
-      for (int c = 0; c < 3; ++c) gbg[c] = p_bg * g[c];
-    }
-  }
-  if (g_background) {
-    if (lane == 0) {
-#pragma unroll
-      for (int c = 0; c < 3; ++c) s_bg[wave][c] = gbg[c];
-    }
-    __syncthreads();
-    if (threadIdx.x < 3) {
-      float s = 0.0f;
-      for (int w = 0; w < (int)(blockDim.x >> 6); ++w) s += s_bg[w][threadIdx.x];
-      bg_parts[(int64_t)blockIdx.x * 4 + threadIdx.x] = s;
-    }
-  }
+  composite_bwd_block(blockIdx.x, s_bg, ts, t_min, t_max, mask, density, rgb, aux, n_aux, background, n_rays, T, g_out,
+                      outputs, targets, target_stride, out_scale, gw0, gw1, gw2, gw3, g_density, g_rgb, g_aux,
+                      g_background, bg_parts);
+}
+
+struct CompositeBwdPass {
+  const float *ts, *density, *rgb, *aux, *g_out, *outputs;
+  float *g_density, *g_rgb, *g_aux, *bg_parts;
+  float gw[kMaxAux];
+  int n_aux, T;
+};
+__global__ void composite_bwd_pair_kernel(CompositeBwdPass p0, CompositeBwdPass p1, int blocks0,
+                                          const float* __restrict__ t_min, const float* __restrict__ t_max,
+                                          const uint8_t* __restrict__ mask, const float* __restrict__ background,
+                                          int64_t n_rays, const float* __restrict__ targets, int64_t target_stride,
+                                          float out_scale, float* __restrict__ g_background) {
+  __shared__ float s_bg[16][3];
+  const bool first = (int)blockIdx.x < blocks0;
+  const CompositeBwdPass& p = first ? p0 : p1;
+  composite_bwd_block(first ? blockIdx.x : blockIdx.x - blocks0, s_bg, p.ts, t_min, t_max, mask, p.density, p.rgb, p.aux,
+                      p.n_aux, background, n_rays, p.T, p.g_out, p.outputs, targets, target_stride, out_scale, p.gw[0],
+                      p.gw[1], p.gw[2], p.gw[3], p.g_density, p.g_rgb, p.g_aux, g_background, p.bg_parts);
 }
 
 __global__ __launch_bounds__(256) void composite_bg_fold_kernel(const float* __restrict__ parts, int n_blocks,
@@ -326,6 +358,38 @@
     __syncthreads();
   }
   if (threadIdx.x < 3) atomicAdd(g_background + threadIdx.x, red[0][threadIdx.x]);
+}
+
+__global__ __launch_bounds__(256) void composite_bg_fold_pair_kernel(const float* __restrict__ parts0,
+                                                                     const float* __restrict__ parts1, int n_blocks,
+                                                                     float* __restrict__ g_background) {
+  __shared__ float red[256][3];
+  float total[2] = {0.0f, 0.0f};
+#pragma unroll
+  for (int pass = 0; pass < 2; ++pass) {
+    const float* parts = pass == 0 ? parts0 : parts1;
+    float s[3] = {0.0f, 0.0f, 0.0f};
+    for (int b = threadIdx.x; b < n_blocks; b += 256) {
+      const float4 v = *reinterpret_cast<const float4*>(parts + (int64_t)b * 4);
+      s[0] += v.x; s[1] += v.y; s[2] += v.z;
+    }
+#pragma unroll
+    for (int c = 0; c < 3; ++c) red[threadIdx.x][c] = s[c];
+    __syncthreads();
+    for (int half = 128; half > 0; half >>= 1) {
+      if ((int)threadIdx.x < half) {
+#pragma unroll
+        for (int c = 0; c < 3; ++c) red[threadIdx.x][c] += red[threadIdx.x + half][c];
+      }
+      __syncthreads();
+    }
+    if (threadIdx.x < 3) total[pass] = red[0][threadIdx.x];
+    __syncthreads();
+  }
+  if (threadIdx.x < 3) {
+    atomicAdd(g_background + threadIdx.x, total[0]);
+    atomicAdd(g_background + threadIdx.x, total[1]);
+  }
 }
 
 struct Dist {
@@ -693,6 +757,50 @@
   return LNRF_OK;
 }
 
+extern "C" int lnrf_composite_bwd_det2(const float* t_min, const float* t_max, const uint8_t* mask,
+                                       const float* background, int64_t n_rays, const float* targets,
+                                       int64_t target_stride, float out_scale,
+                                       const float* ts_a, const float* density_a, const float* rgb_a, const float* aux_a,
+                                       int32_t n_aux_a, int32_t t_a, const float* g_out_a, const float* outputs_a,
+                                       const float* g_aux_w_a, float* g_density_a, float* g_rgb_a, float* g_aux_a,
+                                       const float* ts_b, const float* density_b, const float* rgb_b, const float* aux_b,
+                                       int32_t n_aux_b, int32_t t_b, const float* g_out_b, const float* outputs_b,
+                                       const float* g_aux_w_b, float* g_density_b, float* g_rgb_b, float* g_aux_b,
+                                       float* g_background, void* scratch, int64_t scratch_bytes, lnrf_stream_t stream) {
+  if (n_rays == 0) return LNRF_OK;
+  const int64_t part_bytes = lnrf_composite_bwd_scratch_bytes(n_rays);
+  if (n_rays > 0 && g_background)
+    LNRF_CHECK_ARG(scratch && scratch_bytes >= 2 * part_bytes && (reinterpret_cast<uintptr_t>(scratch) & 15u) == 0,
+                   "scratch too small or unaligned");
+  LNRF_CHECK_ARG(t_min && t_max && mask && background, "null pointer");
+  LNRF_CHECK_ARG(n_rays >= 0 && n_rays <= (int64_t)1 << 30, "bad sizes");
+  const int wpb = 4;
+  const int blocks = (int)((n_rays + wpb - 1) / wpb);
+  CompositeBwdPass p[2] = {
+      {ts_a, density_a, rgb_a, aux_a, g_out_a, outputs_a, g_density_a, g_rgb_a, g_aux_a, nullptr, {0, 0, 0, 0}, n_aux_a, t_a},
+      {ts_b, density_b, rgb_b, aux_b, g_out_b, outputs_b, g_density_b, g_rgb_b, g_aux_b, nullptr, {0, 0, 0, 0}, n_aux_b, t_b}};
+  const float* g_aux_w[2] = {g_aux_w_a, g_aux_w_b};
+  for (int k = 0; k < 2; ++k) {
+    LNRF_CHECK_ARG(p[k].ts && p[k].density && p[k].rgb, "null pointer");
+    LNRF_CHECK_ARG(p[k].g_density && p[k].g_rgb, "null gradient outputs");
+    LNRF_CHECK_ARG(p[k].g_out || (p[k].outputs && targets), "need g_out or outputs+targets");
+    LNRF_CHECK_ARG(p[k].T >= 1, "bad sizes");
+    LNRF_CHECK_ARG(p[k].n_aux >= 0 && p[k].n_aux <= kMaxAux && (p[k].n_aux == 0 || (p[k].aux && p[k].g_aux && g_aux_w[k])),
+                   "bad aux");
+    for (int i = 0; i < p[k].n_aux; ++i) p[k].gw[i] = g_aux_w[k][i];
+    if (g_background) p[k].bg_parts = reinterpret_cast<float*>(reinterpret_cast<char*>(scratch) + k * part_bytes);
+  }
+  hipLaunchKernelGGL(composite_bwd_pair_kernel, dim3((unsigned)(2 * blocks)), dim3(wpb * 64), 0, as_stream(stream), p[0],
+                     p[1], blocks, t_min, t_max, mask, background, n_rays, targets, target_stride, out_scale, g_background);
+  LNRF_LAUNCH_CHECK();
+  if (g_background) {
+    hipLaunchKernelGGL(composite_bg_fold_pair_kernel, dim3(1), dim3(256), 0, as_stream(stream),
+                       (const float*)p[0].bg_parts, (const float*)p[1].bg_parts, blocks, g_background);
+    LNRF_LAUNCH_CHECK();
+  }
+  return LNRF_OK;
+}
+
 extern "C" int lnrf_distortion(const float* ts, const float* t_min, const float* t_max, const uint8_t* mask,
                                const float* density, int64_t n_rays, int32_t t, float grad_scale, float* loss,
                                float* g_density, lnrf_stream_t stream) {
diff --git a/learn-nerf_amd/learn_nerf/_lib.py b/learn-nerf_amd/learn_nerf/_lib.py
--- a/learn-nerf_amd/learn_nerf/_lib.py
+++ b/learn-nerf_amd/learn_nerf/_lib.py
@@ -61,6 +61,9 @@
     "lnrf_composite_bwd_scratch_bytes": (c_int64, [c_int64]),
     "lnrf_composite_bwd_det": (c_int32, [_P, _P, _P, _P, _P, _P, _P, c_int32, _P, c_int64, c_int32, _P, _P, _P,
                                          c_int64, c_float, _F3, _P, _P, _P, _P, _P, c_int64, _P]),
+    "lnrf_composite_bwd_det2": (c_int32, [_P, _P, _P, _P, c_int64, _P, c_int64, c_float]
+                                + 2 * [_P, _P, _P, _P, c_int32, c_int32, _P, _P, _F3, _P, _P, _P]
+                                + [_P, _P, c_int64, _P]),
     "lnrf_distortion": (c_int32, [_P, _P, _P, _P, _P, c_int64, c_int32, c_float, _P, _P, _P]),
     "lnrf_sinusoidal_emb": (c_int32, [_P, c_int64, c_int64, c_int32, c_int32, _P, c_int64, c_int64, _P]),
     "lnrf_dense_fwd": (c_int32, [_P, c_int64, _P, _P, c_int32, _P, c_int64, c_int64, c_int32, c_int32, _P]),
diff --git a/learn-nerf_amd/learn_nerf/ops.py b/learn-nerf_amd/learn_nerf/ops.py
--- a/learn-nerf_amd/learn_nerf/ops.py
+++ b/learn-nerf_amd/learn_nerf/ops.py
@@ -250,6 +250,34 @@
     return g_density, g_rgb, g_aux
 
 
+def composite_bwd_pair(t_min, t_max, mask, background, g_background, targets, out_scale: float, coarse, fine):
+    n = t_min.shape[0]
+    dev = _dev(t_min)
+    assert targets.shape == (n, 3) and targets.stride(1) == 1
+    tstride, tptr = targets.stride(0), L.c_void_p(targets.data_ptr())
+    args, outs, keep = [], [], []
+    for p in (coarse, fine):
+        ts, aux, g_aux_w = p["ts"], p.get("aux"), p.get("g_aux_w", ())
+        t = ts.shape[1]
+        assert ts.shape[0] == n
+        n_aux = 0 if aux is None else aux.shape[-1]
+        g_density = torch.empty((n, t), dtype=F32, device=dev)
+        g_rgb = torch.empty((n, t, 3), dtype=F32, device=dev)
+        g_aux = torch.empty((n, t, n_aux), dtype=F32, device=dev) if n_aux else None
+        gw = (L.c_float * 4)(*([float(x) for x in g_aux_w] + [0.0] * (4 - len(g_aux_w))))
+        keep.append(gw)
+        args += [L.ptr(ts), L.ptr(p["density"]), L.ptr(p["rgb"]), L.ptr(aux), n_aux, t, None, L.ptr(p["outputs"]), gw,
+                 L.ptr(g_density), L.ptr(g_rgb), L.ptr(g_aux)]
+        outs.append((g_density, g_rgb, g_aux))
+    nbytes = 2 * L.lib().lnrf_composite_bwd_scratch_bytes(n)
+    lease = _ws.lease("composite_bwd", nbytes, dev)
+    L.check(L.lib().lnrf_composite_bwd_det2(
+        L.ptr(t_min), L.ptr(t_max), L.ptr(mask, torch.uint8), L.ptr(background), n, tptr, tstride, float(out_scale),
+        *args, L.ptr(g_background), L.ptr(lease.buf, torch.uint8), nbytes, L.stream()), "composite_bwd_det2")
+    lease.release()
+    return outs[0], outs[1]
+
+
 def distortion(ts, t_min, t_max, mask, density, g_density=None, grad_scale: float = 0.0, want_loss: bool = True):
     n, t = ts.shape
     assert want_loss or g_density is not None
diff --git a/learn-nerf_amd/learn_nerf/train.py b/learn-nerf_amd/learn_nerf/train.py
--- a/learn-nerf_amd/learn_nerf/train.py
+++ b/learn-nerf_amd/learn_nerf/train.py
@@ -201,8 +201,16 @@
         if want_grad and coarse_done is None and _ls_pair(self.coarse, ctx_c, self.fine, ctx_f):
             from .model import backward_ls_pair
 
-            gd_c, grgb_c, _ = output_grads("coarse", ts_c, dens_c, rgb_c, out_c, names_c, auxs_c)
-            gd_f, grgb_f, _ = output_grads("fine", ts_f, dens_f, rgb_f, out_f, names_f, auxs_f)
+            passes = [dict(ts=ts, density=dens, rgb=rgb, outputs=out, aux=auxs,
+                           g_aux_w=[self.loss_weights[k] / n for k in names])
+                      for ts, dens, rgb, out, names, auxs in ((ts_c, dens_c, rgb_c, out_c, names_c, auxs_c),
+                                                              (ts_f, dens_f, rgb_f, out_f, names_f, auxs_f))]
+            (gd_c, grgb_c, _), (gd_f, grgb_f, _) = ops.composite_bwd_pair(t_min, t_max, mask, bg, gbg, targets,
+                                                                          out_scale, *passes)
+            if dist_w is not None:
+                for prefix, ts, dens, gd in (("coarse", ts_c, dens_c, gd_c), ("fine", ts_f, dens_f, gd_f)):
+                    dist_rays[prefix] = ops.distortion(ts, t_min, t_max, mask, dens,
+                                                       g_density=gd if dist_w != 0.0 else None, grad_scale=dist_w / n)
             backward_ls_pair(ctx_c, gd_c, grgb_c, gc, ctx_f, gd_f, grgb_f, gf)
         elif want_grad:
             if coarse_done is None:
```

Result: no change. 188.1 million ray-samples/s, median of 6 (+0.7%).
